# Division/CUDA-RayTracing

Hardware: AMD Instinct MI355X
Metric: Mrays/s + achieved HBM GB/s, Stanford bunny 1920x1080x8spp @1/2/4/8 GPU (higher is better)
Workload: dtype f32

## Files before the change

### cuda-raytracing_amd/__init__.py

```python
import contextlib
import ctypes
import os

import numpy as np
import torch

PKG_DIR = os.path.dirname(os.path.abspath(__file__))
ROOT_DIR = os.path.dirname(PKG_DIR)
LIB_PATH = os.path.join(PKG_DIR, "librt_hip.so")
EXP_LIB_PATH = os.path.join(PKG_DIR, "librt_hip_exp.so")
ASSETS_DIR = os.path.join(ROOT_DIR, "assets")

RT_RENDER_STATS = 1
RT_RENDER_VALIDATE = 16
TRACERS = {"fast": 0, "ref": 2, "flat": 4, "wavefront": 8}
STAT_NAMES = ("segments", "nodes", "tri_tests", "tri_accepts", "sphere_accepts", "hits", "misses", "cycles_tree_cut",
              "wave_small_iters", "lane_small", "wave_big_tris", "lane_big_tris", "wave_segment_iters",
              "lane_segments", "tree_nodes", "tree_tri_tests", "cycles_small", "cycles_big", "cycles_total",
              "rounds_coop", "rounds_shared", "coop_rays", "cycles_tree_clusters", "cycles_tree_tris",
              "big_tests", "twin_decided", "twin_tests", "wave_big_iters", "defer_end2", "defer_redo", None, None)
STAT_COUNT = len(STAT_NAMES)
SCENES = {"bunny": 0, "bunny4": 1, "plane1m": 2}

REFERENCE_SPP = 5
REFERENCE_BOUNCES = 6
RNG_STATE_BYTES = 48


class GPUCamera(ctypes.Structure):
    _fields_ = [("origin", ctypes.c_float * 3), ("viewport_worldspace_size", ctypes.c_float * 2),
                ("aspect", ctypes.c_float), ("horizontal", ctypes.c_float * 3),
                ("vertical", ctypes.c_float * 3), ("lower_left_corner", ctypes.c_float * 3)]


class GPUScene(ctypes.Structure):
    _fields_ = [("gpu_spheres", ctypes.c_void_p), ("gpu_materials", ctypes.c_void_p),
                ("gpu_bvh_nodes", ctypes.c_void_p), ("gpu_bvh_face_indices", ctypes.c_void_p),
                ("gpu_vertices", ctypes.c_void_p), ("gpu_faces", ctypes.c_void_p),
                ("sphere_count", ctypes.c_int32), ("material_count", ctypes.c_int32),
                ("rng_state", ctypes.c_void_p), ("environment_cubemap_tex", ctypes.c_uint64),
                ("camera", GPUCamera)]


class GPUMaterial(ctypes.Structure):
    _fields_ = [("albedo", ctypes.c_float * 4), ("emissive", ctypes.c_float * 4), ("specular", ctypes.c_float * 4),
                ("roughness", ctypes.c_float), ("specular_percent", ctypes.c_float), ("IOR", ctypes.c_float),
                ("_pad", ctypes.c_float)]


class BuildOptions(ctypes.Structure):
    _fields_ = [("leaf_tree_min", ctypes.c_uint32), ("cut_clusters", ctypes.c_uint32), ("cluster_max", ctypes.c_uint32),
                ("split_angle", ctypes.c_float), ("bvh_small", ctypes.c_uint32), ("host_bvh", ctypes.c_int32),
                ("leaf_screens", ctypes.c_int32)]


class RenderParams(ctypes.Structure):
    _fields_ = [("surface", ctypes.c_void_p), ("surface_last_frame", ctypes.c_void_p),
                ("width", ctypes.c_int32), ("height", ctypes.c_int32), ("pitch", ctypes.c_uint64),
                ("frame_index", ctypes.c_int32), ("spp", ctypes.c_int32), ("bounces", ctypes.c_int32),
                ("shard_index", ctypes.c_int32), ("shard_count", ctypes.c_int32), ("flags", ctypes.c_int32),
                ("out_shard", ctypes.c_void_p), ("stats", ctypes.c_void_p), ("segment_counter", ctypes.c_void_p),
                ("tile_list", ctypes.c_void_p), ("tile_count", ctypes.c_int64), ("wave_clock", ctypes.c_void_p),
                ("tune", ctypes.c_uint32), ("lane_slots", ctypes.c_void_p), ("lane_slot_count", ctypes.c_int64),
                ("lane_cost", ctypes.c_void_p), ("priority_waves", ctypes.c_int64), ("refill_lanes", ctypes.c_int32),
                ("waves_per_simd", ctypes.c_int32), ("lone_slots", ctypes.c_void_p), ("lone_count", ctypes.c_int64)]


class Ray(ctypes.Structure):
    _fields_ = [("origin", ctypes.c_float * 3), ("tmax", ctypes.c_float), ("direction", ctypes.c_float * 3),
                ("reserved", ctypes.c_uint32)]


class Hit(ctypes.Structure):
    _fields_ = [("t", ctypes.c_float), ("kind", ctypes.c_uint32), ("id", ctypes.c_uint32), ("material", ctypes.c_uint32),
                ("normal", ctypes.c_float * 3), ("bx", ctypes.c_float), ("position", ctypes.c_float * 3),
                ("by", ctypes.c_float)]


class TraceParams(ctypes.Structure):
    _fields_ = [("rays", ctypes.c_void_p), ("count", ctypes.c_int64), ("width", ctypes.c_int32), ("height", ctypes.c_int32),
                ("hits", ctypes.c_void_p), ("flags", ctypes.c_uint32), ("waves_per_simd", ctypes.c_int32)]


class DenoiseParams(ctypes.Structure):
    _fields_ = [("surface", ctypes.c_void_p), ("pitch", ctypes.c_uint64), ("width", ctypes.c_int32), ("height", ctypes.c_int32),
                ("hits", ctypes.c_void_p), ("materials", ctypes.c_void_p), ("material_count", ctypes.c_int32),
                ("flags", ctypes.c_int32), ("out", ctypes.c_void_p), ("out_pitch", ctypes.c_uint64),
                ("scratch", ctypes.c_void_p), ("scratch_bytes", ctypes.c_uint64), ("iterations", ctypes.c_int32),
                ("normal_power_log2", ctypes.c_int32), ("sigma_plane", ctypes.c_float), ("sigma_color", ctypes.c_float)]


HIT_MISS, HIT_SPHERE, HIT_TRIANGLE = 0, 1, 2
RAY_TMAX = 1e30
DENOISE_DEFAULT = -1
DENOISE_DEFAULTS = {"iterations": 5, "normal_power_log2": 5, "sigma_plane": 0.03, "sigma_color": 8.0}

assert ctypes.sizeof(GPUScene) == 136 and ctypes.sizeof(GPUMaterial) == 64
assert ctypes.sizeof(Ray) == 32 and ctypes.sizeof(Hit) == 48 and ctypes.sizeof(TraceParams) == 40
assert ctypes.sizeof(DenoiseParams) == 96

_P, _I, _U32, _U64, _F, _SZ = ctypes.c_void_p, ctypes.c_int, ctypes.c_uint32, ctypes.c_uint64, ctypes.c_float, ctypes.c_size_t
_FP = ctypes.POINTER(ctypes.c_float)
SIGNATURES = {
    "raytracing_process": (None, [_P, _P, _I, _I, _SZ, _I, _P]),
    "init_rng": (None, [_U32, _U32, _P, ctypes.c_uint]),
    "rt_render": (_I, [ctypes.POINTER(RenderParams), _P, _P]),
    "rt_trace_rays": (_I, [ctypes.POINTER(TraceParams), _P, _P]),
    "rt_denoise_scratch_bytes": (_SZ, [_I, _I]),
    "rt_denoise": (_I, [ctypes.POINTER(DenoiseParams), _P]),
    "rt_foreign_mirror_wait": (_I, [_P]),
    "rt_foreign_last_tracer": (_I, [_P]),
    "rt_experimental_loaded": (_I, []),
    "rt_init_rng": (_I, [_P, _I, _I, _I, _I, _U32, _P]),
    "rt_shard_tiles": (ctypes.c_int64, [_I, _I, _I, _I]),
    "rt_unshard": (_I, [_P, _U64, _I, _I, _I, _P, ctypes.c_int64, _P]),
    "rt_shard_plan_capacity": (ctypes.c_int64, [_I, _I, _I]),
    "rt_shard_plan": (_I, [_I, _I, _I, _P, ctypes.c_int64, _P, _P]),
    "rt_get_build_options": (None, [_P]),
    "rt_set_build_options": (_I, [_P]),
    "rt_lane_plan_capacity": (ctypes.c_int64, [ctypes.c_int64]),
    "rt_lane_plan": (ctypes.c_int64, [_P, ctypes.c_int64, ctypes.c_double, ctypes.c_double, _P, ctypes.c_int64, _P]),
    "rt_lone_plan": (ctypes.c_int64, [_P, ctypes.c_int64, ctypes.c_int64, _U32, _P]),
    "rt_lane_refine": (ctypes.c_int64, [_P, ctypes.c_int64, _P, ctypes.c_int64, _P, ctypes.c_double, _P, ctypes.c_int64,
                                        _P]),
    "rt_init_rng_tiles": (_I, [_P, _I, _I, _P, ctypes.c_int64, _U32, _P]),
    "rt_unshard_tiles": (_I, [_P, _U64, _I, _I, _I, _P, ctypes.c_int64, _P, _P]),
    "rt_comm_unique_id": (_I, [_P]),
    "rt_comm_init_rank": (_I, [ctypes.POINTER(_P), _I, _I, _P]),
    "rt_comm_init_all": (_I, [_P, _I, _P]),
    "rt_comm_destroy": (_I, [_P]),
    "rt_comm_rank": (_I, [_P]),
    "rt_comm_size": (_I, [_P]),
    "rt_comm_group_start": (_I, []),
    "rt_comm_group_end": (_I, []),
    "rt_gather_shards": (_I, [_P, _P, _SZ, _P, _SZ, _P, _I, _P]),
    "rt_tonemap_srgb8": (_I, [_P, _U64, _I, _I, _P, _P]),
    "rt_write_pfm": (_I, [ctypes.c_char_p, _P, _U64, _I, _I]),
    "rt_write_ppm": (_I, [ctypes.c_char_p, _P, _I, _I]),
    "rt_set_device": (_I, [_I]),
    "rt_device_count": (_I, []),
    "rt_malloc": (_I, [ctypes.POINTER(_P), _SZ]),
    "rt_malloc_pitch": (_I, [ctypes.POINTER(_P), ctypes.POINTER(_SZ), _SZ, _SZ]),
    "rt_free": (_I, [_P]),
    "rt_memcpy_h2d": (_I, [_P, _P, _SZ]),
    "rt_memcpy_d2h": (_I, [_P, _P, _SZ]),
    "rt_memcpy_d2d": (_I, [_P, _P, _SZ]),
    "rt_memset": (_I, [_P, _I, _SZ]),
    "rt_synchronize": (_I, []),
    "rt_last_error": (ctypes.c_char_p, []),
    "rt_cubemap_create": (_U64, [_FP, _I]),
    "rt_cubemap_destroy": (_I, [_U64]),
    "rt_scene_create": (_P, []),
    "rt_scene_destroy": (None, [_P]),
    "rt_scene_add_material": (_U32, [_P, ctypes.POINTER(GPUMaterial)]),
    "rt_scene_add_triangle": (None, [_P, _FP, _FP, _FP, _I]),
    "rt_scene_add_quad": (None, [_P, _FP, _FP, _FP, _FP, _I]),
    "rt_scene_add_sphere": (None, [_P, _FP, _F, _I]),
    "rt_scene_add_mesh_file": (_I, [_P, ctypes.c_char_p, _FP, _I]),
    "rt_scene_set_environment_file": (_I, [_P, ctypes.c_char_p]),
    "rt_scene_environment": (_I, [_P, ctypes.POINTER(_P), ctypes.POINTER(_I)]),
    "rt_scene_set_camera": (None, [_P, _FP, _F, _F]),
    "rt_scene_set_viewport": (None, [_P, _I, _I]),
    "rt_scene_upload": (_I, [_P, _P]),
    "rt_scene_gpu": (ctypes.POINTER(GPUScene), [_P]),
    "rt_scene_setup": (_I, [_P, _I, ctypes.c_char_p]),
    "rt_scene_setup_plane": (_I, [_P, _I, ctypes.c_char_p]),
    "rt_scene_build": (None, [_P]),
    "rt_scene_camera": (None, [_P, ctypes.POINTER(GPUCamera)]),
    "rt_scene_host_arrays": (_SZ, [_P, ctypes.POINTER(_P), ctypes.POINTER(_SZ), ctypes.POINTER(_P),
                                   ctypes.POINTER(_SZ), ctypes.POINTER(_P), ctypes.POINTER(_SZ), ctypes.POINTER(_P)]),
    "rt_scene_bvh_max_depth": (_I, [_P]),
    "rt_scene_materials": (_I, [_P, _P, ctypes.POINTER(_SZ)]),
    "rt_bvh_build_device": (_I, [_P, _U32, _P, _U32, _P, _P, ctypes.POINTER(_U32), ctypes.POINTER(_I), _P]),
    "rt_scene_mirror_info": (_I, [_P, ctypes.POINTER(_SZ), ctypes.POINTER(_SZ), ctypes.POINTER(_SZ)]),
    "rt_scene_mirror_copy": (_I, [_P, _P, _P, _P]),
    "rt_scene_mirror_nodes": (_I, [_P, _P, ctypes.POINTER(_SZ)]),
    "rt_scene_mirror_face_leaf": (_I, [_P, _P, ctypes.POINTER(_SZ)]),
    "rt_scene_mirror_twins": (_I, [_P, _P, ctypes.POINTER(_SZ), _P, ctypes.POINTER(_SZ)]),
    "rt_mirror_build_check": (_I, [_P, _SZ, _P, _SZ, _P, _SZ, _P, _SZ, _P, ctypes.POINTER(ctypes.c_int)]),
    "rt_cluster_cull_host": (_I, [_P, _P, ctypes.c_float, _P]),
    "rt_twin_check_host": (_I, [_P, _P, _P]),
    "rt_xorwow_jump_matrix": (_I, [_I, ctypes.POINTER(ctypes.c_uint32)]),
    "rt_xorwow_init_host": (None, [_U32, _U64, _P]),
}

_lib = None


class RTError(RuntimeError):
    pass


def lib():
    global _lib
    if _lib is None:
        if not os.path.exists(LIB_PATH):
            raise RTError(f"{LIB_PATH} not built; run `python -c 'import __graft_entry__ as g; g.build()'`")
        L = ctypes.CDLL(LIB_PATH)
        for name, (res, args) in SIGNATURES.items():
            fn = getattr(L, name)
            fn.restype = res
            fn.argtypes = args
        _lib = L
    return _lib


_exp_lib = None


def load_experimental():
    global _exp_lib
    lib()
    if _exp_lib is None:
        if not os.path.exists(EXP_LIB_PATH):
            raise RTError(f"{EXP_LIB_PATH} not built; run `python -c 'import __graft_entry__ as g; g.build()'`")
        _exp_lib = ctypes.CDLL(EXP_LIB_PATH)
    if lib().rt_experimental_loaded() != 1:
        raise RTError("librt_hip_exp.so loaded but its kernels are not registered with librt_hip.so: "
                      + lib().rt_last_error().decode(errors="replace"))
    return _exp_lib


def _check(code, what):
    if code:
        raise RTError(f"{what} failed ({code}): {lib().rt_last_error().decode(errors='replace')}")


def _f3(v):
    return (ctypes.c_float * 3)(*[float(x) for x in v])


def _stream_ptr(stream=None):
    s = stream if stream is not None else torch.cuda.current_stream()
    return ctypes.c_void_p(s.cuda_stream)


class Scene:

    def __init__(self):
        self.handle = lib().rt_scene_create()
        if not self.handle:
            raise RTError("rt_scene_create failed")

    def __del__(self):
        if getattr(self, "handle", None) and _lib is not None:
            _lib.rt_scene_destroy(self.handle)
            self.handle = None

    def add_material(self, albedo=(0, 0, 0), emissive=(0, 0, 0), specular=(0, 0, 0, 0), roughness=0.9,
                     specular_percent=0.0, ior=1.0):
        m = GPUMaterial()
        m.albedo[:] = [*map(float, albedo[:3]), 1.0]
        m.emissive[:] = [*map(float, emissive[:3]), 1.0]
        m.specular[:] = [*map(float, (list(specular) + [0.0])[:4])]
        m.roughness, m.specular_percent, m.IOR = roughness, specular_percent, ior
        return lib().rt_scene_add_material(self.handle, ctypes.byref(m))

    def add_triangle(self, a, b, c, material=0):
        lib().rt_scene_add_triangle(self.handle, _f3(a), _f3(b), _f3(c), material)

    def add_quad(self, a, b, c, d, material=0):
        lib().rt_scene_add_quad(self.handle, _f3(a), _f3(b), _f3(c), _f3(d), material)

    def add_sphere(self, position, radius, material=0):
        lib().rt_scene_add_sphere(self.handle, _f3(position), float(radius), material)

    def add_loaded_scene(self, mesh_path, transform, material=0):
        t = (ctypes.c_float * 16)(*[float(x) for x in transform])
        _check(lib().rt_scene_add_mesh_file(self.handle, mesh_path.encode(), t, material), "add_loaded_scene")

    def set_environment(self, path):
        _check(lib().rt_scene_set_environment_file(self.handle, path.encode()), "set_environment")

    def environment(self):
        p, n = ctypes.c_void_p(), ctypes.c_int()
        _check(lib().rt_scene_environment(self.handle, ctypes.byref(p), ctypes.byref(n)), "rt_scene_environment")
        if not p.value:
            return None
        k = n.value
        buf = ctypes.string_at(p.value, 6 * k * k * 16)
        return np.frombuffer(buf, dtype=np.float32).reshape(6, k, k, 4).copy()

    def setup(self, which="bunny", assets_dir=ASSETS_DIR):
        _check(lib().rt_scene_setup(self.handle, SCENES[which], assets_dir.encode()), f"setup({which})")

    def setup_plane(self, n=708, assets_dir=ASSETS_DIR):
        _check(lib().rt_scene_setup_plane(self.handle, int(n), assets_dir.encode()), f"setup_plane({n})")

    def set_camera(self, position=(0, 0, 0), angle_x=0.0, angle_y=180.0):
        lib().rt_scene_set_camera(self.handle, _f3(position), float(angle_x), float(angle_y))

    def set_viewport(self, width, height):
        lib().rt_scene_set_viewport(self.handle, int(width), int(height))

    def upload(self, rng_state_ptr):
        _check(lib().rt_scene_upload(self.handle, ctypes.c_void_p(rng_state_ptr)), "upload")

    @property
    def gpu(self):
        return lib().rt_scene_gpu(self.handle)

    def build(self):
        lib().rt_scene_build(self.handle)

    def camera(self):
        c = GPUCamera()
        lib().rt_scene_camera(self.handle, ctypes.byref(c))
        return c

    def max_depth(self):
        return lib().rt_scene_bvh_max_depth(self.handle)

    def mirror(self, trees=False):
        import numpy as np
        n = [ctypes.c_size_t() for _ in range(3)]
        _check(lib().rt_scene_mirror_info(self.handle, *[ctypes.byref(x) for x in n]), "rt_scene_mirror_info")
        tris = np.zeros((n[0].value, 12), dtype=np.float32)
        tree = np.zeros((n[1].value, 16), dtype=np.float32)
        ltris = np.zeros((n[2].value, 12), dtype=np.float32)
        _check(lib().rt_scene_mirror_copy(self.handle, tris.ctypes.data, tree.ctypes.data, ltris.ctypes.data),
               "rt_scene_mirror_copy")
        return (tris, tree, ltris) if trees else tris

    def mirror_nodes(self):
        import numpy as np
        n = ctypes.c_size_t()
        _check(lib().rt_scene_mirror_nodes(self.handle, None, ctypes.byref(n)), "rt_scene_mirror_nodes")
        out = np.zeros((n.value, 8), dtype=np.float32)
        _check(lib().rt_scene_mirror_nodes(self.handle, out.ctypes.data, ctypes.byref(n)), "rt_scene_mirror_nodes")
        return out

    def mirror_face_leaf(self):
        import numpy as np
        n = ctypes.c_size_t()
        _check(lib().rt_scene_mirror_face_leaf(self.handle, None, ctypes.byref(n)), "rt_scene_mirror_face_leaf")
        out = np.zeros(n.value, dtype=np.uint32)
        if n.value:
            _check(lib().rt_scene_mirror_face_leaf(self.handle, out.ctypes.data, ctypes.byref(n)), "rt_scene_mirror_face_leaf")
        return out

    def mirror_twins(self):
        import numpy as np
        nq, nu = ctypes.c_size_t(), ctypes.c_size_t()
        _check(lib().rt_scene_mirror_twins(self.handle, None, ctypes.byref(nq), None, ctypes.byref(nu)), "rt_scene_mirror_twins")
        q = np.zeros((nq.value, 28), dtype=np.float32)
        u = np.zeros((nu.value, 16), dtype=np.float32)
        _check(lib().rt_scene_mirror_twins(self.handle, q.ctypes.data, ctypes.byref(nq), u.ctypes.data, ctypes.byref(nu)),
               "rt_scene_mirror_twins")
        return q, u

    def materials(self):
        n = ctypes.c_size_t()
        _check(lib().rt_scene_materials(self.handle, None, ctypes.byref(n)), "rt_scene_materials")
        out = np.zeros((n.value, 16), dtype=np.float32)
        if n.value:
            _check(lib().rt_scene_materials(self.handle, out.ctypes.data, ctypes.byref(n)), "rt_scene_materials")
        return out

    def host_arrays(self):
        import numpy as np
        ptrs = [ctypes.c_void_p() for _ in range(4)]
        counts = [ctypes.c_size_t() for _ in range(3)]
        lib().rt_scene_host_arrays(self.handle, ctypes.byref(ptrs[0]), ctypes.byref(counts[0]), ctypes.byref(ptrs[1]),
                                   ctypes.byref(counts[1]), ctypes.byref(ptrs[2]), ctypes.byref(counts[2]),
                                   ctypes.byref(ptrs[3]))

        def grab(p, nbytes):
            if not p.value or nbytes == 0:
                return np.zeros(0, dtype=np.uint8)
            return np.frombuffer(ctypes.string_at(p.value, nbytes), dtype=np.uint8).copy()

        nn, nf, nv = counts[0].value, counts[1].value, counts[2].value
        return {"nodes": grab(ptrs[0], nn * 32), "face_indices": grab(ptrs[1], nf * 4),
                "vertices": grab(ptrs[2], nv * 32), "faces": grab(ptrs[3], nf * 16)}


def mirror_build_check(nodes, face_indices, faces, vertices):
    import numpy as np
    nodes, fi = np.ascontiguousarray(nodes), np.ascontiguousarray(face_indices, dtype=np.uint32)
    faces, vertices = np.ascontiguousarray(faces), np.ascontiguousarray(vertices)
    meta = np.zeros((fi.size, 2), dtype=np.uint32)
    tw = ctypes.c_int(0)
    _check(lib().rt_mirror_build_check(nodes.ctypes.data, nodes.shape[0], fi.ctypes.data, fi.size, faces.ctypes.data,
                                       faces.shape[0], vertices.ctypes.data, vertices.shape[0], meta.ctypes.data,
                                       ctypes.byref(tw)), "rt_mirror_build_check")
    return meta, bool(tw.value)


def bvh_build_device(vertices, faces, stream=None):
    import torch
    nf = faces.shape[0]
    nodes = torch.empty((max(1, 2 * nf - 1), 8), dtype=torch.float32, device=faces.device)
    fi = torch.empty((nf,), dtype=torch.int32, device=faces.device)
    count, depth = _U32(0), _I(0)
    _check(lib().rt_bvh_build_device(vertices.data_ptr(), vertices.shape[0], faces.data_ptr(), nf, nodes.data_ptr(),
                                     fi.data_ptr(), ctypes.byref(count), ctypes.byref(depth), _stream_ptr(stream)),
           "rt_bvh_build_device")
    return nodes, fi, count.value, depth.value


def alloc_surface(width, height, device=None):
    row_floats = ((width * 16 + 255) // 256) * 256 // 4
    t = torch.zeros((height, row_floats), dtype=torch.float32, device=device or "cuda")
    return t


def surface_view(t, width):
    return t[:, : width * 4].reshape(t.shape[0], width, 4)


def alloc_rng(count, device=None):
    return torch.zeros((count * RNG_STATE_BYTES // 4,), dtype=torch.int32, device=device or "cuda")


def init_rng_states(rng, width, height, seed, shard_index=0, shard_count=1, stream=None):
    _check(lib().rt_init_rng(ctypes.c_void_p(rng.data_ptr()), width, height, shard_index, shard_count, seed,
                             _stream_ptr(stream)), "rt_init_rng")


def render(scene, surface, last, width, height, spp, bounces, frame_index=0, shard_index=0, shard_count=1,
           out_shard=None, stats=None, segment_counter=None, stream=None, tracer="fast", tile_list=None,
           wave_clock=None, tune=0, lane_slots=None, lane_cost=None, priority_waves=0, refill_lanes=0,
           waves_per_simd=0, lone_slots=None, validate=False):
    p = RenderParams()
    if lone_slots is not None and lone_slots.numel() > 0:
        assert lone_slots.dtype == torch.int32 and lone_slots.is_cuda and lone_slots.dim() == 1
        p.lone_slots, p.lone_count = lone_slots.data_ptr(), lone_slots.numel()
    if lane_slots is not None:
        assert lane_slots.dtype == torch.int32 and lane_slots.is_cuda and lane_slots.numel() % 64 == 0
        p.lane_slots, p.lane_slot_count = lane_slots.data_ptr(), lane_slots.numel()
        p.priority_waves = int(priority_waves)
    if lane_cost is not None:
        assert lane_cost.dtype == torch.int32 and lane_cost.is_cuda
        p.lane_cost = lane_cost.data_ptr()
    if tile_list is not None:
        assert tile_list.dtype == torch.int32 and tile_list.is_cuda and tile_list.dim() == 1
        p.tile_list, p.tile_count = tile_list.data_ptr(), tile_list.numel()
    if wave_clock is not None:
        n = tile_list.numel() if tile_list is not None else tiles_of(width, height, shard_index, shard_count)
        waves = lane_slots.numel() // 64 if lane_slots is not None else 4 * n
        assert wave_clock.dtype == torch.int64 and wave_clock.numel() >= waves
        p.wave_clock = wave_clock.data_ptr()
    p.tune = int(tune)
    p.refill_lanes = int(refill_lanes)
    p.waves_per_simd = int(waves_per_simd)
    p.surface = surface.data_ptr() if surface is not None else None
    p.surface_last_frame = last.data_ptr() if last is not None else None
    p.width, p.height = width, height
    p.pitch = surface.shape[1] * 4 if surface is not None else width * 16
    p.frame_index, p.spp, p.bounces = frame_index, spp, bounces
    p.shard_index, p.shard_count = shard_index, shard_count
    p.out_shard = out_shard.data_ptr() if out_shard is not None else None
    p.flags = TRACERS[tracer] | (RT_RENDER_VALIDATE if validate else 0)
    if segment_counter is not None:
        p.segment_counter = segment_counter.data_ptr()
    if stats is not None:
        p.flags |= RT_RENDER_STATS
        p.stats = stats.data_ptr()
    gpu = scene.gpu if hasattr(scene, "gpu") else ctypes.pointer(scene)
    _check(lib().rt_render(ctypes.byref(p), ctypes.cast(gpu, ctypes.c_void_p), _stream_ptr(stream)), "rt_render")


def _trace(scene, rays, count, width, height, hits, stream, waves_per_simd):
    if hits is None:
        hits = torch.empty((count, 12), dtype=torch.float32, device=rays.device if rays is not None else "cuda")
    assert hits.dtype == torch.float32 and hits.is_cuda and hits.is_contiguous() and hits.dim() == 2
    assert hits.shape[1] == 12 and hits.shape[0] >= count
    p = TraceParams()
    p.rays = rays.data_ptr() if rays is not None else None
    p.count, p.width, p.height = count, width, height
    p.hits = hits.data_ptr()
    p.waves_per_simd = int(waves_per_simd)
    gpu = scene.gpu if hasattr(scene, "gpu") else ctypes.pointer(scene)
    _check(lib().rt_trace_rays(ctypes.byref(p), ctypes.cast(gpu, ctypes.c_void_p), _stream_ptr(stream)), "rt_trace_rays")
    return hits


def trace_rays(scene, rays, hits=None, stream=None, waves_per_simd=0):
    assert rays.dtype == torch.float32 and rays.is_cuda and rays.is_contiguous() and rays.dim() == 2 and rays.shape[1] == 8
    return _trace(scene, rays, rays.shape[0], 0, 0, hits, stream, waves_per_simd)


def trace_camera(scene, width, height, hits=None, stream=None, waves_per_simd=0):
    return _trace(scene, None, int(width) * int(height), int(width), int(height), hits, stream, waves_per_simd)


def hit_fields(hits):
    ints = hits.view(torch.int32) if isinstance(hits, torch.Tensor) else hits.view(np.int32)
    return {"t": hits[:, 0], "kind": ints[:, 1], "id": ints[:, 2], "material": ints[:, 3], "normal": hits[:, 4:7],
            "bx": hits[:, 7], "position": hits[:, 8:11], "by": hits[:, 11]}


def gbuffer(scene, width, height, stream=None, waves_per_simd=0):
    w, h = int(width), int(height)
    f = hit_fields(trace_camera(scene, w, h, stream=stream, waves_per_simd=waves_per_simd))
    hit = f["kind"] != HIT_MISS
    mats = torch.from_numpy(scene.materials()).to(hit.device)
    albedo = torch.zeros((w * h, 3), dtype=torch.float32, device=hit.device)
    if mats.shape[0]:
        albedo = torch.where(hit[:, None], mats[f["material"].long().clamp(0, mats.shape[0] - 1), :3], albedo)
    return {"depth": torch.where(hit, f["t"], torch.full_like(f["t"], float("inf"))).reshape(h, w),
            "normal": f["normal"].reshape(h, w, 3).clone(), "position": f["position"].reshape(h, w, 3).clone(),
            "albedo": albedo.reshape(h, w, 3), "material": f["material"].reshape(h, w).clone(),
            "prim": torch.where(hit, f["id"], torch.full_like(f["id"], -1)).reshape(h, w),
            "kind": f["kind"].reshape(h, w).clone()}


def denoise_scratch_bytes(width, height):
    return int(lib().rt_denoise_scratch_bytes(int(width), int(height)))


def _allocating_on(stream):
    return torch.cuda.stream(stream) if stream is not None else contextlib.nullcontext()


def _denoise(surface, hits, materials_ptr, material_count, width, height, out, scratch, iterations, normal_power_log2,
             sigma_plane, sigma_color, stream):
    w, h = int(width), int(height)
    assert surface.dtype == torch.float32 and surface.is_cuda and surface.dim() == 2 and surface.stride(1) == 1
    assert surface.shape[0] >= h and surface.shape[1] >= 4 * w
    assert hits.dtype == torch.float32 and hits.is_cuda and hits.is_contiguous() and hits.dim() == 2
    assert hits.shape[1] == 12 and hits.shape[0] >= w * h
    need = denoise_scratch_bytes(w, h)
    with _allocating_on(stream):
        if out is None:
            out = alloc_surface(w, h, device=surface.device)
        if scratch is None:
            scratch = torch.empty((need // 4,), dtype=torch.float32, device=surface.device)
    assert out.dtype == torch.float32 and out.is_cuda and out.dim() == 2 and out.stride(1) == 1
    assert out.shape[0] >= h and out.shape[1] >= 4 * w
    assert scratch.is_cuda and scratch.is_contiguous()
    p = DenoiseParams()
    p.surface, p.pitch = surface.data_ptr(), surface.stride(0) * 4
    p.width, p.height = w, h
    p.hits, p.materials, p.material_count = hits.data_ptr(), materials_ptr, int(material_count)
    p.out, p.out_pitch = out.data_ptr(), out.stride(0) * 4
    p.scratch, p.scratch_bytes = scratch.data_ptr(), scratch.numel() * scratch.element_size()
    p.iterations, p.normal_power_log2 = int(iterations), int(normal_power_log2)
    p.sigma_plane, p.sigma_color = float(sigma_plane), float(sigma_color)
    _check(lib().rt_denoise(ctypes.byref(p), _stream_ptr(stream)), "rt_denoise")
    return out
# ... 234 lines not shown
```

### cuda-raytracing_amd/build.py

```python
import os
import re
import shutil
import subprocess
import sys

ROOT = os.path.dirname(os.path.dirname(os.path.abspath(__file__)))
PKG = os.path.join(ROOT, "cuda-raytracing_amd")
CSRC = os.path.join(PKG, "csrc")
INC = os.path.join(ROOT, "include")
BUILD = os.path.join(PKG, "build")
LIB = os.path.join(PKG, "librt_hip.so")
ORACLE_DIR = os.path.join(ROOT, "oracle")
ORACLE_LIB = os.path.join(ORACLE_DIR, "liboracle.so")

HIPCC = os.environ.get("HIPCC", "/opt/rocm/bin/hipcc")
ARCH = os.environ.get("RT_OFFLOAD_ARCH", "gfx950")

FP_FLAGS = ["-ffp-contract=off", "-fno-fast-math"]
HIP_CODEGEN_FLAGS = ["-mllvm", "-structurizecfg-skip-uniform-regions=1", "-mllvm", "-amdgpu-remove-redundant-endcf=0"]
HOST_SOURCES = ["scene.cpp", "objload.cpp", "mirror.cpp", "leaftree.cpp", "xorwow.cpp", "image.cpp", "shard.cpp"]
HIP_SOURCES = ["rt_fast_prod.hip", "rt_fast_lean.hip", "rt_fast_timing.hip", "rt_fast_stats.hip", "rt_ref.hip", "rt_kernel.hip", "image.hip",
               "bvh_build.hip", "comm.hip", "rt_query.hip", "denoise.hip"]
EXP_SOURCES = ["rt_fast_ab.hip", "rt_fast_ab2.hip", "rt_fast_refill.hip", "rt_fast_screen.hip", "rt_lone.hip", "rt_wavefront.hip",
               "rt_exp.hip"]
# ... 22 lines not shown
                 "-fhip-fp32-correctly-rounded-divide-sqrt", "-munsafe-fp-atomics", "-fno-slp-vectorize",
                 *HIP_CODEGEN_FLAGS, "-I", INC, "-I", CSRC, "-c", os.path.join(CSRC, src), "-o", obj]


LLVM_BIN = "/opt/rocm/lib/llvm/bin"
_VECTOR_OP = re.compile(r"\s*(v_|global_|scratch_|buffer_|ds_|flat_)")
_LANE_OP = re.compile(r"\s*v_(readlane|readfirstlane|writelane)_")


def disassemble(obj):
    import tempfile
    with tempfile.TemporaryDirectory() as td:
        fat, co = os.path.join(td, "fat.bin"), os.path.join(td, "dev.co")
        secs = subprocess.run([f"{LLVM_BIN}/llvm-readelf", "-S", obj], check=True, capture_output=True, text=True).stdout
        if ".hip_fatbin" not in secs:
            return ""
        subprocess.run([f"{LLVM_BIN}/llvm-objcopy", f"--dump-section=.hip_fatbin={fat}", obj, os.path.join(td, "x.o")],
                       check=True, capture_output=True)
        subprocess.run([f"{LLVM_BIN}/clang-offload-bundler", "--type=o", f"--targets=hipv4-amdgcn-amd-amdhsa--{ARCH}",
                        f"--input={fat}", f"--output={co}", "--unbundle"], check=True, capture_output=True)
        return subprocess.run([f"{LLVM_BIN}/llvm-objdump", "-d", f"--mcpu={ARCH}", co], check=True,
                              capture_output=True, text=True).stdout


def parse_disassembly(dis):
    base, ins = {}, []
    kernel = None
    for ln in dis.split("\n"):
        m = re.match(r"^([0-9a-f]+) <(\S+)>:$", ln)
        if m:
            kernel = m.group(2)
            base[kernel] = int(m.group(1), 16)
            continue
        m = re.match(r"^\t(.*?)\s*// ([0-9A-F]+):[0-9A-F ]*(?:<(\S+)\+0x([0-9a-f]+)>)?", ln)
        if m:
            tgt = (m.group(3), int(m.group(4), 16)) if m.group(3) else None
            ins.append((int(m.group(2), 16), m.group(1), tgt, kernel))
    return base, ins


def exec_narrowing_hazards(dis):
    base, ins = parse_disassembly(dis)
    at = {a: i for i, (a, _, _, _) in enumerate(ins)}
    out = []
    for i, (addr, text, _, k) in enumerate(ins):
        if not text.startswith("s_and_b64 exec, exec,"):
            continue
        j, target = i + 1, None
        while j < len(ins) and not ins[j][1].startswith("s_or_b64 exec, exec,"):
            if target is None and ins[j][1].startswith("s_cbranch_execz") and ins[j][2]:
                sym, off = ins[j][2]
                target = base.get(sym, -1) + off
            j += 1
        if target is None:
            continue
        if target not in at:
            out.append((k, addr, ["(execz target not found)"]))
            continue
        bad = []
        for _, tx, _, _ in ins[at[target]:]:
            if tx.startswith("s_or_b64 exec, exec,") or tx.startswith("s_endpgm"):
                break
            if _VECTOR_OP.match(tx) and not _LANE_OP.match(tx):
                bad.append(tx)
        if bad:
            out.append((k, addr, bad))
    return out


def check_exec_narrowing(objs):
    problems, flagged = [], []
    for obj in objs:
        dis = disassemble(obj)
        if dis and not parse_disassembly(dis)[1]:
            problems.append(f"{os.path.basename(obj)}: device code but no instruction parsed (llvm-objdump format?)")
            flagged.append(obj)
            continue
        for k, addr, bad in exec_narrowing_hazards(dis):
            problems.append(f"{os.path.basename(obj)}: {k} at 0x{addr:x}: " + "; ".join(bad[:4]))
            flagged.append(obj)
    if problems:
        for obj in set(flagged):
            for f in (obj, obj + ".cmd"):
                if os.path.exists(f):
                    os.remove(f)
        raise RuntimeError("exec narrowed without a save with vector code behind it (tools/exec_narrow_scan.py, "
                           "rt_fast_body.h RT_FAST_FAMILY):\n  " + "\n  ".join(problems))


def _compile(jobs, force):
    headers = _deps(CSRC, (".h",)) + _deps(INC, (".h",))

    def stale(j):
        obj, cmd = j
        rec = obj + ".cmd"
        same_cmd = os.path.exists(rec) and open(rec).read() == " ".join(cmd)
        return force or not same_cmd or not _newer(obj, [cmd[cmd.index("-c") + 1]] + headers)

    def run(j):
        _run(j[1])
        with open(j[0] + ".cmd", "w") as fh:
            fh.write(" ".join(j[1]))

    from concurrent.futures import ThreadPoolExecutor
    workers = max(1, min(len(jobs), int(os.environ.get("MAX_JOBS", os.cpu_count() or 1)), 8))
    todo = [j for j in jobs if stale(j)]
    with ThreadPoolExecutor(max_workers=workers) as ex:
        list(ex.map(run, todo))
    return bool(todo)


def build_product(force=False):
    os.makedirs(BUILD, exist_ok=True)
    jobs = [_hip_job(src) for src in HIP_SOURCES]
    for src in HOST_SOURCES:
        obj = os.path.join(BUILD, src + ".o")
        jobs.append((obj, ["g++", "-O2", "-std=c++17", "-fPIC", *FP_FLAGS, "-I", INC, "-I", CSRC,
                           "-c", os.path.join(CSRC, src), "-o", obj]))
    exp_jobs = [_hip_job(src) for src in EXP_SOURCES]
    changed = _compile(jobs + exp_jobs, force)
    objs = [o for o, _ in jobs]
    eobjs = [o for o, _ in exp_jobs]
    relink = changed or not _newer(LIB, objs)
    relink_exp = changed or not _newer(EXP_LIB, eobjs + [LIB])
    if relink or relink_exp:
        check_exec_narrowing([o for o, _ in jobs + exp_jobs if o.endswith(".hip.o")])
    if relink:
        tmp = LIB + ".tmp"
        _run([HIPCC, "-shared", "-fPIC", f"--offload-arch={ARCH}", *objs, "-L/opt/rocm/lib", "-lrccl", "-o", tmp])
        os.replace(tmp, LIB)
    if relink_exp:
        tmp = EXP_LIB + ".tmp"
        _run([HIPCC, "-shared", "-fPIC", f"--offload-arch={ARCH}", *eobjs, "-L", PKG, "-l:librt_hip.so",
              "-Wl,-rpath,$ORIGIN", "-Wl,--no-undefined", "-o", tmp])
        os.replace(tmp, EXP_LIB)
    return LIB


HOST_DRIVER_SRC = os.path.join(ROOT, "tests", "cpp", "host_driver.cpp")
HOST_DRIVER = os.path.join(ROOT, "tests", "cpp", "host_driver")


def build_host_driver(force=False):
    deps = [HOST_DRIVER_SRC, LIB, os.path.join(INC, "rt_abi.h")]
    if not os.path.exists(HOST_DRIVER_SRC) or (not force and _newer(HOST_DRIVER, deps)):
        return HOST_DRIVER
    tmp = HOST_DRIVER + ".tmp"
    _run(["g++", "-O2", "-std=c++17", "-I", INC, HOST_DRIVER_SRC, "-L", PKG, "-lrt_hip",
          "-Wl,-rpath,$ORIGIN/../../cuda-raytracing_amd", "-o", tmp])
    os.replace(tmp, HOST_DRIVER)
    return HOST_DRIVER


def build_oracle(force=False):
    src = os.path.join(ORACLE_DIR, "rt_oracle.c")
    deps = [src, os.path.abspath(__file__)] + _deps(ORACLE_DIR, (".h",))
    if not force and _newer(ORACLE_LIB, deps):
        return ORACLE_LIB
    tmp = ORACLE_LIB + ".tmp"
    _run(["gcc", "-O2", "-std=c11", "-fPIC", "-shared", "-fopenmp", *FP_FLAGS, src, "-o", tmp, "-lm"])
    os.replace(tmp, ORACLE_LIB)
    return ORACLE_LIB


def build_reference_parts(force=False):
    out = os.path.join(ORACLE_DIR, "_ref", "libref_glm.so")
    deps = [os.path.join(ORACLE_DIR, "ref_glm.cpp"), os.path.join(ORACLE_DIR, "build_ref.sh")]
    if not os.path.isdir("/root/reference/include/glm") or (not force and _newer(out, deps)):
        return out if os.path.exists(out) else None
    _run(["bash", os.path.join(ORACLE_DIR, "build_ref.sh")])
    return out


def build_all(force=False):
    build_product(force)
    build_oracle(force)
    build_reference_parts(force)
    build_host_driver(force)


if __name__ == "__main__":
    build_all(force="--force" in sys.argv)
```

### cuda-raytracing_amd/csrc/mirror.cpp

```cpp
#include "mirror.h"

#include <cstdlib>
#include <functional>

#include "leaftree.h"

#include <algorithm>
#include <cmath>
#include <cstring>
#include <map>
#include <mutex>
#include <stdexcept>
#include <string>

namespace {
void put_flat(float* o, const float* p0, const float* p1, const float* p2, uint32_t face) {
    o[0] = p0[0], o[1] = p0[1], o[2] = p0[2];
    o[3] = p1[0] - p0[0], o[4] = p1[1] - p0[1], o[5] = p1[2] - p0[2];
    o[6] = p2[0] - p0[0], o[7] = p2[1] - p0[1], o[8] = p2[2] - p0[2];
    std::memcpy(&o[9], &face, 4);
    o[10] = o[11] = 0.0f;
}
void put_pair(float* q, const float* a, const float* b) {
    static const float zero[12] = {};
    if (!b) b = zero;
    for (int c = 0; c < 9; c++) q[2 * c] = a[c], q[2 * c + 1] = b[c];
    std::memcpy(&q[18], &a[9], 4);
    std::memcpy(&q[19], &b[9], 4);
}
}

void rt_twin_bounds(const float* r, float* kd, float* ke) {
    const double U = std::ldexp(1.0, -24);
    const double n1 = std::fabs((double)r[3]) + std::fabs((double)r[4]) + std::fabs((double)r[5]);
    const double n2 = std::fabs((double)r[6]) + std::fabs((double)r[7]) + std::fabs((double)r[8]);
    const double w = 1.0 + std::ldexp(1.0, -20);
    *kd = (float)(10.0001 * U * n1 * n2 * w * w);
    *ke = (float)(10.0001 * U * std::max(n1, n2) * w * w);
}

namespace {
bool build_twins(const float* tris, uint32_t first, uint32_t count, std::vector<float>& quads,
                 std::vector<float>& units, uint32_t* nq, uint32_t* nu) {
    if (count >= 0xffffu) return false;
    auto key = [&](uint32_t i, bool swapped) {
        const float* r = &tris[(size_t)(first + i) * 12];
        std::string k(reinterpret_cast<const char*>(r), 12);
        k.append(reinterpret_cast<const char*>(r + (swapped ? 6 : 3)), 12);
        k.append(reinterpret_cast<const char*>(r + (swapped ? 3 : 6)), 12);
        return k;
    };
    std::map<std::string, std::vector<uint32_t>> by;
    for (uint32_t i = 0; i < count; i++) by[key(i, false)].push_back(i);
    std::vector<char> used(count, 0);
    std::vector<std::pair<uint32_t, uint32_t>> un;
    for (uint32_t i = 0; i < count; i++) {
        if (used[i]) continue;
        used[i] = 1;
        uint32_t twin = ~0u;
        auto it = by.find(key(i, true));
        if (it != by.end())
            for (uint32_t j : it->second)
                if (!used[j]) {
                    twin = j;
                    used[j] = 1;
                    break;
                }
        un.push_back({i, twin});
    }
    static const float zero[12] = {};
    const uint32_t none = ~0u;
    auto face = [&](uint32_t pos) { return pos == none ? none : *reinterpret_cast<const uint32_t*>(&tris[(size_t)(first + pos) * 12 + 9]); };
    auto packed = [&](uint32_t pos, uint32_t twin) { return (pos & 0xffffu) | ((twin == none ? 0xffffu : twin) << 16); };
    for (const auto& [pos, twin] : un) {
        float q[16] = {};
        std::memcpy(q, &tris[(size_t)(first + pos) * 12], 10 * 4);
        const uint32_t ft = face(twin), w = packed(pos, twin);
        std::memcpy(&q[10], &ft, 4);
        std::memcpy(&q[11], &w, 4);
        rt_twin_bounds(&tris[(size_t)(first + pos) * 12], &q[12], &q[13]);
        if (twin == none) q[12] = -1.0f;
        units.insert(units.end(), q, q + 16);
    }
    for (size_t u = 0; u < un.size(); u += 2) {
        const bool hb = u + 1 < un.size();
        const float* ra = &tris[(size_t)(first + un[u].first) * 12];
        const float* rb = hb ? &tris[(size_t)(first + un[u + 1].first) * 12] : zero;
        float q[28] = {};
        put_pair(q, ra, rb);
        float kd, ke;
        rt_twin_bounds(ra, &kd, &ke);
        q[20] = un[u].second == none ? -1.0f : kd, q[22] = ke;
        rt_twin_bounds(rb, &kd, &ke);
        q[21] = (!hb || un[u + 1].second == none) ? -1.0f : kd, q[23] = ke;
        const uint32_t wa = packed(un[u].first, un[u].second), wb = hb ? packed(un[u + 1].first, un[u + 1].second) : none;
        const uint32_t fa = face(un[u].second), fb = hb ? face(un[u + 1].second) : none;
        std::memcpy(&q[24], &wa, 4);
        std::memcpy(&q[25], &wb, 4);
        std::memcpy(&q[26], &fa, 4);
        std::memcpy(&q[27], &fb, 4);
        quads.insert(quads.end(), q, q + 28);
    }
    *nq = (uint32_t)((un.size() + 1) / 2);
    *nu = (uint32_t)un.size();
    return true;
}
}

void rt_build_mirror(const GPUBVHNode* nodes, size_t node_count, const uint32_t* fi, size_t index_count,
                     const GPUFace* faces, size_t face_count, const GPUVertex* verts, size_t vertex_count,
                     MirrorHost* out) {
    auto bad = [](const char* what) { throw std::runtime_error(std::string("mirror: ") + what); };
    out->tris.assign(index_count * 12, 0.0f);
    for (size_t i = 0; i < index_count; i++) {
        const uint32_t f = fi[i];
        if (f >= face_count) bad("face index out of range");
        const GPUFace& fc = faces[f];
        if (fc.v0 >= vertex_count || fc.v1 >= vertex_count || fc.v2 >= vertex_count) bad("vertex index out of range");
        put_flat(&out->tris[i * 12], verts[fc.v0].position, verts[fc.v1].position, verts[fc.v2].position, f);
    }

    out->pairs.clear();
    out->quads.clear();
    out->units.clear();
    out->tree.clear();
    out->ltris.clear();
    out->flat.clear();
    out->depth = 0;
    out->fast = true;
    out->screens = 0;
    std::vector<uint32_t> big;
    out->spairs.assign(index_count * 20, 0.0f);
    if (node_count == 0) return;
    std::vector<std::pair<uint32_t, int>> st{{0u, 0}};
    size_t visited = 0;
    while (!st.empty()) {
        const auto [n, d] = st.back();
        st.pop_back();
        if (n >= node_count) bad("node index out of range");
        if (++visited > node_count) bad("node graph is not a tree");
        const GPUBVHNode& nd = nodes[n];
        for (int k = 0; k < 3; k++) {
            const float lo = std::fabs(nd.bmin[k]), hi = std::fabs(nd.bmax[k]);
            if ((lo != 0.0f && (lo < 0x1p-60f || lo > 0x1p62f)) || (hi != 0.0f && (hi < 0x1p-60f || hi > 0x1p62f)))
                out->fast = false;
        }
        if (nd.prim_count > 0) {
            if ((size_t)nd.first_index + nd.prim_count > index_count) bad("leaf range out of range");
            out->depth = std::max(out->depth, d);
            if (nd.prim_count > MIRROR_BIG_LEAF)
                big.push_back(n);
            else
                for (uint32_t j = 0; j < nd.prim_count; j += 2)
                    put_pair(&out->spairs[((size_t)nd.first_index + j) * 20], &out->tris[((size_t)nd.first_index + j) * 12],
                             j + 1 < nd.prim_count ? &out->tris[((size_t)nd.first_index + j + 1) * 12] : nullptr);
        } else {
            st.push_back({nd.first_index, d + 1});
            st.push_back({nd.first_index + 1, d + 1});
        }
    }
// ... 52 lines not shown
        }
        po = (uint32_t)(out->pairs.size() / 20);
        std::memcpy(&lead[10], &po, 4);
        std::memcpy(&lead[11], &pf, 4);
        for (uint32_t j = 0; j < nd.prim_count; j += 2) {
            float q[20];
            put_pair(q, &out->tris[((size_t)nd.first_index + j) * 12],
                     j + 1 < nd.prim_count ? &out->tris[((size_t)nd.first_index + j + 1) * 12] : nullptr);
            out->pairs.insert(out->pairs.end(), q, q + 20);
        }
        const uint32_t qb = (uint32_t)(out->quads.size() / 28), ub = (uint32_t)(out->units.size() / 16);
        uint32_t nq = 0, nu = 0;
        if (twins_ok && build_twins(out->tris.data(), nd.first_index, nd.prim_count, out->quads, out->units, &nq, &nu)) {
            float* second = &out->tris[((size_t)nd.first_index + 1) * 12];
            float* third = &out->tris[((size_t)nd.first_index + 2) * 12];
            std::memcpy(&second[10], &qb, 4);
            std::memcpy(&second[11], &nq, 4);
            std::memcpy(&third[10], &ub, 4);
            std::memcpy(&third[11], &nu, 4);
        }
    }
    const uint32_t nl = (uint32_t)(out->ltris.size() / 12);
    for (uint32_t r : roots) std::memcpy(&out->tree[(size_t)r * 16 + 12], &nl, 4);
    rt_build_treelets(nodes, node_count, out->treelets);
    rt_build_private_nodes(nodes, node_count, out->nodes);
    out->face_leaf.clear();
    if (!out->pairs.empty() || !out->tree.empty()) {
        std::vector<uint32_t> fl(face_count, FACE_NO_LEAF);
        const size_t nn = out->nodes.size() / 8;
        for (size_t k = 0; k < nn; k++) {
            uint32_t first, count;
            std::memcpy(&first, &out->nodes[k * 8 + 6], 4);
            std::memcpy(&count, &out->nodes[k * 8 + 7], 4);
            if (count == 0 || (size_t)first + count > index_count) continue;
            for (uint32_t i = first; i < first + count; i++) {
                uint32_t f;
                std::memcpy(&f, &out->tris[(size_t)i * 12 + 9], 4);
                if (f >= face_count) continue;
                fl[f] = fl[f] == FACE_NO_LEAF || fl[f] == (uint32_t)k ? (uint32_t)k : FACE_TWO_LEAVES;
            }
        }
        out->face_leaf.resize(face_count);
        std::memcpy(out->face_leaf.data(), fl.data(), face_count * 4);
    }
}

void rt_build_private_nodes(const GPUBVHNode* nodes, size_t node_count, std::vector<float>& out) {
    out.clear();
    if (node_count == 0) return;
    std::vector<uint32_t> slot(node_count, ~0u);
    slot[0] = 0;
    uint32_t pairs = 0;
    std::vector<uint32_t> st{0u};
    while (!st.empty()) {
        const uint32_t v = st.back();
        st.pop_back();
        const GPUBVHNode& nd = nodes[v];
        if (nd.prim_count > 0) continue;
        const uint32_t l = nd.first_index, r = nd.first_index + 1;
        slot[l] = 2 + 2 * pairs, slot[r] = 3 + 2 * pairs;
        pairs++;
        st.push_back(l);
        st.push_back(r);
    }
    out.assign((size_t)(2 + 2 * pairs) * 8, 0.0f);
    for (size_t v = 0; v < node_count; v++) {
        if (slot[v] == ~0u) continue;
        GPUBVHNode nd = nodes[v];
        if (nd.prim_count == 0) nd.first_index = slot[nd.first_index];
        std::memcpy(&out[(size_t)slot[v] * 8], &nd, sizeof nd);
    }
}

std::vector<float> rt_ltris_device_layout(const std::vector<float>& ltris) {
    const size_t n = ltris.size() / 12;
    std::vector<float> d(ltris.size());
    for (size_t i = 0; i < n; i++)
        for (int f = 0; f < 3; f++) std::memcpy(&d[(f * n + i) * 4], &ltris[i * 12 + 4 * f], 16);
    return d;
}

void rt_build_treelets(const GPUBVHNode* nodes, size_t node_count, std::vector<float>& out) {
    out.clear();
    if (node_count == 0 || nodes[0].prim_count > 0) return;
    constexpr uint32_t EMPTY = 0xffffffffu;
    const float inf = INFINITY;
    std::vector<uint32_t> roots{0u};
    for (size_t k = 0; k < roots.size(); k++) {
        std::vector<uint32_t> taken{roots[k]};
        std::map<uint32_t, bool> expanded;
        for (size_t q = 0; q < taken.size(); q++) {
            const GPUBVHNode& nd = nodes[taken[q]];
            if (nd.prim_count > 0) continue;
            if (taken.size() + 2 > 63) break;
            expanded[taken[q]] = true;
            taken.push_back(nd.first_index + 1);
            taken.push_back(nd.first_index);
        }
        struct Slot { uint32_t node; int parent; uint32_t size; unsigned long long anc; };
        std::vector<Slot> slots;
        std::function<uint32_t(uint32_t, int, unsigned long long)> place = [&](uint32_t n, int parent,
                                                                                unsigned long long anc) -> uint32_t {
            const uint32_t me = (uint32_t)slots.size();
            slots.push_back({n, parent, 1u, anc});
            if (expanded.count(n)) {
                const unsigned long long a2 = anc | (1ull << me);
                const uint32_t s1 = place(nodes[n].first_index + 1, (int)me, a2);
                const uint32_t s2 = place(nodes[n].first_index, (int)me, a2);
                slots[me].size = 1u + s1 + s2;
            }
            return slots[me].size;
        };
        place(roots[k], -1, 0ull);
        const size_t base = out.size();
        out.resize(base + 64 * 12, 0.0f);
        for (uint32_t p = 0; p < 64; p++) {
            float* o = &out[base + p * 12];
            if (p >= slots.size()) {
                o[0] = o[1] = o[2] = inf, o[3] = o[4] = o[5] = -inf;
                std::memcpy(&o[7], &EMPTY, 4);
                continue;
            }
            const GPUBVHNode& nd = nodes[slots[p].node];
            o[0] = nd.bmin[0], o[1] = nd.bmin[1], o[2] = nd.bmin[2], o[3] = nd.bmax[0], o[4] = nd.bmax[1], o[5] = nd.bmax[2];
            uint32_t X = nd.first_index, cnt = nd.prim_count, frontier = 0u;
            if (cnt == 0 && !expanded.count(slots[p].node)) {
                X = (uint32_t)roots.size();
                roots.push_back(slots[p].node);
                frontier = 1u;
            }
            std::memcpy(&o[6], &X, 4);
            std::memcpy(&o[7], &cnt, 4);
            const uint32_t lo = (uint32_t)slots[p].anc, hi = (uint32_t)(slots[p].anc >> 32);
            std::memcpy(&o[8], &lo, 4);
            std::memcpy(&o[9], &hi, 4);
            std::memcpy(&o[10], &slots[p].size, 4);
            std::memcpy(&o[11], &frontier, 4);
        }
    }
}

namespace {
struct Entry {
    const void* face_indices;
    const void* vertices;
    const void* faces;
    void* block;
    MirrorDevice dev;
};
std::mutex g_mutex;
std::map<const void*, Entry> g_mirrors;

void release(Entry& e) {
    if (e.block) rt_free(e.block);
    e.block = nullptr;
}
}

int rt_internal_install_mirror(const GPUScene* s, const MirrorHost& m, bool owned, uint64_t fingerprint) {
    const std::vector<float> lt = rt_ltris_device_layout(m.ltris);
    const std::vector<float>* parts[11] = {&m.nodes, &m.tris, &m.pairs, &m.tree, &lt, &m.spairs, &m.flat, &m.treelets, &m.quads,
                                           &m.units, &m.face_leaf};
    size_t off[11], total = 0;
    for (int i = 0; i < 11; i++) {
        off[i] = total;
        total += (parts[i]->size() * 4 + 255) & ~(size_t)255;
    }
    void* block = nullptr;
    if (rt_malloc(&block, total + 256) != 0) return -1;
    char* b = static_cast<char*>(block);
    for (int i = 0; i < 11; i++)
        if (!parts[i]->empty() && rt_memcpy_h2d(b + off[i], parts[i]->data(), parts[i]->size() * 4) != 0) {
            rt_free(block);
            return -1;
        }
    auto at = [&](int i) -> const void* { return parts[i]->empty() ? nullptr : b + off[i]; };
    Entry e{s->gpu_bvh_face_indices, s->gpu_vertices, s->gpu_faces, block, {}};
    e.dev.nodes = at(0);
    e.dev.tris = b + off[1];
    e.dev.pairs = at(2);
    e.dev.tree = at(3);
    e.dev.ltris = at(4);
    e.dev.spairs = at(5);
    e.dev.flat = at(6);
    e.dev.treelets = at(7);
    e.dev.quads = at(8);
    e.dev.units = at(9);
    e.dev.face_leaf = at(10);
    e.dev.depth = m.depth;
    e.dev.fast = m.fast;
    e.dev.screens = m.screens;
    e.dev.owned = owned;
    e.dev.fingerprint = fingerprint;
    std::lock_guard<std::mutex> lock(g_mutex);
    auto it = g_mirrors.find(s->gpu_bvh_nodes);
    if (it != g_mirrors.end()) {
        release(it->second);
        g_mirrors.erase(it);
    }
    g_mirrors.emplace(s->gpu_bvh_nodes, e);
    return 0;
}

void rt_internal_forget_mirror(const void* gpu_nodes) {
    std::lock_guard<std::mutex> lock(g_mutex);
    auto it = g_mirrors.find(gpu_nodes);
    if (it == g_mirrors.end()) return;
    release(it->second);
    g_mirrors.erase(it);
}

bool rt_internal_lookup_mirror(const GPUScene* s, MirrorDevice* out) {
    std::lock_guard<std::mutex> lock(g_mutex);
    *out = MirrorDevice{};
    auto it = g_mirrors.find(s->gpu_bvh_nodes);
    if (it == g_mirrors.end()) return false;
    const Entry& e = it->second;
    if (e.face_indices != s->gpu_bvh_face_indices || e.vertices != s->gpu_vertices || e.faces != s->gpu_faces) {
        out->depth = e.dev.depth;
        return false;
    }
    *out = e.dev;
    return true;
}

namespace {
std::mutex g_opt_mutex;
rt_build_options default_options() {
    rt_build_options o;
    const LeafTreeParams p;
    o.leaf_tree_min = MIRROR_TREE_LEAF;
    o.cut_clusters = p.cut_clusters;
    o.cluster_max = p.cluster_max;
    o.split_angle = (float)p.split_angle;
    o.bvh_small = 16;
    o.host_bvh = 0;
    o.leaf_screens = 0;
    return o;
}
rt_build_options g_options = default_options();
}

extern "C" int rt_mirror_build_check(const GPUBVHNode* nodes, size_t node_count, const uint32_t* face_indices,
                                     size_t index_count, const GPUFace* faces, size_t face_count,
                                     const GPUVertex* vertices, size_t vertex_count, uint32_t* meta, int* twins) {
    try {
        MirrorHost m;
        rt_build_mirror(nodes, node_count, face_indices, index_count, faces, face_count, vertices, vertex_count, &m);
        for (size_t i = 0; i < index_count; i++) std::memcpy(&meta[2 * i], &m.tris[i * 12 + 10], 8);
        *twins = m.twins && !m.quads.empty() ? 1 : 0;
        return 0;
    } catch (const std::exception& e) {
        rt_internal_set_error(e.what());
        return -1;
    }
}

extern "C" void rt_get_build_options(rt_build_options* out) {
    if (!out) return;
    std::lock_guard<std::mutex> lock(g_opt_mutex);
    *out = g_options;
}

extern "C" int rt_set_build_options(const rt_build_options* o) {
    const rt_build_options v = o ? *o : default_options();
    if (v.leaf_tree_min < 2 || v.cut_clusters < 1 || v.cut_clusters > 32 || v.cluster_max < 1 || v.cluster_max > kClusterMax ||
        !(v.split_angle >= 0.0f && v.split_angle < 3.2f) || v.bvh_small < 2 || v.bvh_small > 64 || (v.host_bvh != 0 && v.host_bvh != 1) ||
        (v.leaf_screens != 0 && v.leaf_screens != 1)) {
        rt_internal_set_error("rt_set_build_options: value out of range");
        return 1;
    }
    std::lock_guard<std::mutex> lock(g_opt_mutex);
    g_options = v;
    return 0;
}
```

### cuda-raytracing_amd/csrc/mirror.h

```cpp
#pragma once

#include <cstddef>
#include <cstdint>
#include <vector>

#include "rt_abi.h"

constexpr uint32_t MIRROR_BIG_LEAF = 8;
constexpr uint32_t MIRROR_TREE_LEAF = 1024;
constexpr uint32_t FACE_NO_LEAF = 0xffffffffu, FACE_TWO_LEAVES = 0xfffffffeu;

struct MirrorHost {
    std::vector<float> nodes;
    std::vector<float> tris;
    std::vector<float> pairs;
    std::vector<float> quads;
    std::vector<float> units;
    std::vector<float> spairs;
    std::vector<float> tree;
    std::vector<float> ltris;
    std::vector<float> flat;
    std::vector<float> treelets;
    std::vector<float> face_leaf;
    int depth = 0;
    bool fast = true;
    int screens = 0;
    bool twins = true;
};

void rt_build_mirror(const GPUBVHNode* nodes, size_t node_count, const uint32_t* face_indices, size_t index_count,
                     const GPUFace* faces, size_t face_count, const GPUVertex* vertices, size_t vertex_count,
                     MirrorHost* out);

void rt_twin_bounds(const float* rec, float* kd, float* ke);

std::vector<float> rt_ltris_device_layout(const std::vector<float>& ltris);

void rt_build_private_nodes(const GPUBVHNode* nodes, size_t node_count, std::vector<float>& out);

void rt_build_treelets(const GPUBVHNode* nodes, size_t node_count, std::vector<float>& out);

struct MirrorDevice {
    const void* nodes = nullptr;
    const void* tris = nullptr;
    const void* pairs = nullptr;
    const void* quads = nullptr;
    const void* units = nullptr;
    const void* spairs = nullptr;
    const void* tree = nullptr;
    const void* ltris = nullptr;
    const void* flat = nullptr;
    const void* treelets = nullptr;
    const void* face_leaf = nullptr;
    int depth = -1;
    bool fast = false;
    int screens = 0;
    bool owned = true;
    uint64_t fingerprint = 0;
};
int rt_internal_install_mirror(const GPUScene* scene, const MirrorHost& m, bool owned = true,
                               uint64_t fingerprint = 0);
void rt_internal_forget_mirror(const void* gpu_nodes);
bool rt_internal_lookup_mirror(const GPUScene* scene, MirrorDevice* out);

void rt_internal_set_error(const char* msg);
```

### cuda-raytracing_amd/csrc/rt_common.h

```cpp
#pragma once

#include <hip/hip_runtime.h>

#include "rt_abi.h"
#include "rt_math.h"

namespace rtk {

constexpr int TILE = 16;
constexpr int BLOCK = 256;
constexpr int WAVE = 64;

struct FlatTri {
    float4 a, b, c;
};

struct RenderArgs {
    const GeometrySphere* spheres;
    const GPUMaterial* materials;
    const GPUBVHNode* nodes;
    const uint32_t* face_indices;
    const GPUVertex* vertices;
    const GPUFace* faces;
    const FlatTri* tris;
    rt_rng_state* rng;
    const float* sky;
    int sky_n;
    int sphere_count;
    GPUCamera cam;
    float qw, qx, qy, qz;
    char* surface;
    const char* last;
    float4* out_shard;
    uint64_t pitch;
    int width, height, frame_index, spp, bounces;
    int shard_index, shard_count, tiles_x;
    const int32_t* tile_list;
    unsigned long long* wave_clock;
    const int32_t* lane_slots;
    long long slot_count;
    long long entry_count;
    unsigned long long* queue_head;
    int refill_lanes;
    int waves_per_simd;
    uint32_t* lane_cost;
    int priority_waves;
    const int* gate;
    int gate_value;
    unsigned long long* stats;
    unsigned long long* seg_counter;
    int scene_fast;
    int screens;
    const float4* pairs;
    const float4* quads;
    const float4* units;
    const float4* tree;
    const float4* ltris;
    const float4* spairs;
    const float4* flat;
    const uint32_t* face_leaf;
    uint32_t tune;
};

struct Counters {
    unsigned long long seg = 0, node = 0, tri = 0, tacc = 0, sacc = 0, hit = 0, miss = 0;
    unsigned long long w_small = 0, l_small = 0, w_big = 0, l_big = 0, w_seg = 0, l_seg = 0;
    unsigned long long ktest = 0, ktri = 0;
    unsigned long long cy_small = 0, cy_big = 0, r_coop = 0, r_shared = 0, coop_rays = 0, w_iter = 0;
    unsigned long long cy_tcl = 0, cy_ttri = 0, cy_tree = 0;
    uint32_t lane_work = 0;
    unsigned long long big_tests = 0, tw_test = 0, tw_dec = 0, big_iters = 0;
    uint32_t end2 = 0, redo = 0;
};

__device__ __forceinline__ rtm::f3 ld3(const float* p) { return rtm::f3{p[0], p[1], p[2]}; }

__device__ __forceinline__ int shard_tile(const RenderArgs& a, int k) {
    const int t = a.tile_list ? a.tile_list[k] : a.shard_index + k * a.shard_count;
    return (t >= 0 && t < a.tiles_x * ((a.height + TILE - 1) / TILE)) ? t : -1;
}

__device__ __forceinline__ void tile_pixel(int tid, int* lx, int* ly) {
    const int w = tid >> 6, l = tid & 63;
    *lx = (w & 1) * 8 + (l & 7);
    *ly = (w >> 1) * 8 + (l >> 3);
}

}
```

### cuda-raytracing_amd/csrc/rt_fast.h

```cpp
#pragma once

namespace rtfast {

constexpr int BIG = 8;
constexpr int LEAN_BIT = 128;
constexpr int WAVE = 64;

using rtm::f3;

struct Ray {
    f3 o, d, nd, r;
    bool fast;
};

__device__ __forceinline__ bool in_range_or_zero(float v, float lo, float hi) {
    const float a = fabsf(v);
    return v == 0.0f || (a >= lo && a <= hi);
}

__device__ __forceinline__ Ray make_ray(f3 o, f3 d, f3 nd, bool scene_fast) {
    Ray R;
    R.o = o, R.d = d, R.nd = nd;
    R.r = rtm::mk(1.0f / d.x, 1.0f / d.y, 1.0f / d.z);
    const float dlo = 0x1p-40f, dhi = 0x1p20f;
// ... 687 lines not shown
}

template <bool TIMING, class C>
__device__ __forceinline__ void coop_tree(const float4* tris, const float4* tree, const float4* ltris, const float4* flat,
                                          unsigned long long m, uint32_t root_l, const Ray& R, Hit& h, const Trav& T,
                                          uint32_t* scratch, uint32_t tune, C& c) {
    const uint32_t lane = threadIdx.x & 63u;
    const bool order = (tune & 0x80000000u) != 0;
    const f3 rnd_l = rtm::mk(1.0f / R.nd.x, 1.0f / R.nd.y, 1.0f / R.nd.z);
    while (m) {
        const int r = __ffsll((long long)m) - 1;
        m &= m - 1;
        if (TIMING && lane == 0) c.r_coop++;
        const uint32_t root = (uint32_t)__builtin_amdgcn_readlane((int)root_l, r);
        const uint32_t f0 = (uint32_t)__builtin_amdgcn_readlane((int)T.first, r);
        const uint32_t c0 = (uint32_t)__builtin_amdgcn_readlane((int)T.count, r);
        Ray B;
        B.o = bcast3(R.o, r);
        B.nd = bcast3(R.nd, r);
        B.d = B.nd, B.r = B.nd;
        B.fast = __builtin_amdgcn_readlane(R.fast ? 1 : 0, r) != 0;
        const f3 rnd = bcast3(rnd_l, r);
        const float best = bcast(h.best, r);
        const f4v K2 = ((ConstF4)(tree + 4 * (size_t)root))[2];
        const f4v KR = ((ConstF4)(tree + 4 * (size_t)root))[3];
        const uint32_t cb = __float_as_uint(K2.x), nc = __float_as_uint(K2.y), kb = __float_as_uint(K2.z),
                       nk = __float_as_uint(K2.w);
        const size_t ln = __float_as_uint(KR.x);
        const float4* cl = flat + cb;
        const float4* ct = flat + kb;
        LeafBest L;
        L.t = best, L.j = 0, L.id = 0, L.bx = 0.0f, L.by = 0.0f, L.found = false;
        L.nan = !(best == best);
        const bool cull_ok = B.fast && !L.nan;
        float cbest = best;
        for (uint32_t kbase = 0; kbase < nk; kbase += 64u) {
            const uint32_t k = kbase + lane;
            bool need = false;
            uint32_t s0 = 0, s1 = 0;
            float te = 0.0f;
            if (k < nk) {
                const float4 K0 = ct[k], K1 = ct[nk + k], K3 = ct[3 * nk + k];
                s0 = __float_as_uint(K3.y), s1 = __float_as_uint(K3.z);
                need = !(cull_ok && (__float_as_uint(K3.w) & 1u) && cluster_cull(B, rnd, cbest, K0, K1, ct[2 * nk + k], K3));
                if (order) {
                    const float tx1 = (K0.x - B.o.x) * rnd.x, tx2 = (K1.x - B.o.x) * rnd.x;
                    const float ty1 = (K0.y - B.o.y) * rnd.y, ty2 = (K1.y - B.o.y) * rnd.y;
                    const float tz1 = (K0.z - B.o.z) * rnd.z, tz2 = (K1.z - B.o.z) * rnd.z;
                    te = fmaxf(fmaxf(fminf(tx1, tx2), fminf(ty1, ty2)), fminf(tz1, tz2));
                    te = te == te ? te : 0.0f;
                }
            }
            const unsigned long long mk = __ballot(need);
            const uint32_t ns = (uint32_t)__popcll(mk);
            if (TIMING && lane == 0) c.ktest += min(64u, nk - kbase), c.r_shared += ns;
            uint32_t rank = 0;
            if (order) {
                for (unsigned long long w = mk; w; w &= w - 1) {
                    const int b = __ffsll((long long)w) - 1;
                    const float tb = bcast(te, b);
                    rank += (tb < te || (tb == te && b < (int)lane)) ? 1u : 0u;
                }
            } else {
                rank = __builtin_amdgcn_mbcnt_hi((uint32_t)(mk >> 32), __builtin_amdgcn_mbcnt_lo((uint32_t)mk, 0u));
            }
            for (uint32_t q = 0; q < ns; q += 2) {
                const int a = __ffsll((long long)__ballot(need && rank == q)) - 1;
                const int b = q + 1 < ns ? __ffsll((long long)__ballot(need && rank == q + 1)) - 1 : -1;
                const uint32_t a0 = (uint32_t)__builtin_amdgcn_readlane((int)s0, a);
                const uint32_t a1 = (uint32_t)__builtin_amdgcn_readlane((int)s1, a);
                uint32_t b0 = 0, b1 = 0;
                if (b >= 0) {
                    b0 = (uint32_t)__builtin_amdgcn_readlane((int)s0, b);
                    b1 = (uint32_t)__builtin_amdgcn_readlane((int)s1, b);
                }
                const unsigned long long tc0 = TIMING ? __builtin_amdgcn_s_memtime() : 0;
                const uint32_t ci = lane < 32u ? a0 + lane : b0 + (lane - 32u);
                const bool has = lane < 32u ? ci < a1 : ci < b1;
                bool need2 = false;
                uint32_t tb = 0, n = 0;
                if (has) {
                    const float4 Q3 = cl[3 * nc + ci];
                    const uint32_t info = __float_as_uint(Q3.w);
                    tb = __float_as_uint(Q3.z), n = info >> 8;
                    need2 = !(cull_ok && (info & 1u) && cluster_cull(B, rnd, cbest, cl[ci], cl[nc + ci], cl[2 * nc + ci], Q3));
                }
                const unsigned long long mc = __ballot(need2);
                const uint32_t nsc = (uint32_t)__popcll(mc);
                if (TIMING && lane == 0) c.l_big++, c.ktest += __popcll(__ballot(has)), c.coop_rays += nsc;
                const unsigned long long tc1 = TIMING ? __builtin_amdgcn_s_memtime() : 0;
                if (TIMING) c.cy_tcl += tc1 - tc0;
                if (need2) {
                    const uint32_t rk = __builtin_amdgcn_mbcnt_hi((uint32_t)(mc >> 32), __builtin_amdgcn_mbcnt_lo((uint32_t)mc, 0u));
                    scratch[rk] = tb | ((n - 1u) << 26);
                }
                __builtin_amdgcn_wave_barrier();
                constexpr uint32_t CL = kClusterMax, PER = 64u / kClusterMax;
                for (uint32_t base = 0; base < nsc; base += PER) {
                    if (TIMING && lane == 0) c.w_big++;
                    const uint32_t slot = base + lane / CL, i = lane % CL;
                    if (slot < nsc) {
                        const uint32_t w = scratch[slot], my_tb = w & 0x03ffffffu, my_n = (w >> 26) + 1u;
                        if (i < my_n) {
                            const size_t t = (size_t)(my_tb + i);
                            leaf_candidate(B, ltris[t], ltris[ln + t], ltris[2 * ln + t], L);
                        }
                    }
                }
                __builtin_amdgcn_wave_barrier();
                if (TIMING) c.cy_ttri += __builtin_amdgcn_s_memtime() - tc1;
                if (__ballot(L.found)) {
                    const uint32_t mk2 = __ockl_wfred_min_u32(L.found ? tkey(L.t) : 0xffffffffu);
                    const float up = __uint_as_float(mk2 + 1u);
                    cbest = fminf(cbest, up);
                }
            }
        }
        if (__ballot(L.nan)) {
            if ((int)lane == r) {
                for (uint32_t q = f0; q < f0 + c0; q++) {
                    float t, x, y;
                    bool dummy = false;
                    const float4 A = tris[3 * q], Bq = tris[3 * q + 1], Cc = tris[3 * q + 2];
                    if (tri_accept(R.o, R.nd, A, Bq, Cc, h.best, &t, &x, &y, &dummy)) {
                        h.best = t, h.kind = 2, h.bx = x, h.by = y;
                        h.id = __float_as_uint(Cc.y);
                    }
                }
            }
            continue;
        }
        const uint32_t mt = __ockl_wfred_min_u32(L.found ? tkey(L.t) : 0xffffffffu);
        const uint32_t mj = __ockl_wfred_min_u32(L.found && tkey(L.t) == mt ? L.j : 0xffffffffu);
        if (mt != 0xffffffffu) {
            const int wl = __ffsll((long long)__ballot(L.found && L.j == mj)) - 1;
            const float wt = bcast(L.t, wl), wbx = bcast(L.bx, wl), wby = bcast(L.by, wl);
            const uint32_t wid = (uint32_t)__builtin_amdgcn_readlane((int)L.id, wl);
            if ((int)lane == r) h.best = wt, h.kind = 2, h.id = wid, h.bx = wbx, h.by = wby;
        }
    }
}


template <bool STATS, class C>
__device__ __forceinline__ bool trav_begin(const float4* nodes4, const Ray& R, const Hit& h, Trav& T, C& c) {
    const float4 lo = nodes4[0], hi = nodes4[1];
    if (STATS) c.node++;
    float tmin, tmax;
    slab_exact(R, lo, hi, &tmin, &tmax);
    T.first = __float_as_uint(hi.z), T.count = __float_as_uint(hi.w), T.sp = (int)threadIdx.x * 4;
    return tmax >= tmin && tmin < h.best && tmax > 0.0f;
}

template <bool STATS, class C>
__device__ __forceinline__ bool screen_leaf(const float4* tris, const float4* pairs, const Ray& R, Hit& h, const Trav& T,
                                            C& c) {
    if (!R.fast || !pairs) return false;
    const float4 lead = tris[3 * (size_t)T.first + 2];
    if (__float_as_uint(lead.w) != 3u) return false;
    const float4* S = pairs + 5 * ((size_t)__float_as_uint(lead.z) - 1);
    const float4 K0 = S[0], K1 = S[1], K2 = S[2], K3 = S[3];
    const f3 rnd = rtm::mk(1.0f / R.nd.x, 1.0f / R.nd.y, 1.0f / R.nd.z);
    if (!cluster_cull(R, rnd, h.best, K0, K1, K2, K3)) return false;
    const float4 P = S[4];
    const uint32_t n = __float_as_uint(K3.y);
    const uint32_t pos[4] = {__float_as_uint(P.x), __float_as_uint(P.y), __float_as_uint(P.z), __float_as_uint(P.w)};
    for (uint32_t k = 0; k < n && k < 4u; k++) {
        const size_t i = (size_t)T.first + pos[k];
        test_triangle<STATS>(R, tris[3 * i], tris[3 * i + 1], tris[3 * i + 2], h, c);
    }
    return true;
}

constexpr uint32_t DEFER_NONE = 0xffffffffu, DEFER_OFF = 0xfffffffeu, DEFER_END1 = 0xfffffffdu, DEFER_END2 = 0xfffffffcu;
constexpr int DEFER_WORDS = 5 * 64;
template <int MODE>
__device__ __forceinline__ uint32_t* defer_words(uint32_t* scratch) {
    return scratch + ((MODE & 4) ? 64 : 0) + (threadIdx.x & 63u);
}

__device__ __forceinline__ float next_up(float t) {
    return __uint_as_float((__float_as_uint(t) & 0x7fffffffu) + 1u);
}

__device__ __forceinline__ bool defer_leaf(uint32_t* D, const float4* nodes4, const Trav& T, const Ray& R, const Hit& h) {
    if (!D || D[0] != DEFER_NONE || !(h.best <= 1e30f) || !R.fast) return false;
    const f4v lo = ((ConstF4)nodes4)[0], hi = ((ConstF4)nodes4)[1];
    const float sc = fmaxf(fmaxf(fmaxf(fabsf(lo.x), fabsf(lo.y)), fmaxf(fabsf(lo.z), fabsf(lo.w))),
                           fmaxf(fabsf(hi.x), fabsf(hi.y)));
    const float ro = fmaxf(fmaxf(fabsf(R.o.x), fabsf(R.o.y)), fabsf(R.o.z));
    if (!(sc < 0x1p16f && ro < 0x1p16f)) return false;
    D[0] = T.first, D[64] = T.count, D[128] = __float_as_uint(h.best);
    return true;
}

template <bool DEFER, class S>
__device__ __forceinline__ bool pop_d(const float4* nodes4, uint32_t* D, const S& stk, const Ray& R, const Hit& h, Trav& T) {
    for (;;) {
        if (!pop(nodes4, stk, T.sp, R, h.best, T.first, T.count)) return false;
        if (!DEFER || T.count <= (uint32_t)BIG || !defer_leaf(D, nodes4, T, R, h)) return true;
    }
}

template <bool STATS, bool SCR = false, bool DEF = false, bool LEAN = false, class S, class C>
__device__ __forceinline__ bool small_step(const float4* nodes4, const float4* tris, const float4* spairs, const S& stk,
                                           const Ray& R, Hit& h, Trav& T, C& c, const float4* pairs = nullptr,
                                           uint32_t* D = nullptr) {
    if constexpr (SCR) {
        if (T.count > (uint32_t)BIG) {
            if (!screen_leaf<STATS>(tris, pairs, R, h, T, c)) {
                T.sp |= SCREENED;
                return true;
            }
            return pop(nodes4, stk, T.sp, R, h.best, T.first, T.count);
        }
    }
    if (T.count > 0) {
        if (!STATS && (LEAN || spairs)) {
            for (uint32_t i = T.first; i < T.first + T.count; i += 2) pair_test(R, ld_pair(spairs, i), h);
        } else {
            for (uint32_t i = T.first; i < T.first + T.count; i++)
                test_triangle<STATS>(R, tris[3 * i], tris[3 * i + 1], tris[3 * i + 2], h, c);
        }
        return pop_d<DEF>(nodes4, D, stk, R, h, T);
    }
    if (inner_step<STATS>(nodes4, stk, T.sp, R, h.best, T.first, T.count, c)) {
        if (!DEF || T.count <= (uint32_t)BIG || !defer_leaf(D, nodes4, T, R, h)) return true;
    }
    return pop_d<DEF>(nodes4, D, stk, R, h, T);
}

template <bool STATS, int MODE, class C>
__device__ __forceinline__ bool big_round(const float4* tris, const float4* pairs, const float4* quads, const float4* units,
                                          const float4* tree,
                                          const float4* ltris, const float4* flat, uint32_t* scratch, uint32_t tune,
                                          unsigned long long big, bool waiting,
                                          const Ray& R, Hit& h, const Trav& T, C& c) {
    constexpr bool LEAN = (MODE & LEAN_BIT) != 0;
    if ((MODE & 4) && (LEAN || tree)) {
        bool at_tree = false;
        uint32_t root = 0;
        if (waiting) {
            const float4 lead = tris[3 * (size_t)T.first + 2];
            at_tree = __float_as_uint(lead.w) == 2u;
            root = __float_as_uint(lead.z);
        }
        const unsigned long long mt = __ballot(at_tree);
        if (mt) {
            if (!STATS && (LEAN || flat) && (tune & 0x40000000u) == 0)
            {
                const unsigned long long tt0 = (MODE & 8) ? __builtin_amdgcn_s_memtime() : 0;
                coop_tree<(MODE & 8) != 0>(tris, tree, ltris, flat, mt, root, R, h, T, scratch, tune, c);
                if (MODE & 8) c.cy_tree += __builtin_amdgcn_s_memtime() - tt0;
            }
            else if (at_tree)
                tree_leaf<STATS>(tris, tree, ltris, root, T.first, T.count, R, h, c);
            return at_tree;
        }
    }
    const int l0 = __ffsll((long long)big) - 1;
    const uint32_t f0 = __builtin_amdgcn_readlane(T.first, l0);
    const uint32_t c0 = __builtin_amdgcn_readlane(T.count, l0);
    if (STATS) {
        uint32_t mx = waiting ? T.count : 0u;
        for (int off = 32; off > 0; off >>= 1) mx = max(mx, (uint32_t)__shfl_xor((int)mx, off));
        c.w_big += (threadIdx.x & 63) == 0 ? mx : 0;
        c.l_big += waiting ? T.count : 0;
    }
    if (__ballot(waiting && T.first == f0) == big) {
        const f4v lead = ((ConstF4)(tris + 3 * (size_t)f0))[2];
        const uint32_t k = (uint32_t)__popcll(big);
        if (!STATS && (MODE & 3) < 2 && (LEAN || quads) && (__float_as_uint(lead.w) & 1u)) {
            const f4v l2 = ((ConstF4)(tris + 3 * (size_t)f0 + 3))[2];
            const f4v l3 = ((ConstF4)(tris + 3 * (size_t)f0 + 6))[2];
            const uint32_t nq = __float_as_uint(l2.w), nu = __float_as_uint(l3.w);
            const uint32_t cw = (tune >> 21) & 7u;
            if (nu && (tune & 1u) == 0 && k * (70u * ((nu + 63u) / 64u) + 70u) * (cw ? cw : 4u) < 4u * 95u * nq) {
                coop_units<(MODE & 8) != 0>(tris, units + 4 * (size_t)__float_as_uint(l3.z), nu, big, f0, c0, R, h, c);
                if (MODE & 8) c.r_coop++, c.coop_rays += k;
                return waiting;
            }
            if (nq) {
                if (MODE & 8) c.r_shared++;
                const Hit h0 = h;
                uint32_t bpos = NO_POS;
                bool nan = !(h.best == h.best);
                ConstF4 qs = (ConstF4)(quads + 7 * (size_t)__float_as_uint(l2.z));
                for (uint32_t q = 0; q < nq; q++, qs += 7) {
                    const Pair P = make_pair(qs[0], qs[1], qs[2], qs[3], qs[4]);
                    const f4v bnd = qs[5];
                    if (waiting) quad_test<(MODE & 8) != 0>(R.o, R.nd, P, bnd, qs + 6, h, bpos, nan, c);
                }
                if (MODE & 8) c.big_iters += nq;
                if (waiting && nan) {
                    h = h0;
                    leaf_sequential(tris, f0, c0, R.o, R.nd, h);
                }
                return waiting;
            }
        }
        if (!STATS && (MODE & 3) < 2 && (LEAN || pairs) && (__float_as_uint(lead.w) & 1u)) {
            const float4* lp = pairs + 5 * (size_t)__float_as_uint(lead.z);
            const uint32_t np = (c0 + 1u) / 2u, chunks = (np + 63u) / 64u;
            const uint32_t cchunks = (c0 + 63u) / 64u;
            if ((MODE & 3) == 0 && (tune & 1u) == 0 && k * (40u * chunks + 60u) < 40u * np) {
                coop_leaf(tris, lp, big, f0, c0, R, h);
// ... 45 lines not shown
    return big_round<STATS, MODE>(tris, pairs, quads, units, tree, ltris, flat, scratch, tune, big, waiting, R, h, T, c) || dfr;
}

__device__ __forceinline__ uint32_t bcastu(uint32_t v, int lane) { return (uint32_t)__builtin_amdgcn_readlane((int)v, lane); }

template <class S>
__device__ __forceinline__ void lone_traverse(const float4* nodes4, const float4* tris, const S& stk, int r,
                                              const Ray& R, Hit& h, Trav& T, bool& active) {
    constexpr int SL = S::LDS_ENTRIES;
    const int lane = (int)(threadIdx.x & 63u);
    const int sp0 = (int)bcastu((uint32_t)T.sp, r);
    const int rc = S::column(sp0);
    uint32_t* const col = stk.lds0 + rc;
    int sp = S::depth(sp0);
    uint32_t cf = bcastu(T.first, r), cc = bcastu(T.count, r);
    Ray U;
    U.o = bcast3(R.o, r), U.d = bcast3(R.d, r), U.nd = bcast3(R.nd, r), U.r = bcast3(R.r, r);
    U.fast = __builtin_amdgcn_readlane(R.fast ? 1 : 0, r) != 0;
    float best = bcast(h.best, r);
    int kind = __builtin_amdgcn_readlane(h.kind, r);
    uint32_t id = bcastu(h.id, r);
    float bx = bcast(h.bx, r), by = bcast(h.by, r);
    uint32_t e_idx = 0, e_first = 0, e_count = 0;
    float e_tmin = 0.0f;
    bool e_exact = false;
    if (lane < sp) {
        e_idx = col[lane * S::LANES];
        const float4 lo = nodes4[2 * e_idx], hi = nodes4[2 * e_idx + 1];
        float tx;
        if (U.fast) {
            slab_approx(U, lo, hi, &e_tmin, &tx);
        } else {
            slab_exact(U, lo, hi, &e_tmin, &tx);
            e_exact = true;
        }
        e_first = __float_as_uint(hi.z), e_count = __float_as_uint(hi.w);
    }
    bool done = false;
    for (;;) {
        bool do_pop = false;
        if (cc == 0) {
            const f4v a0 = ((ConstF4)nodes4)[2 * cf], a1 = ((ConstF4)nodes4)[2 * cf + 1];
            const f4v b0 = ((ConstF4)nodes4)[2 * cf + 2], b1 = ((ConstF4)nodes4)[2 * cf + 3];
            const float4 l0 = make_float4(a0.x, a0.y, a0.z, a0.w), l1 = make_float4(a1.x, a1.y, a1.z, a1.w);
            const float4 r0 = make_float4(b0.x, b0.y, b0.z, b0.w), r1 = make_float4(b1.x, b1.y, b1.z, b1.w);
            float tl = 0.0f, tlx = 0.0f, tr = 0.0f, trx = 0.0f;
            int okl = UNSURE, okr = UNSURE, rlt = UNSURE;
            if (U.fast) {
                slab_approx(U, l0, l1, &tl, &tlx);
                slab_approx(U, r0, r1, &tr, &trx);
                okl = classify_ok(tl, tlx);
                okr = classify_ok(tr, trx);
                rlt = okr == YES ? classify_lt(tr, best) : NO;
            }
            bool exact_l = false;
            if (__builtin_amdgcn_readfirstlane((okl == UNSURE || okr == UNSURE || rlt == UNSURE) ? 1 : 0)) {
                slab_exact(U, l0, l1, &tl, &tlx);
                slab_exact(U, r0, r1, &tr, &trx);
                okl = (tlx >= tl && tlx > 0.0f) ? YES : NO;
                okr = (trx >= tr && trx > 0.0f) ? YES : NO;
                rlt = (okr == YES && tr < best) ? YES : NO;
                exact_l = true;
            }
            if (__builtin_amdgcn_readfirstlane(rlt == YES ? 1 : 0)) {
                if (__builtin_amdgcn_readfirstlane(okl == YES ? 1 : 0)) {
                    if (lane == sp) {
                        e_idx = cf, e_tmin = tl, e_exact = exact_l;
                        e_first = __float_as_uint(l1.z), e_count = __float_as_uint(l1.w);
                    }
                    sp++;
                }
                cf = __float_as_uint(r1.z), cc = __float_as_uint(r1.w);
            } else {
                bool llt = false;
                if (__builtin_amdgcn_readfirstlane(okl == YES ? 1 : 0)) {
                    int cl = exact_l ? (tl < best ? YES : NO) : classify_lt(tl, best);
                    if (__builtin_amdgcn_readfirstlane(cl == UNSURE ? 1 : 0)) {
                        float te, tx;
                        slab_exact(U, l0, l1, &te, &tx);
                        cl = te < best ? YES : NO;
                    }
                    llt = __builtin_amdgcn_readfirstlane(cl == YES ? 1 : 0) != 0;
                }
                if (llt) cf = __float_as_uint(l1.z), cc = __float_as_uint(l1.w);
                else do_pop = true;
            }
        } else if (cc <= (uint32_t)BIG) {
            float t = 0.0f, x = 0.0f, y = 0.0f;
            bool nan = false, acc = false;
            if ((uint32_t)lane < cc) {
                const uint32_t i = cf + (uint32_t)lane;
                acc = tri_accept(U.o, U.nd, tris[3 * i], tris[3 * i + 1], tris[3 * i + 2], best, &t, &x, &y, &nan);
            }
            if (__ballot(nan)) {
                if (lane == 0) {
                    for (uint32_t i = cf; i < cf + cc; i++) {
                        float tt, xx, yy;
                        bool dummy = false;
                        if (tri_accept(U.o, U.nd, tris[3 * i], tris[3 * i + 1], tris[3 * i + 2], best, &tt, &xx, &yy, &dummy)) {
                            best = tt, kind = 2, bx = xx, by = yy, id = __float_as_uint(tris[3 * i + 2].y);
                        }
                    }
                }
                best = bcast(best, 0), kind = __builtin_amdgcn_readlane(kind, 0), id = bcastu(id, 0);
                bx = bcast(bx, 0), by = bcast(by, 0);
            } else if (__ballot(acc)) {
                const uint32_t mk = __ockl_wfred_min_u32(acc ? tkey(t) : 0xffffffffu);
                const uint32_t mi = __ockl_wfred_min_u32(acc && tkey(t) == mk ? (uint32_t)lane : 0xffffffffu);
                const int wl = (int)mi;
                best = bcast(t, wl), bx = bcast(x, wl), by = bcast(y, wl), kind = 2;
                id = __float_as_uint(tris[3 * (cf + mi) + 2].y);
            }
            do_pop = true;
        } else {
            break;
        }
        if (do_pop) {
            int cl = NO;
            if (lane < sp) cl = e_exact ? (e_tmin < best ? YES : NO) : classify_lt(e_tmin, best);
            if (__ballot(cl == UNSURE)) {
                if (cl == UNSURE) {
                    const float4 lo = nodes4[2 * e_idx], hi = nodes4[2 * e_idx + 1];
                    float tx;
                    slab_exact(U, lo, hi, &e_tmin, &tx);
                    e_exact = true;
                    cl = e_tmin < best ? YES : NO;
                }
            }
            const unsigned long long m = __ballot(cl == YES);
            if (!m) {
                done = true;
                sp = 0;
                break;
            }
            const int j = 63 - __clzll((long long)m);
            cf = bcastu(e_first, j), cc = bcastu(e_count, j);
            sp = j;
        }
    }
    if (lane == r) {
        T.first = cf, T.count = cc, T.sp = S::empty(rc) + sp * S::STEP;
        h.best = best, h.kind = kind, h.id = id, h.bx = bx, h.by = by;
        active = !done;
    }
    if (!done) {
        if (lane < sp && lane < SL) col[lane * S::LANES] = e_idx;
        for (int j = SL; j < sp; j++) {
            const uint32_t v = bcastu(e_idx, j);
            if (lane == r) stk.put(S::empty(rc) + j * S::STEP, v);
        }
    }
}

template <bool STATS, int MODE, class S, class C>
__device__ __forceinline__ void trace(const float4* nodes4, const float4* tris, const float4* pairs,
                                      const float4* tree, const float4* ltris, const float4* flat,
                                      const float4* spairs, uint32_t tune_arg, const S& stk, uint32_t* scratch,
                                      Ray& R, Hit& h, bool live, C& c, const float4* quads = nullptr,
                                      const float4* units = nullptr, const uint32_t* face_leaf = nullptr) {
    constexpr bool LEAN = (MODE & LEAN_BIT) != 0;
    const uint32_t tune = LEAN ? 0u : tune_arg;
    Trav T{0, 0, 0};
    bool active = live && trav_begin<STATS>(nodes4, R, h, T, c);
    constexpr bool scr_on = !STATS && (MODE & 16) != 0 && (MODE & 32) != 0;
    constexpr bool TIMING = (MODE & 8) != 0;
    constexpr bool DEFER = !STATS && (MODE & 32) == 0 && (MODE & 4) != 0;
    uint32_t* const D = (DEFER && (tune & (1u << 24)) == 0) ? defer_words<MODE>(scratch) : nullptr;
    if (D) D[0] = DEFER_NONE;
    unsigned long long t0 = TIMING ? __builtin_amdgcn_s_memtime() : 0;
    for (;;) {
        if constexpr ((MODE & 16) != 0) {
            const bool inner = active && T.count == 0;
            const bool leafs = active && T.count > 0 && (T.count <= (uint32_t)BIG || (scr_on && !(T.sp & SCREENED)));
            const unsigned long long mI = __ballot(inner), mL = __ballot(leafs);
            if (mI | mL) {
                const uint32_t nI = (uint32_t)__popcll(mI), nL = (uint32_t)__popcll(mL);
                if constexpr (!STATS) {
#ifndef RT_LONE_MAX
#define RT_LONE_MAX 1
#endif
                    if (nI + nL <= (uint32_t)RT_LONE_MAX && (tune & (1u << 26)) == 0) {
                        const int r = __ffsll((long long)(mI | mL)) - 1;
                        if (S::depth(__builtin_amdgcn_readlane(T.sp, r)) <= S::LDS_ENTRIES &&
                            (!scr_on || (uint32_t)__builtin_amdgcn_readlane((int)T.count, r) <= (uint32_t)BIG)) {
#ifdef RT_LANE_HIST
                            const unsigned long long tl0 = TIMING ? __builtin_amdgcn_s_memtime() : 0;
#endif
                            lone_traverse(nodes4, tris, stk, r, R, h, T, active);
#ifdef RT_LANE_HIST
                            if (TIMING) c.cy_ttri += __builtin_amdgcn_s_memtime() - tl0;
#endif
                            continue;
                        }
                    }
                }
                const uint32_t qv = (tune >> 13) & 7u, q = qv ? qv - 1u : 1u;
                if (TIMING) c.w_small++, c.l_small += inner || leafs;
#ifdef RT_LANE_HIST
                const unsigned long long th0 = TIMING ? __builtin_amdgcn_s_memtime() : 0;
#endif
                if (!mI || nL * 4u >= nI * (q + 1u)) {
                    if (leafs) {
                        active = small_step<STATS, scr_on, false, LEAN>(nodes4, tris, spairs, stk, R, h, T, c, pairs);
                        if (TIMING) c.lane_work++;
                    }
                } else if (inner) {
                    active = small_step<STATS, false, DEFER, LEAN>(nodes4, tris, spairs, stk, R, h, T, c, nullptr, D);
                    if (TIMING) c.lane_work++;
                }
#ifdef RT_LANE_HIST
                if (TIMING) {
                    const unsigned long long dt = __builtin_amdgcn_s_memtime() - th0;
                    const uint32_t n = nI + nL;
                    c.ktest += n <= 4u ? dt : 0ull;
                    c.ktri += (n > 4u && n <= 16u) ? dt : 0ull;
                    c.cy_tcl += dt;
                    c.r_shared += n <= 4u;
                }
#endif
                continue;
            }
        }
        const bool small = active && T.count <= (uint32_t)BIG;
        if (__ballot(small)) {
            if (STATS) {
                c.w_small += (threadIdx.x & 63) == 0;
                c.l_small += small;
            } else if (TIMING) {
                c.w_small++;
                c.l_small += small;
            }
            if (small) {
                active = small_step<STATS>(nodes4, tris, spairs, stk, R, h, T, c);
                if (TIMING) c.lane_work++;
            }
            continue;
        }
        if (TIMING) {
            const unsigned long long t1 = __builtin_amdgcn_s_memtime();
            c.cy_small += t1 - t0;
            t0 = t1;
        }
        const unsigned long long big = __ballot(active);
        if (!big) {
            if (DEFER && D) {
                const uint32_t st = D[0];
                bool go = false;
                if (st < DEFER_END2) {
                    const uint32_t entry = D[128], h1 = __float_as_uint(h.best);
                    D[192] = h1, D[256] = st, D[0] = DEFER_END1;
                    h.best = h1 != entry ? next_up(h.best) : h.best;
                    T.first = st, T.count = D[64];
                    go = true;
                } else if (st == DEFER_END1) {
                    const uint32_t entry = D[128], h1 = D[192];
                    const float bnd = h1 != entry ? next_up(__uint_as_float(h1)) : __uint_as_float(h1);
                    D[0] = DEFER_NONE;
                    if (__float_as_uint(h.best) == __float_as_uint(bnd)) {
                        h.best = __uint_as_float(h1);
                        if (h1 != entry) {
                            const uint32_t P = (LEAN || face_leaf) ? face_leaf[h.id] : 0xffffffffu;
                            float tp = INFINITY, tx;
                            if (P < 0xfffffffeu) slab_exact(R, ldo(nodes4, 2 * P), ldo(nodes4, 2 * P + 1), &tp, &tx);
                            if (tp > h.best) {
                                const float b2 = P < 0xfffffffeu ? next_up(tp) : __uint_as_float(entry);
                                T.first = D[256], T.count = D[64];
                                D[256] = __float_as_uint(b2), D[0] = DEFER_END2;
                                h.best = b2;
                                if (TIMING) c.end2++;
                                go = true;
                            }
                        }
                    }
                } else if (st == DEFER_END2) {
                    if (__float_as_uint(h.best) != D[256]) {
                        h.best = __uint_as_float(D[128]);
                        D[0] = DEFER_OFF;
                        if (TIMING) c.redo++;
                        active = trav_begin<STATS>(nodes4, R, h, T, c);
                    } else {
                        h.best = __uint_as_float(D[192]);
                        D[0] = DEFER_NONE;
                    }
                }
                if (go) active = true;
                if (__ballot(active)) continue;
            }
            break;
        }
        if (big_round_d<STATS, MODE>(nodes4, D, tris, pairs, quads, units, tree, ltris, flat, scratch, tune, big, active, R, h,
                                     T, c)) {
            if (TIMING) c.lane_work += 3;
            if constexpr (scr_on) T.sp &= ~SCREENED;
            active = pop_d<DEFER>(nodes4, D, stk, R, h, T);
        }
        if (TIMING) {
            const unsigned long long t1 = __builtin_amdgcn_s_memtime();
            c.cy_big += t1 - t0;
            t0 = t1;
        }
    }
}

}
```

### cuda-raytracing_amd/csrc/rt_fast_body.h

```cpp
#pragma once

#include <hip/hip_runtime.h>

#include <algorithm>
#include <map>
#include <mutex>
#include <utility>

#include "rt_abi.h"
#include "rt_device.h"
#include "rt_math.h"
#include "rt_common.h"
#include "leaftree.h"
#include "rt_fast.h"
#include "rt_render.h"

namespace rtk {

typedef const volatile __attribute__((address_space(4))) RenderArgs* KernelArgs;
template <bool COLD, class T>
__device__ __forceinline__ T arg(const RenderArgs& a, T RenderArgs::*m) {
    if constexpr (COLD) return ((KernelArgs)__builtin_amdgcn_kernarg_segment_ptr())->*m;
    else return a.*m;
}
// ... 116 lines not shown
        }
    };
    auto bind_entry = [&](long long i) {
        const long long s = a.lane_slots ? (long long)a.lane_slots[i] : i;
        const bool ok = s >= 0 && s < a.slot_count;
        bind(ok ? (int)(s >> 8) : -1, (int)(s & 255));
    };
    const int lane = (int)(threadIdx.x & 63u);
    const int lb = xcd_block(LEAN ? 0u : a.tune);
    bind_entry((long long)lb * WAVE + lane);
    if (a.lane_slots && lb < a.priority_waves) __builtin_amdgcn_s_setprio(3);
    constexpr bool REFILL = (MODE & 64) != 0;
    bool drained = !REFILL || a.queue_head == nullptr || __popcll(__ballot(pixel)) < 32;
    const long long qbase = (long long)gridDim.x * WAVE;
    Counters c;
    const rtm::f3 cam_o = ld3(a.cam.origin), cam_h = ld3(a.cam.horizontal), cam_v = ld3(a.cam.vertical),
                  cam_ll = ld3(a.cam.lower_left_corner);
    float acc_r = 0.0f, acc_g = 0.0f, acc_b = 0.0f;
    int sample = 0, bounce = 0;
    bool path = false;
    rtm::f3 ro = cam_o, rd = cam_o, color = rtm::mk(0, 0, 0), thr = rtm::mk(1, 1, 1);
    auto cam = [&](const rtm::f3& loaded, size_t off) {
        if constexpr (COLD) return arg3<true>(a, offsetof(RenderArgs, cam) + off);
        else return loaded;
    };
    const unsigned long long t_start = (MODE & 8) ? __builtin_amdgcn_s_memtime() : 0;
    const bool wave_times = (MODE & 8) && !LEAN && (a.tune & 2048u);
    const unsigned long long rt_start = (a.wave_clock || wave_times) ? __builtin_amdgcn_s_memrealtime() : 0;

#ifdef RT_LIVE_HIST
    unsigned long long lh_t = 0;
    uint32_t lh_n = 0;
#endif
    for (;;) {
        if (!drained) {
            const unsigned long long idle = __ballot(!pixel && !path);
            const uint32_t ni = (uint32_t)__popcll(idle);
            if (ni && (ni >= (uint32_t)a.refill_lanes || !__ballot(path))) {
                const int lead = __ffsll((long long)idle) - 1;
                unsigned long long base = 0;
                if (lane == lead) base = atomicAdd(a.queue_head, (unsigned long long)ni);
                base = ((unsigned long long)(uint32_t)__builtin_amdgcn_readlane((int)(uint32_t)(base >> 32), lead) << 32) |
                       (uint32_t)__builtin_amdgcn_readlane((int)(uint32_t)base, lead);
                const long long qn = a.entry_count - qbase;
                if (!pixel && !path) {
                    const unsigned long long i =
                        base + __builtin_amdgcn_mbcnt_hi((uint32_t)(idle >> 32), __builtin_amdgcn_mbcnt_lo((uint32_t)idle, 0u));
                    if ((long long)i < qn) {
                        bind_entry(qbase + (long long)i);
                        acc_r = acc_g = acc_b = 0.0f;
                        sample = 0;
                    }
                }
                if ((long long)(base + ni) >= qn) drained = true;
            }
        }
        if (pixel && !path) {
            if (sample < A(&RenderArgs::spp)) {
                const float ru = rng.uniform();
                const float rv = rng.uniform();
                const float uvx = ((float)x + ru) / (float)A(&RenderArgs::width);
                const float uvy = ((float)y + rv) / (float)A(&RenderArgs::height);
                const rtm::f3 co = cam(cam_o, offsetof(GPUCamera, origin)), ch = cam(cam_h, offsetof(GPUCamera, horizontal)),
                              cv = cam(cam_v, offsetof(GPUCamera, vertical)),
                              cl = cam(cam_ll, offsetof(GPUCamera, lower_left_corner));
                ro = co;
                rd = rtm::sub(rtm::add(rtm::add(cl, rtm::muls(ch, uvx)), rtm::muls(cv, uvy)), co);
                color = rtm::mk(0, 0, 0);
                thr = rtm::mk(1, 1, 1);
                bounce = 0;
                path = true;
                if (A(&RenderArgs::bounces) == 0) {
                    sample++;
                    path = false;
                    continue;
                }
            } else {
                pixel = false;
                const float fs = (float)A(&RenderArgs::spp);
                const rtm::f4 res{acc_r / fs, acc_g / fs, acc_b / fs, (float)min(sample, 1 << 24) / fs};
                const int frame_index = A(&RenderArgs::frame_index);
                const float lerp = frame_index > 0 ? 1.0f / (float)(frame_index + 1) : 1.0f;
                float4 prev;
                float4* out;
                float4* const out_shard = A(&RenderArgs::out_shard);
                const char* const last = A(&RenderArgs::last);
                if (out_shard) {
                    prev = last ? reinterpret_cast<const float4*>(last)[slot] : make_float4(0, 0, 0, 0);
                    out = out_shard + slot;
                } else {
                    const size_t at = (size_t)y * A(&RenderArgs::pitch) + (size_t)x * 16;
                    prev = last ? *reinterpret_cast<const float4*>(last + at) : make_float4(0, 0, 0, 0);
                    out = reinterpret_cast<float4*>(A(&RenderArgs::surface) + at);
                }
                const rtm::f4 o = rtm::mix4(rtm::f4{prev.x, prev.y, prev.z, prev.w}, res, lerp);
                *out = make_float4(o.x, o.y, o.z, 1.0f);
                rt_rng_state* rs = rng_slot();
                rs->d = rng.d;
                rs->v[0] = rng.v0;
                rs->v[1] = rng.v1;
                rs->v[2] = rng.v2;
                rs->v[3] = rng.v3;
                rs->v[4] = rng.v4;
                if (MODE & 8) {
                    uint32_t* const lane_cost = A(&RenderArgs::lane_cost);
                    if (lane_cost) lane_cost[slot] = c.lane_work + (uint32_t)c.seg;
                }
            }
        }
#ifdef RT_LIVE_HIST
        if (MODE & 8) {
            const unsigned long long tn = __builtin_amdgcn_s_memtime();
            if (lh_t) {
                const unsigned long long dt = tn - lh_t;
                c.ktest += lh_n <= 8u ? dt : 0ull;
                c.ktri += (lh_n > 8u && lh_n <= 16u) ? dt : 0ull;
                c.cy_tcl += (lh_n > 16u && lh_n <= 32u) ? dt : 0ull;
                c.cy_ttri += dt;
            }
            lh_t = tn;
            lh_n = (uint32_t)__popcll(__ballot(pixel || path));
        }
#endif
        if (!__ballot(path)) {
            if (drained) break;
            continue;
        }
        if (MODE & 8) c.w_iter++;
        if (STATS) {
            c.w_seg += (threadIdx.x & 63) == 0;
            c.l_seg += path;
        }

        rtfast::Hit h;
        h.best = 1e30f, h.kind = 0, h.id = 0, h.bx = h.by = 0.0f;
        const rtm::f3 nd = rtm::normalize(rd);
        if (path) {
            c.seg++;
            const int sphere_count = A(&RenderArgs::sphere_count);
            const GeometrySphere* const spheres = A(&RenderArgs::spheres);
            for (int i = 0; i < sphere_count; i++) {
                const GeometrySphere& sp = spheres[i];
                float dist;
                if (rtd::intersect_sphere(ro, nd, ld3(sp.position), sp.radius * sp.radius, &dist)) {
                    if (dist >= h.best) continue;
                    h.best = dist;
                    h.kind = 1;
                    h.id = (uint32_t)i;
                    if (STATS) c.sacc++;
                }
            }
        }
        rtfast::Ray R = rtfast::make_ray(ro, rd, nd, A(&RenderArgs::scene_fast) != 0);
        rtfast::trace<STATS, MODE>(nodes4, tris, a.pairs, a.tree, a.ltris, a.flat, a.spairs, a.tune, stk, scratch, R, h,
                                   path, c, a.quads, a.units, a.face_leaf);
        if (!path) continue;

        bool end = shade_segment<STATS, COLD>(a, h, ro, rd, nd, rng, color, thr, c);
        if (++bounce >= A(&RenderArgs::bounces)) end = true;
        if (end) {
            acc_r += color.x;
            acc_g += color.y;
            acc_b += color.z;
            sample++;
            path = false;
        }
    }

    if (unsigned long long* const seg_counter = A(&RenderArgs::seg_counter)) {
        unsigned long long v = c.seg;
        for (int off = 32; off > 0; off >>= 1) v += __shfl_xor(v, off);
        if ((threadIdx.x & 63) == 0) atomicAdd(seg_counter, v);
    }
    unsigned long long* const wave_clock = A(&RenderArgs::wave_clock);
    if (wave_clock && lane == 0) wave_clock[lb] = __builtin_amdgcn_s_memrealtime() - rt_start;
    unsigned long long* const stats = A(&RenderArgs::stats);
    unsigned long long lane_max = c.l_small;
    if (MODE & 8)
        for (int off = 32; off > 0; off >>= 1) {
            const unsigned long long o = __shfl_xor(lane_max, off);
            lane_max = o > lane_max ? o : lane_max;
        }
    unsigned long long lane_sum = c.l_small;
    unsigned long long big_sum[5] = {c.big_tests, c.tw_dec, c.tw_test, c.end2, c.redo};
    if ((MODE & 8) && stats)
        for (int off = 32; off > 0; off >>= 1) {
            lane_sum += __shfl_xor(lane_sum, off);
            for (int k = 0; k < 5; k++) big_sum[k] += __shfl_xor(big_sum[k], off);
        }
    if ((MODE & 8) && stats && lane == 0) {
        atomicAdd(stats + RT_STAT_CYCLES_SMALL, c.cy_small);
        atomicAdd(stats + RT_STAT_CYCLES_BIG, c.cy_big);
        atomicAdd(stats + RT_STAT_CYCLES_TOTAL, __builtin_amdgcn_s_memtime() - t_start);
        atomicAdd(stats + RT_STAT_ROUNDS_COOP, c.r_coop);
        atomicAdd(stats + RT_STAT_ROUNDS_SHARED, c.r_shared);
        atomicAdd(stats + RT_STAT_COOP_RAYS, c.coop_rays);
        atomicAdd(stats + RT_STAT_WAVE_SMALL_ITERS, c.w_small);
        atomicAdd(stats + RT_STAT_LANE_SMALL, lane_sum);
        atomicAdd(stats + RT_STAT_BIG_TESTS, big_sum[0]);
        atomicAdd(stats + RT_STAT_TWIN_DECIDED, big_sum[1]);
        atomicAdd(stats + RT_STAT_TWIN_TESTS, big_sum[2]);
        atomicAdd(stats + RT_STAT_WAVE_BIG_ITERS, c.big_iters);
        atomicAdd(stats + RT_STAT_DEFER_END2, big_sum[3]);
        atomicAdd(stats + RT_STAT_DEFER_REDO, big_sum[4]);
        atomicAdd(stats + RT_STAT_TREE_NODES, c.ktest);
        atomicAdd(stats + RT_STAT_TREE_TRI_TESTS, c.ktri);
        atomicAdd(stats + RT_STAT_WAVE_BIG_TRIS, c.w_big);
        atomicAdd(stats + RT_STAT_LANE_BIG_TRIS, c.l_big);
        atomicAdd(stats + RT_STAT_CYCLES_TREE_CLUSTERS, c.cy_tcl);
        atomicAdd(stats + RT_STAT_CYCLES_TREE_CUT, c.cy_tree);
        atomicAdd(stats + RT_STAT_CYCLES_TREE_TRIS, c.cy_ttri);
        if (wave_times) {
            unsigned long long* w = stats + RT_STAT_COUNT + 8 * (size_t)lb;
            w[0] = rt_start;
            w[1] = __builtin_amdgcn_s_memrealtime();
            w[2] = c.cy_small;
            w[3] = c.cy_big;
            w[4] = c.r_coop + c.r_shared;
            w[5] = c.w_iter;
            w[6] = c.w_small;
            w[7] = lane_max;
        }
    }
    if (STATS) {
        atomicAdd(stats + RT_STAT_SEGMENTS, c.seg);
        atomicAdd(stats + RT_STAT_NODES, c.node);
        atomicAdd(stats + RT_STAT_TRI_TESTS, c.tri);
        atomicAdd(stats + RT_STAT_TRI_ACCEPTS, c.tacc);
        atomicAdd(stats + RT_STAT_SPHERE_ACCEPTS, c.sacc);
        atomicAdd(stats + RT_STAT_HITS, c.hit);
        atomicAdd(stats + RT_STAT_MISSES, c.miss);
        atomicAdd(stats + RT_STAT_WAVE_SMALL_ITERS, c.w_small);
        atomicAdd(stats + RT_STAT_LANE_SMALL, c.l_small);
        atomicAdd(stats + RT_STAT_WAVE_BIG_TRIS, c.w_big);
        atomicAdd(stats + RT_STAT_LANE_BIG_TRIS, c.l_big);
        atomicAdd(stats + RT_STAT_CYCLES_TREE_CLUSTERS, c.cy_tcl);
        atomicAdd(stats + RT_STAT_CYCLES_TREE_CUT, c.cy_tree);
        atomicAdd(stats + RT_STAT_CYCLES_TREE_TRIS, c.cy_ttri);
        atomicAdd(stats + RT_STAT_WAVE_SEGMENT_ITERS, c.w_seg);
        atomicAdd(stats + RT_STAT_LANE_SEGMENTS, c.l_seg);
        atomicAdd(stats + RT_STAT_TREE_NODES, c.ktest);
        atomicAdd(stats + RT_STAT_TREE_TRI_TESTS, c.ktri);
    }
}

template <int STACK, bool STATS, int MODE>
__global__ __launch_bounds__(WAVE) void render_fast_kernel(RenderArgs a) {
    constexpr int SL = STACK < RT_LDS_SL ? STACK : RT_LDS_SL;
    __shared__ uint32_t stack_lds[(SL + rtfast::STACK_PAD_ROWS) * WAVE];
    __shared__ uint32_t scratch_lds[((MODE & 4) ? 64 : 0) + rtfast::DEFER_WORDS];
    uint32_t ovf[STACK > SL ? STACK - SL : 1];
    render_fast_body<STACK, STATS, MODE>(a, rtfast::Stack<SL>{stack_lds, ovf}, scratch_lds);
}
template <int STACK, bool STATS, int MODE>
__global__ __launch_bounds__(WAVE) __attribute__((amdgpu_waves_per_eu(5))) void render_fast_kernel_w5(RenderArgs a) {
    constexpr int SL = STACK < RT_LDS_SL ? STACK : RT_LDS_SL;
    __shared__ uint32_t stack_lds[(SL + rtfast::STACK_PAD_ROWS) * WAVE];
    __shared__ uint32_t scratch_lds[((MODE & 4) ? 64 : 0) + rtfast::DEFER_WORDS];
    uint32_t ovf[STACK > SL ? STACK - SL : 1];
    render_fast_body<STACK, STATS, MODE>(a, rtfast::Stack<SL>{stack_lds, ovf}, scratch_lds);
}
template <int STACK, bool STATS, int MODE>
__global__ __launch_bounds__(WAVE) __attribute__((amdgpu_waves_per_eu(6))) void render_fast_kernel_w6(RenderArgs a) {
    constexpr int SL = STACK < RT_LDS_SL ? STACK : RT_LDS_SL;
    __shared__ uint32_t stack_lds[(SL + rtfast::STACK_PAD_ROWS) * WAVE];
    __shared__ uint32_t scratch_lds[((MODE & 4) ? 64 : 0) + rtfast::DEFER_WORDS];
    uint32_t ovf[STACK > SL ? STACK - SL : 1];
    render_fast_body<STACK, STATS, MODE>(a, rtfast::Stack<SL>{stack_lds, ovf}, scratch_lds);
}
template <int STACK, bool STATS, int MODE>
__global__ __launch_bounds__(WAVE) __attribute__((amdgpu_waves_per_eu(7))) void render_fast_kernel_w7(RenderArgs a) {
    constexpr int SL = STACK < RT_LDS_SL ? STACK : RT_LDS_SL;
    __shared__ uint32_t stack_lds[(SL + rtfast::STACK_PAD_ROWS) * WAVE];
    __shared__ uint32_t scratch_lds[((MODE & 4) ? 64 : 0) + rtfast::DEFER_WORDS];
    uint32_t ovf[STACK > SL ? STACK - SL : 1];
    render_fast_body<STACK, STATS, MODE>(a, rtfast::Stack<SL>{stack_lds, ovf}, scratch_lds);
}

template <class K>
int resident_waves(K kernel) {
    static std::mutex mu;
    static std::map<std::pair<int, const void*>, int> cache;
    int dev = 0;
    if (hipGetDevice(&dev) != hipSuccess) return 0;
    std::lock_guard<std::mutex> lock(mu);
    const auto key = std::make_pair(dev, (const void*)kernel);
    auto it = cache.find(key);
    if (it != cache.end()) return it->second;
    hipFuncAttributes fa;
    int cus = 0;
    if (hipFuncGetAttributes(&fa, (const void*)kernel) != hipSuccess ||
        hipDeviceGetAttribute(&cus, hipDeviceAttributeMultiprocessorCount, dev) != hipSuccess)
        return 0;
    const int vgpr_waves = fa.numRegs > 0 ? std::min(8, 512 / ((fa.numRegs + 7) / 8 * 8)) : 8;
    const int lds_waves = fa.sharedSizeBytes > 0 ? (int)(160 * 1024 / fa.sharedSizeBytes) / 4 : 8;
    return cache[key] = std::max(1, std::min(vgpr_waves, lds_waves)) * 4 * std::max(cus, 1);
}

template <class K>
size_t cap_lds_bytes(K kernel, int cap) {
    if (cap < 1 || cap > 4) return 0;
    hipFuncAttributes fa;
    if (hipFuncGetAttributes(&fa, (const void*)kernel) != hipSuccess) return 0;
    const size_t per_wave = (size_t)(160 * 1024 / (4 * cap)) & ~(size_t)1023;
    return per_wave > fa.sharedSizeBytes ? per_wave - fa.sharedSizeBytes : 0;
}

template <class K>
// ... 44 lines not shown
```

### cuda-raytracing_amd/csrc/rt_kernel.hip

```cpp
#include <hip/hip_runtime.h>

#include <cstdio>
#include <cstdlib>
#include <vector>
#include <cstring>
#include <map>
#include <atomic>
#include <memory>
#include <mutex>
#include <stdexcept>
#include <string>
#include <thread>

#include "rt_abi.h"
#include "rt_device.h"
#include "rt_math.h"
#include "xorwow.h"
#include "rt_common.h"
#include "leaftree.h"
#include "rt_fast.h"

#include "mirror.h"

static_assert(MIRROR_BIG_LEAF == (uint32_t)rtfast::BIG, "pair records exist for exactly the big leaves");

static thread_local std::string g_last_error;

static int set_error(const std::string& msg, int code = 1) {
    g_last_error = msg;
    return code;
}
static int check(hipError_t e, const char* what) {
    if (e == hipSuccess) return 0;
    return set_error(std::string(what) + ": " + hipGetErrorString(e), (int)e);
}

extern "C" const char* rt_last_error(void) { return g_last_error.c_str(); }

static size_t bytes_from(const void* p) {
    hipDeviceptr_t base = nullptr;
    size_t size = 0;
    if (!p || hipMemGetAddressRange(&base, &size, (hipDeviceptr_t)p) != hipSuccess) return 0;
    return size - (size_t)((const char*)p - (const char*)base);
}

void rt_internal_set_error(const char* msg) { set_error(msg); }

extern "C" int rt_set_device(int device) { return check(hipSetDevice(device), "hipSetDevice"); }
extern "C" int rt_device_count(void) {
    int n = 0;
    return hipGetDeviceCount(&n) == hipSuccess ? n : 0;
}
extern "C" int rt_malloc(void** ptr, size_t bytes) { return check(hipMalloc(ptr, bytes), "hipMalloc"); }
extern "C" int rt_malloc_pitch(void** ptr, size_t* pitch, size_t width_bytes, size_t height) {
    return check(hipMallocPitch(ptr, pitch, width_bytes, height), "hipMallocPitch");
}
extern "C" int rt_free(void* ptr) { return check(hipFree(ptr), "hipFree"); }
extern "C" int rt_memcpy_h2d(void* dst, const void* src, size_t n) {
    return check(hipMemcpy(dst, src, n, hipMemcpyHostToDevice), "hipMemcpy H2D");
}
extern "C" int rt_memcpy_d2h(void* dst, const void* src, size_t n) {
    return check(hipMemcpy(dst, src, n, hipMemcpyDeviceToHost), "hipMemcpy D2H");
}
extern "C" int rt_memcpy_d2d(void* dst, const void* src, size_t n) {
    return check(hipMemcpy(dst, src, n, hipMemcpyDeviceToDevice), "hipMemcpy D2D");
}
extern "C" int rt_memset(void* dst, int value, size_t n) { return check(hipMemset(dst, value, n), "hipMemset"); }
extern "C" int rt_synchronize(void) { return check(hipDeviceSynchronize(), "hipDeviceSynchronize"); }

static std::mutex g_cube_mutex;
static std::map<uint64_t, int> g_cube_size;

extern "C" uint64_t rt_cubemap_create(const float* rgba, int size) {
    if (!rgba || size <= 0) {
        set_error("rt_cubemap_create: bad arguments");
        return 0;
    }
    void* p = nullptr;
    const size_t bytes = (size_t)6 * size * size * 16;
    if (rt_malloc(&p, bytes) || rt_memcpy_h2d(p, rgba, bytes)) return 0;
    std::lock_guard<std::mutex> lock(g_cube_mutex);
    g_cube_size[(uint64_t)p] = size;
    return (uint64_t)p;
}

extern "C" int rt_cubemap_destroy(uint64_t handle) {
    {
        std::lock_guard<std::mutex> lock(g_cube_mutex);
        if (!g_cube_size.erase(handle)) return set_error("rt_cubemap_destroy: unknown handle");
    }
    return rt_free((void*)handle);
}

static int cube_size(uint64_t handle) {
    std::lock_guard<std::mutex> lock(g_cube_mutex);
    auto it = g_cube_size.find(handle);
    return it == g_cube_size.end() ? -1 : it->second;
}

#include "rt_render.h"

namespace {

using namespace rtk;

__global__ __launch_bounds__(BLOCK) void init_rng_kernel(rt_rng_state* states, const uint32_t* __restrict__ jump,
                                                         uint32_t seed, int64_t count, int width, int height,
                                                         int shard_index, int shard_count, int tiles_x,
                                                         const int32_t* __restrict__ tile_list) {
    const int64_t s = (int64_t)blockIdx.x * blockDim.x + threadIdx.x;
    if (s >= count) return;
    uint64_t sub;
    if (shard_count <= 0) {
        sub = (uint64_t)s;
    } else {
        const int64_t k = s / BLOCK;
        const int tile = tile_list ? tile_list[k] : shard_index + (int)k * shard_count;
        if (tile < 0 || tile >= tiles_x * ((height + TILE - 1) / TILE)) return;
        int lx, ly;
        tile_pixel((int)(s % BLOCK), &lx, &ly);
        const int x = (tile % tiles_x) * TILE + lx, y = (tile / tiles_x) * TILE + ly;
        if (x >= width || y >= height) return;
        sub = (uint64_t)y * (uint64_t)width + (uint64_t)x;
    }
    uint32_t st[6];
    rt_xorwow_seed(seed, st);
    uint32_t v[5] = {st[1], st[2], st[3], st[4], st[5]};
    for (int k = 0; sub && k < RT_XORWOW_JUMPS; k++, sub >>= 2) {
        const uint32_t reps = (uint32_t)(sub & 3u);
        const uint32_t* m = jump + (size_t)k * 800;
        for (uint32_t r = 0; r < reps; r++) {
            uint32_t o[5] = {0, 0, 0, 0, 0};
            for (int i = 0; i < 5; i++) {
                const uint32_t word = v[i];
                for (int j = 0; j < 32; j++) {
                    const uint32_t mask = 0u - ((word >> j) & 1u);
                    const uint32_t* row = m + i * 160 + j * 5;
                    o[0] ^= row[0] & mask;
                    o[1] ^= row[1] & mask;
                    o[2] ^= row[2] & mask;
                    o[3] ^= row[3] & mask;
                    o[4] ^= row[4] & mask;
                }
            }
            for (int w = 0; w < 5; w++) v[w] = o[w];
        }
    }
    rt_rng_state* out = states + s;
    out->d = st[0];
    for (int i = 0; i < 5; i++) out->v[i] = v[i];
    for (int i = 0; i < 6; i++) out->unused[i] = 0;
}

__global__ __launch_bounds__(BLOCK) void unshard_kernel(char* surface, uint64_t pitch, int width, int height,
                                                        int shard_count, const float4* shards, int64_t per_shard,
                                                        int tiles_x, const int32_t* __restrict__ tile_lists) {
    const int rank = blockIdx.y;
    const int64_t k = blockIdx.x;
    const int tile = tile_lists ? tile_lists[(size_t)rank * per_shard + k] : rank + (int)k * shard_count;
    int lx, ly;
    tile_pixel(threadIdx.x, &lx, &ly);
    const int x = (tile % tiles_x) * TILE + lx, y = (tile / tiles_x) * TILE + ly;
    if (tile < 0 || tile >= tiles_x * ((height + TILE - 1) / TILE) || x >= width || y >= height) return;
    const float4 v = shards[((size_t)rank * per_shard + k) * BLOCK + threadIdx.x];
    *reinterpret_cast<float4*>(surface + (size_t)y * pitch + (size_t)x * 16) = v;
}

const uint32_t* device_jump_table() {
    static std::mutex mu;
    static std::map<int, uint32_t*> per_device;
    int dev = 0;
    if (hipGetDevice(&dev) != hipSuccess) return nullptr;
    std::lock_guard<std::mutex> lock(mu);
    auto it = per_device.find(dev);
    if (it != per_device.end()) return it->second;
    uint32_t* d = nullptr;
    const size_t bytes = (size_t)RT_XORWOW_JUMPS * 800 * 4;
    if (hipMalloc(&d, bytes) != hipSuccess) return nullptr;
    if (hipMemcpy(d, rt_xorwow_jump_table(), bytes, hipMemcpyHostToDevice) != hipSuccess) return nullptr;
    per_device[dev] = d;
    return d;
}

std::atomic<const ExperimentalKernels*> g_experimental{nullptr};

bool needs_experimental(const rt_render_params* p, bool has_tree, bool screens) {
    const bool stats = (p->flags & RT_RENDER_STATS) != 0;
    if ((p->flags & RT_RENDER_TRACER_WAVEFRONT) || p->refill_lanes || p->lone_count > 0) return true;
    if (screens && (p->tune & 4096u) == 0 && (!stats || (p->tune & 256u))) return true;
    if (stats || p->lane_cost) return false;
    const uint32_t mode = (p->tune >> 4) & 3u;
    return (p->tune & 4096u) != 0 || (!has_tree && (mode == 2u || mode == 3u));
}

constexpr uint32_t kKernelTuneBits = 1u | (1u << 11) | (7u << 13) | (15u << 16) | (7u << 21) | (1u << 24) | (1u << 26) |
                                     (1u << 30) | (1u << 31);

int lean_mode(const RenderArgs& a, int mode) {
    if ((mode & 4) || (a.tune & kKernelTuneBits)) return mode;
    const bool have = a.nodes && a.tris && a.spairs && a.pairs && a.quads && a.units;
    return have ? mode | rtfast::LEAN_BIT : mode;
}

hipError_t launch_prod(int stack, int mode, const RenderArgs& a, int waves, hipStream_t s) {
    const int m = lean_mode(a, mode);
    return (m & rtfast::LEAN_BIT) ? launch_fast_lean(stack, m, a, waves, s) : launch_fast_prod(stack, m, a, waves, s);
}

hipError_t launch_fast(const RenderArgs& args, int waves, int depth, bool stats, hipStream_t s) {
    const int stack = (depth >= 0 && depth + 2 <= 30) ? 30 : (depth >= 0 && depth + 2 <= 40) ? 40 : 64;
    const ExperimentalKernels* x = g_experimental.load();
    const bool scr = args.screens != 0 && (args.tune & 4096u) == 0;
    if (stats && (args.tune & 256u)) {
        if (scr) return x ? x->fast_screen(stack, args.tree ? 61 : 57, args, waves, s) : hipErrorNotSupported;
        if (!args.tree && (args.tune & 4096u)) return launch_fast_timing(stack, 9, args, waves, s);
        return launch_fast_timing(stack, lean_mode(args, args.tree ? 29 : 25), args, waves, s);
    }
    if (!stats && args.lane_cost) {
        if (scr) return x ? x->fast_screen(stack, args.tree ? 61 : 57, args, waves, s) : hipErrorNotSupported;
        return launch_fast_timing(stack, lean_mode(args, args.tree ? 29 : 25), args, waves, s);
    }
    if (stats) return launch_fast_stats(stack, (args.tree && (args.tune & 128u)) ? 6 : 2, args, waves, s);
    const bool split = (args.tune & 4096u) == 0;
    if (args.queue_head) return x ? x->fast_refill(stack, args.tree ? 85 : 81, args, waves, s) : hipErrorNotSupported;
    if (scr && split && (args.tree || ((args.tune >> 4) & 3u) < 2u))
        return x ? x->fast_screen(stack, args.tree ? 53 : 49, args, waves, s) : hipErrorNotSupported;
    if (args.tree) {
        if (split) return launch_prod(stack, 21, args, waves, s);
        return x ? x->fast_ab(stack, 5, args, waves, s) : hipErrorNotSupported;
    }
    const uint32_t mode = (args.tune >> 4) & 3u;
    if (split && mode < 2) return launch_prod(stack, 17, args, waves, s);
    if (!x) return hipErrorNotSupported;
    if (mode == 2) return x->fast_ab(stack, 2, args, waves, s);
    if (mode == 3) return x->fast_ab(stack, 0, args, waves, s);
    return x->fast_ab(stack, 1, args, waves, s);
}

}

void rtk::register_experimental_kernels(const rtk::ExperimentalKernels* k, uint32_t abi) {
    if (k && abi != rtk::kExperimentalAbi) {
        char msg[160];
        std::snprintf(msg, sizeof msg, "librt_hip_exp.so refused: its ABI stamp 0x%08x is not librt_hip.so's 0x%08x "
                      "(rebuild both)", abi, rtk::kExperimentalAbi);
        set_error(msg);
        return;
    }
    g_experimental.store(k);
}
const rtk::ExperimentalKernels* rtk::experimental_kernels() { return g_experimental.load(); }

namespace {
struct LoneStreams {
    hipStream_t side = nullptr;
    hipEvent_t fork = nullptr, join = nullptr;
};
LoneStreams* lone_streams(hipStream_t s) {
    static std::mutex mu;
    static std::map<std::pair<int, hipStream_t>, LoneStreams> all;
    int dev = 0;
    if (hipGetDevice(&dev) != hipSuccess) return nullptr;
    std::lock_guard<std::mutex> lock(mu);
    LoneStreams& l = all[std::make_pair(dev, s)];
    if (!l.side && (hipStreamCreateWithFlags(&l.side, hipStreamNonBlocking) != hipSuccess ||
                    hipEventCreateWithFlags(&l.fork, hipEventDisableTiming) != hipSuccess ||
                    hipEventCreateWithFlags(&l.join, hipEventDisableTiming) != hipSuccess)) {
        l = LoneStreams{};
        return nullptr;
    }
    return &l;
}

unsigned long long* queue_counter(hipStream_t s) {
    static std::mutex mu;
    static std::map<std::pair<int, hipStream_t>, unsigned long long*> counters;
    int dev = 0;
    if (hipGetDevice(&dev) != hipSuccess) return nullptr;
    std::lock_guard<std::mutex> lock(mu);
    auto& c = counters[std::make_pair(dev, s)];
    if (!c && hipMalloc(&c, sizeof(unsigned long long)) != hipSuccess) c = nullptr;
    return c;
}

int tiles_of_shard(int width, int height, int shard_index, int shard_count) {
    const int tiles = ((width + TILE - 1) / TILE) * ((height + TILE - 1) / TILE);
    if (shard_index >= tiles) return 0;
    return (tiles - shard_index + shard_count - 1) / shard_count;
}

void sky_quat(float* w, float* x, float* y, float* z) {
    const float ex = 0.0f, ey = 3.1415926536f, ez = 0.0f;
    const float cx = rtm::rt_cosf(ex * 0.5f), cy = rtm::rt_cosf(ey * 0.5f), cz = rtm::rt_cosf(ez * 0.5f);
    const float sx = rtm::rt_sinf(ex * 0.5f), sy = rtm::rt_sinf(ey * 0.5f), sz = rtm::rt_sinf(ez * 0.5f);
    *w = cx * cy * cz + sx * sy * sz;
    *x = sx * cy * cz - cx * sy * sz;
    *y = cx * sy * cz + sx * cy * sz;
    *z = cx * cy * sz - sx * sy * cz;
}

}

extern "C" int64_t rt_shard_tiles(int width, int height, int shard_index, int shard_count) {
    if (width <= 0 || height <= 0 || shard_count <= 0 || shard_index < 0 || shard_index >= shard_count) return 0;
    return tiles_of_shard(width, height, shard_index, shard_count);
}

__device__ __forceinline__ unsigned long long mix64(unsigned long long x) {
    x ^= x >> 30;
    x *= 0xbf58476d1ce4e5b9ull;
    x ^= x >> 27;
    x *= 0x94d049bb133111ebull;
    x ^= x >> 31;
    return x;
}

struct HashArrays {
    const uint32_t* w[4];
    unsigned long long n[4];
};

__global__ __launch_bounds__(BLOCK) void fingerprint_kernel(HashArrays h, unsigned long long* out) {
    unsigned long long acc = 0;
    const unsigned long long stride = (unsigned long long)gridDim.x * BLOCK;
    for (int k = 0; k < 4; k++) {
        for (unsigned long long i = (unsigned long long)blockIdx.x * BLOCK + threadIdx.x; i < h.n[k]; i += stride)
            acc += mix64(((unsigned long long)k << 60) ^ (i << 32) ^ h.w[k][i]);
    }
    __shared__ unsigned long long part[BLOCK / 64];
    for (int off = 32; off > 0; off >>= 1) acc += __shfl_xor(acc, off);
    if ((threadIdx.x & 63) == 0) part[threadIdx.x >> 6] = acc;
    __syncthreads();
    if (threadIdx.x == 0) {
        unsigned long long t = 0;
        for (int w = 0; w < BLOCK / 64; w++) t += part[w];
        atomicAdd(out, t);
    }
}

__global__ void fingerprint_gate_kernel(unsigned long long* acc, unsigned long long salt, unsigned long long expected,
                                        int have, int* flag, unsigned long long* out) {
    const unsigned long long fp = *acc ^ salt;
    *flag = (have && fp == expected) ? 1 : 0;
    *out = fp;
    *acc = 0;
}

static uint64_t host_fingerprint(const std::vector<const uint32_t*>& w, const std::vector<size_t>& n, uint64_t salt) {
    auto mix = [](unsigned long long x) {
        x ^= x >> 30;
        x *= 0xbf58476d1ce4e5b9ull;
        x ^= x >> 27;
        x *= 0x94d049bb133111ebull;
        x ^= x >> 31;
        return x;
    };
    unsigned long long acc = 0;
    for (int k = 0; k < 4; k++)
        for (size_t i = 0; i < n[k]; i++) acc += mix(((unsigned long long)k << 60) ^ ((unsigned long long)i << 32) ^ w[k][i]);
    return acc ^ salt;
}

namespace {
// ... 255 lines not shown
}

extern "C" int rt_render(const rt_render_params* p, const GPUScene* scene, void* stream) {
    if (!p || !scene) return set_error("rt_render: null argument");
    if (p->width <= 0 || p->height <= 0 || p->spp <= 0 || p->bounces < 0)
        return set_error("rt_render: bad frame size / spp / bounces");
    if (p->shard_count <= 0 || p->shard_index < 0 || p->shard_index >= p->shard_count)
        return set_error("rt_render: bad shard");
    if (!p->out_shard && (!p->surface || p->pitch < (uint64_t)p->width * 16))
        return set_error("rt_render: need a surface with pitch >= 16*width, or out_shard");
    if (p->shard_count > 1 && !p->out_shard) return set_error("rt_render: sharded render needs out_shard");
    if (!scene->rng_state || !scene->gpu_bvh_nodes || !scene->gpu_materials)
        return set_error("rt_render: scene not uploaded (rng_state / bvh / materials missing)");
    if ((p->flags & RT_RENDER_STATS) && !p->stats) return set_error("rt_render: stats flag without buffer");

    RenderArgs a;
    std::memset(&a, 0, sizeof(a));
    a.spheres = scene->gpu_spheres;
    a.materials = scene->gpu_materials;
    a.nodes = scene->gpu_bvh_nodes;
    a.face_indices = scene->gpu_bvh_face_indices;
    a.vertices = scene->gpu_vertices;
    a.faces = scene->gpu_faces;
    a.rng = (rt_rng_state*)scene->rng_state;
    a.sphere_count = scene->sphere_count;
    a.cam = scene->camera;
    if (scene->environment_cubemap_tex) {
        const int n = cube_size(scene->environment_cubemap_tex);
        if (n <= 0) return set_error("rt_render: unknown environment cube map handle");
        a.sky = (const float*)scene->environment_cubemap_tex;
        a.sky_n = n;
    }
    sky_quat(&a.qw, &a.qx, &a.qy, &a.qz);
    a.surface = (char*)p->surface;
    a.last = (const char*)p->surface_last_frame;
    a.out_shard = (float4*)p->out_shard;
    a.pitch = p->pitch;
    a.width = p->width, a.height = p->height;
    a.frame_index = p->frame_index, a.spp = p->spp, a.bounces = p->bounces;
    a.shard_index = p->shard_index, a.shard_count = p->shard_count;
    a.tiles_x = (p->width + TILE - 1) / TILE;
    a.stats = (unsigned long long*)p->stats;
    a.seg_counter = (unsigned long long*)p->segment_counter;

    if (p->tile_list && (p->tile_count <= 0 || p->tile_count > (int64_t)1 << 28))
        return set_error("rt_render: tile_list needs 0 < tile_count < 2^28");
    if (p->tile_list && !p->out_shard && p->shard_count > 1) return set_error("rt_render: sharded render needs out_shard");
    a.tile_list = p->tile_list;
    a.wave_clock = (unsigned long long*)p->wave_clock;
    const int tiles = p->tile_list ? (int)p->tile_count : tiles_of_shard(p->width, p->height, p->shard_index, p->shard_count);
    if (tiles == 0) return 0;
    if (p->lane_slots && (p->lane_slot_count <= 0 || p->lane_slot_count % WAVE != 0 || p->lane_slot_count > (int64_t)1 << 30))
        return set_error("rt_render: lane_slots needs a positive multiple of 64 entries (< 2^30)");
    a.lane_slots = p->lane_slots;
    a.slot_count = (long long)tiles * TILE * TILE;
    if (a.slot_count > (1LL << 32)) return set_error("rt_render: more than 2^32 pixel slots in one launch");
    a.lane_cost = p->lane_cost;
    a.priority_waves = p->lane_slots ? (int)std::min<int64_t>(std::max<int64_t>(p->priority_waves, 0), 1 << 30) : 0;
    const int waves = p->lane_slots ? (int)(p->lane_slot_count / WAVE) : tiles * 4;
    a.entry_count = (long long)waves * WAVE;
    if (p->refill_lanes < 0 || p->refill_lanes > 64) return set_error("rt_render: refill_lanes must be in [0, 64]");
    if (p->waves_per_simd < 0 || p->waves_per_simd > 7)
        return set_error("rt_render: waves_per_simd must be 0 (default), 1-4 (LDS-capped residency), 5, 6 or 7");
    if (((p->tune >> 9) & 3u) == 1u)
        return set_error("rt_render: RT_TUNE occupancy override 1 (compiler's choice) is not built");
    a.waves_per_simd = p->waves_per_simd;
    a.refill_lanes = p->refill_lanes;
    {
        const bool compact = p->out_shard != nullptr;
        const size_t slots = (size_t)tiles * TILE * TILE;
        const size_t frame = (size_t)p->pitch * (size_t)(p->height - 1) + (size_t)p->width * 16;
        const size_t rng_need = (compact ? slots : (size_t)p->width * p->height) * sizeof(rt_rng_state);
        if (bytes_from(scene->rng_state) < rng_need) return set_error("rt_render: rng_state is smaller than the frame / shard");
        if (compact && bytes_from(p->out_shard) < slots * 16) return set_error("rt_render: out_shard too small");
        if (compact && p->surface_last_frame && bytes_from(p->surface_last_frame) < slots * 16)
            return set_error("rt_render: surface_last_frame (shard) too small");
        if (!compact && bytes_from(p->surface) < frame) return set_error("rt_render: surface too small");
        if (!compact && p->surface_last_frame && bytes_from(p->surface_last_frame) < frame)
            return set_error("rt_render: surface_last_frame too small");
        if (p->tile_list && bytes_from(p->tile_list) < (size_t)tiles * 4) return set_error("rt_render: tile_list too small");
        if (p->wave_clock && bytes_from(p->wave_clock) < (size_t)waves * 8)
            return set_error("rt_render: wave_clock too small");
        if (p->lane_slots && bytes_from(p->lane_slots) < (size_t)p->lane_slot_count * 4)
            return set_error("rt_render: lane_slots too small");
        if (p->lane_cost && bytes_from(p->lane_cost) < slots * 4) return set_error("rt_render: lane_cost too small");
        const size_t stats_need = (RT_STAT_COUNT + ((p->tune & 2048u) ? (size_t)waves * 8 : 0)) * 8;
        if (p->stats && bytes_from(p->stats) < stats_need) return set_error("rt_render: stats too small");
    }
    const bool want_ref = (p->flags & RT_RENDER_TRACER_REF) != 0;
    MirrorDevice mir;
    int* gate = nullptr;
    bool foreign_fast = false;
    if ((!rt_internal_lookup_mirror(scene, &mir) || !mir.owned) && !want_ref) {
        if (foreign_frame(scene, (hipStream_t)stream, &mir, &foreign_fast, &gate) != 0) return 1;
        if (!foreign_fast) gate = nullptr, mir = MirrorDevice{};
    }
    const void* tris = mir.tris;
    const int depth = mir.depth;
    const bool scene_fast = mir.fast;
    a.tune = p->tune;
    a.pairs = (a.tune & 2u) ? nullptr : (const float4*)mir.pairs;
    a.quads = (a.tune & ((1u << 20) | 2u)) ? nullptr : (const float4*)mir.quads;
    a.units = (const float4*)mir.units;
    a.tree = (a.tune & 4u) ? nullptr : (const float4*)mir.tree;
    a.ltris = (const float4*)mir.ltris;
    a.spairs = (a.tune & 8u) ? nullptr : (const float4*)mir.spairs;
    a.flat = (const float4*)mir.flat;
    a.face_leaf = (const uint32_t*)mir.face_leaf;
    a.tris = want_ref ? nullptr : (const FlatTri*)tris;
    const bool stats = (p->flags & RT_RENDER_STATS) != 0;
    hipStream_t s = (hipStream_t)stream;
    const bool want_flat = (p->flags & RT_RENDER_TRACER_FLAT) != 0;
    if ((p->lane_slots || p->lane_cost || p->refill_lanes) && (gate || !a.tris || want_flat))
        return set_error("rt_render: lane_slots / lane_cost / refill_lanes need the production tracer on an rt_scene_upload scene");
    if (p->lane_cost && p->refill_lanes) return set_error("rt_render: lane_cost probes run without refill");
    const bool want_wf = (p->flags & RT_RENDER_TRACER_WAVEFRONT) != 0;
    if (want_wf && (gate || !a.tris || want_flat || stats || p->lane_cost || p->refill_lanes || p->wave_clock ||
                    p->lone_count))
        return set_error("rt_render: the wavefront tracer needs an rt_scene_upload scene and no statistics / lane_cost / "
                         "wave_clock / refill / lone frames");
    if (want_wf && (p->spp > 65535 || p->bounces > 255 || (int64_t)p->spp * p->bounces > 65536))
        return set_error("rt_render: the wavefront tracer needs spp <= 65535, bounces <= 255, spp x bounces <= 65536");
    a.screens = (mir.screens > 0 && (a.tune & (1u << 28)) == 0 && a.tris && !(p->flags & RT_RENDER_TRACER_FLAT)) ? 1 : 0;
    if (!g_experimental.load() && needs_experimental(p, a.tree != nullptr, a.screens != 0))
        return set_error("rt_render: this frame asks for an experimental render path (wavefront tracer, refill, lone-pixel "
                         "kernel or an RT_TUNE A/B variant), which lives in librt_hip_exp.so -- load it first "
                         "(rt.load_experimental())");
    const bool lone = p->lone_count > 0;
    if (p->lone_count < 0 || p->lone_count > (int64_t)1 << 28 || (lone && !p->lone_slots))
        return set_error("rt_render: lone_count must be in [0, 2^28] with lone_slots");
    if (lone && (!p->lane_slots || gate || !a.tris || want_flat || stats || p->lane_cost || p->refill_lanes))
        return set_error("rt_render: lone_slots need lane_slots and the production tracer on an rt_scene_upload scene "
                         "(no statistics / lane_cost / refill frames)");
    if (lone && (!mir.treelets || depth < 0 || depth > 75))
        return set_error("rt_render: lone_slots need the scene's treelets (a BVH of depth <= 75 with an inner root)");
    if (lone && bytes_from(p->lone_slots) < (size_t)p->lone_count * 4) return set_error("rt_render: lone_slots too small");
    if ((p->flags & RT_RENDER_VALIDATE) && lone && validate_lone(p->lone_slots, p->lone_count, p->lane_slots,
                                                                  p->lane_slot_count, a.slot_count, s) != 0)
        return 1;
    if (p->refill_lanes) {
        a.queue_head = queue_counter(s);
        if (!a.queue_head) return set_error("rt_render: cannot allocate the refill queue counter");
        if (check(hipMemsetAsync(a.queue_head, 0, sizeof(unsigned long long), s), "hipMemsetAsync") != 0) return 1;
    }
    a.scene_fast = scene_fast ? 1 : 0;
    const GPUBVHNode* const trav_nodes =
        (mir.nodes && (a.tune & (1u << 27)) == 0) ? (const GPUBVHNode*)mir.nodes : scene->gpu_bvh_nodes;
    auto trav = [&](const RenderArgs& x) {
        RenderArgs f = x;
        f.nodes = trav_nodes;
        if (trav_nodes != (const GPUBVHNode*)mir.nodes) f.face_leaf = nullptr;
        return f;
    };
    hipError_t e;
    if (gate) {
        a.gate = gate, a.gate_value = 1;
        e = want_flat ? launch_ref_tracer(true, a, tiles * 4, depth, stats, s) : launch_fast(trav(a), waves, depth, stats, s);
        if (e == hipSuccess) {
            RenderArgs r = a;
            r.tris = nullptr, r.gate_value = 0;
            e = launch_ref_tracer(false, r, tiles * 4, -1, stats, s);
        }
    } else if (!a.tris)
        e = launch_ref_tracer(false, a, tiles * 4, depth, stats, s);
    else if (want_flat)
        e = launch_ref_tracer(true, a, tiles * 4, depth, stats, s);
    else if (want_wf)
        e = g_experimental.load()->wavefront(trav(a), depth, s);
    else if (lone) {
        LoneStreams* ls = lone_streams(s);
        if (!ls) return set_error("rt_render: cannot create the lone-pixel stream");
        if (check(hipEventRecord(ls->fork, s), "hipEventRecord") || check(hipStreamWaitEvent(ls->side, ls->fork, 0), "hipStreamWaitEvent"))
            return 1;
        e = g_experimental.load()->lone(a, p->lone_slots, (int)p->lone_count, mir.treelets, ls->side);
        if (e == hipSuccess) e = launch_fast(trav(a), waves, depth, stats, s);
        if (check(hipEventRecord(ls->join, ls->side), "hipEventRecord") || check(hipStreamWaitEvent(s, ls->join, 0), "hipStreamWaitEvent"))
            return 1;
    } else
        e = launch_fast(trav(a), waves, depth, stats, s);
    return check(e, "render_kernel launch");
}

extern "C" int rt_trace_rays(const rt_trace_params* p, const GPUScene* scene, void* stream) {
    if (!p) return set_error("rt_trace_rays: null params");
    if (!scene) return set_error("rt_trace_rays: null scene");
    if (!p->hits) return set_error("rt_trace_rays: null hits");
    if (p->flags != 0) return set_error("rt_trace_rays: flags must be 0");
    if (p->waves_per_simd != 0 && (p->waves_per_simd < 5 || p->waves_per_simd > 7))
        return set_error("rt_trace_rays: waves_per_simd must be 0 (default), 5, 6 or 7");
    const bool camera = p->rays == nullptr;
    if (camera && (p->width <= 0 || p->height <= 0)) return set_error("rt_trace_rays: camera mode needs width, height > 0");
    const int64_t count = camera ? (int64_t)p->width * p->height : p->count;
    if (count < 0) return set_error("rt_trace_rays: negative count");
    if (count > (int64_t)1 << 31) return set_error("rt_trace_rays: more than 2^31 rays in one call");
    if ((((uintptr_t)p->rays) | ((uintptr_t)p->hits)) & 15u) return set_error("rt_trace_rays: rays and hits must be 16-byte aligned");
    if (count == 0) return 0;

    MirrorDevice mir;
    if (!rt_internal_lookup_mirror(scene, &mir) || !mir.owned)
        return set_error("rt_trace_rays: this GPUScene was not uploaded by rt_scene_upload (a foreign scene has no private "
                         "mirror to query; foreign scenes are not supported here)");
    if (!mir.nodes || !mir.tris) return set_error("rt_trace_rays: the scene's mirror has no triangles to traverse");
    if (scene->sphere_count > 0 && !scene->gpu_spheres) return set_error("rt_trace_rays: sphere_count without spheres");
    if (!camera && bytes_from(p->rays) < (size_t)count * sizeof(rt_ray)) return set_error("rt_trace_rays: rays too small");
    if (bytes_from(p->hits) < (size_t)count * sizeof(rt_hit)) return set_error("rt_trace_rays: hits too small");

    QueryArgs q;
    std::memset(&q, 0, sizeof(q));
    q.rays = p->rays;
    q.hits = p->hits;
    q.count = count;
    q.width = camera ? p->width : 1, q.height = camera ? p->height : 1;
    q.cam = scene->camera;
    q.spheres = scene->gpu_spheres;
    q.sphere_count = scene->sphere_count;
    q.scene_fast = mir.fast ? 1 : 0;
    q.faces = scene->gpu_faces;
    q.vertices = scene->gpu_vertices;
    q.nodes = (const GPUBVHNode*)mir.nodes;
    q.tris = (const FlatTri*)mir.tris;
    q.pairs = (const float4*)mir.pairs, q.quads = (const float4*)mir.quads, q.units = (const float4*)mir.units;
    q.tree = (const float4*)mir.tree, q.ltris = (const float4*)mir.ltris, q.spairs = (const float4*)mir.spairs;
    q.flat = (const float4*)mir.flat;
    q.face_leaf = (const uint32_t*)mir.face_leaf;
    const int depth = mir.depth;
    const int stack = (depth >= 0 && depth + 2 <= 30) ? 30 : (depth >= 0 && depth + 2 <= 40) ? 40 : 64;
    int mode = q.tree ? 21 : 17;
    if (mode == 17 && q.spairs && q.pairs && q.quads && q.units) mode |= rtfast::LEAN_BIT;
    const int w = p->waves_per_simd ? p->waves_per_simd : (mode == 21 ? 5 : 7);
    return check(launch_query(stack, mode, w, q, (hipStream_t)stream), "query_kernel launch");
}

extern "C" int rt_experimental_loaded() { return rtk::experimental_kernels() ? 1 : 0; }

extern "C" int rt_init_rng(void* states, int width, int height, int shard_index, int shard_count, uint32_t seed,
                           void* stream) {
    if (!states || width <= 0 || height <= 0 || shard_count <= 0 || shard_index < 0 || shard_index >= shard_count)
        return set_error("rt_init_rng: bad arguments");
    const uint32_t* jump = device_jump_table();
    if (!jump) return set_error("rt_init_rng: jump table upload failed");
    const int tiles_x = (width + TILE - 1) / TILE;
    int64_t count;
    int sc;
    if (shard_count == 1) {
        count = (int64_t)width * height;
        sc = 0;
    } else {
        count = (int64_t)tiles_of_shard(width, height, shard_index, shard_count) * BLOCK;
        sc = shard_count;
    }
    if (count == 0) return 0;
    if (bytes_from(states) < (size_t)count * sizeof(rt_rng_state)) return set_error("rt_init_rng: rng_states too small");
    const int blocks = (int)((count + BLOCK - 1) / BLOCK);
    hipLaunchKernelGGL(init_rng_kernel, dim3(blocks), dim3(BLOCK), 0, (hipStream_t)stream, (rt_rng_state*)states, jump,
                       seed, count, width, height, shard_index, sc, tiles_x, (const int32_t*)nullptr);
    return check(hipGetLastError(), "init_rng_kernel launch");
}

extern "C" int rt_init_rng_tiles(void* states, int width, int height, const int32_t* tile_list, int64_t tile_count,
                                 uint32_t seed, void* stream) {
    if (!states || !tile_list || width <= 0 || height <= 0 || tile_count <= 0 || tile_count > ((int64_t)1 << 28))
        return set_error("rt_init_rng_tiles: bad arguments");
    const uint32_t* jump = device_jump_table();
    if (!jump) return set_error("rt_init_rng_tiles: jump table upload failed");
    const int64_t count = tile_count * BLOCK;
    if (bytes_from(states) < (size_t)count * sizeof(rt_rng_state) || bytes_from(tile_list) < (size_t)tile_count * 4)
        return set_error("rt_init_rng_tiles: rng_states or tile_list too small");
    hipLaunchKernelGGL(init_rng_kernel, dim3((unsigned)tile_count), dim3(BLOCK), 0, (hipStream_t)stream,
                       (rt_rng_state*)states, jump, seed, count, width, height, 0, 1, (width + TILE - 1) / TILE,
                       tile_list);
    return check(hipGetLastError(), "init_rng_kernel launch");
}

extern "C" int rt_unshard(void* surface, uint64_t pitch, int width, int height, int shard_count, const void* shards,
                          int64_t per_shard, void* stream) {
    if (!surface || !shards || shard_count <= 0 || per_shard <= 0 || width <= 0 || height <= 0)
        return set_error("rt_unshard: bad arguments");
    if (bytes_from(shards) < (size_t)shard_count * per_shard * BLOCK * 16 ||
        bytes_from(surface) < pitch * (size_t)(height - 1) + (size_t)width * 16)
        return set_error("rt_unshard: shards or surface too small");
    const int tiles_x = (width + TILE - 1) / TILE;
    hipLaunchKernelGGL(unshard_kernel, dim3((unsigned)per_shard, shard_count), dim3(BLOCK), 0, (hipStream_t)stream,
                       (char*)surface, pitch, width, height, shard_count, (const float4*)shards, per_shard, tiles_x,
                       (const int32_t*)nullptr);
    return check(hipGetLastError(), "unshard_kernel launch");
}

extern "C" int rt_unshard_tiles(void* surface, uint64_t pitch, int width, int height, int shard_count,
                                const void* shards, int64_t per_shard, const int32_t* tile_lists, void* stream) {
    if (!surface || !shards || !tile_lists || shard_count <= 0 || per_shard <= 0 || width <= 0 || height <= 0)
        return set_error("rt_unshard_tiles: bad arguments");
    if (bytes_from(shards) < (size_t)shard_count * per_shard * BLOCK * 16 ||
        bytes_from(tile_lists) < (size_t)shard_count * per_shard * 4 ||
        bytes_from(surface) < pitch * (size_t)(height - 1) + (size_t)width * 16)
        return set_error("rt_unshard_tiles: shards, tile_lists or surface too small");
    hipLaunchKernelGGL(unshard_kernel, dim3((unsigned)per_shard, shard_count), dim3(BLOCK), 0, (hipStream_t)stream,
                       (char*)surface, pitch, width, height, shard_count, (const float4*)shards, per_shard,
                       (width + TILE - 1) / TILE, tile_lists);
    return check(hipGetLastError(), "unshard_kernel launch");
}

extern "C" void raytracing_process(void* surface, void* surface_last_frame, int width, int height, size_t pitch,
                                   int frame_index, GPUScene* scene) {
    rt_render_params p;
    std::memset(&p, 0, sizeof(p));
    p.surface = surface;
    p.surface_last_frame = surface_last_frame;
    p.width = width, p.height = height, p.pitch = pitch;
    p.frame_index = frame_index;
    p.spp = 5;
    p.bounces = 6;
    p.shard_index = 0, p.shard_count = 1;
    if (rt_render(&p, scene, nullptr) != 0)
        std::printf("(raytracing_kernel_main) failed to launch error = %s\n", rt_last_error());
}

extern "C" void init_rng(uint32_t thread_block_count, uint32_t thread_block_size, void* states, unsigned int seed) {
    const uint32_t* jump = device_jump_table();
    const int64_t count = (int64_t)thread_block_count * thread_block_size;
    if (bytes_from(states) < (size_t)count * sizeof(rt_rng_state)) {
        set_error("init_rng: rngStates is smaller than thread_block_count * thread_block_size states");
        std::printf("(init_rng) failed: %s\n", rt_last_error());
        return;
    }
    if (!jump || count == 0) {
        set_error("init_rng: jump table upload failed");
        std::printf("(init_rng) failed: %s\n", rt_last_error());
        return;
    }
    hipLaunchKernelGGL(init_rng_kernel, dim3(thread_block_count), dim3(thread_block_size), 0, nullptr,
                       (rt_rng_state*)states, jump, seed, count, 0, 0, 0, 0, 0, (const int32_t*)nullptr);
    if (check(hipGetLastError(), "init_rng_kernel launch")) std::printf("(init_rng) failed: %s\n", rt_last_error());
}


// ... 41 lines not shown
```

### include/rt_abi.h

```cpp
#ifndef RT_ABI_H
#define RT_ABI_H

#include <stddef.h>
#include <stdint.h>

#ifdef __cplusplus
extern "C" {
#endif

#if defined(__cplusplus)
#define RT_ALIGNAS(n) alignas(n)
#else
#define RT_ALIGNAS(n) _Alignas(n)
#endif


typedef struct GPUCamera {
    float origin[3];
    float viewport_worldspace_size[2];
    float aspect;
    float horizontal[3];
    float vertical[3];
    float lower_left_corner[3];
} GPUCamera;
// ... 162 lines not shown
    uint32_t material;
    float normal[3];
    float bx;
    float position[3];
    float by;
} rt_hit;

typedef struct rt_trace_params {
    const rt_ray* rays;
    int64_t count;
    int32_t width, height;
    rt_hit* hits;
    uint32_t flags;
    int32_t waves_per_simd;
} rt_trace_params;

#if defined(__cplusplus)
static_assert(sizeof(rt_ray) == 32 && offsetof(rt_ray, tmax) == 12 && offsetof(rt_ray, direction) == 16 &&
              offsetof(rt_ray, reserved) == 28, "rt_ray");
static_assert(sizeof(rt_hit) == 48 && offsetof(rt_hit, kind) == 4 && offsetof(rt_hit, id) == 8 &&
              offsetof(rt_hit, material) == 12 && offsetof(rt_hit, normal) == 16 && offsetof(rt_hit, bx) == 28 &&
              offsetof(rt_hit, position) == 32 && offsetof(rt_hit, by) == 44, "rt_hit");
static_assert(sizeof(rt_trace_params) == 40 && offsetof(rt_trace_params, hits) == 24 &&
              offsetof(rt_trace_params, flags) == 32, "rt_trace_params");
#endif

int rt_trace_rays(const rt_trace_params* params, const GPUScene* scene, void* stream);

#define RT_DENOISE_DEFAULT (-1)
#define RT_DENOISE_MAX_HEIGHT 131072
#define RT_DENOISE_MAX_PIXELS 1073741824

typedef struct rt_denoise_params {
    const void* surface;
    uint64_t pitch;
    int32_t width, height;
    const rt_hit* hits;
    const GPUMaterial* materials;
    int32_t material_count;
    int32_t flags;
    void* out;
    uint64_t out_pitch;
    void* scratch;
    uint64_t scratch_bytes;
    int32_t iterations;
    int32_t normal_power_log2;
    float sigma_plane;
    float sigma_color;
} rt_denoise_params;

#if defined(__cplusplus)
static_assert(sizeof(rt_denoise_params) == 96 &&offsetof(rt_denoise_params, pitch) == 8 &&
              offsetof(rt_denoise_params, width) == 16 && offsetof(rt_denoise_params, hits) == 24 &&
              offsetof(rt_denoise_params, materials) == 32 && offsetof(rt_denoise_params, material_count) == 40 &&
              offsetof(rt_denoise_params, flags) == 44 && offsetof(rt_denoise_params, out) == 48 &&
              offsetof(rt_denoise_params, out_pitch) == 56 && offsetof(rt_denoise_params, scratch) == 64 &&
              offsetof(rt_denoise_params, scratch_bytes) == 72 && offsetof(rt_denoise_params, iterations) == 80 &&
              offsetof(rt_denoise_params, normal_power_log2) == 84 && offsetof(rt_denoise_params, sigma_plane) == 88 &&
              offsetof(rt_denoise_params, sigma_color) == 92,
              "rt_denoise_params");
#endif

size_t rt_denoise_scratch_bytes(int width, int height);
int rt_denoise(const rt_denoise_params* params, void* stream);

int rt_init_rng(void* rng_states, int width, int height, int shard_index, int shard_count, uint32_t seed,
                void* stream);

int64_t rt_shard_tiles(int width, int height, int shard_index, int shard_count);

int rt_unshard(void* surface, uint64_t pitch, int width, int height, int shard_count, const void* shards,
               int64_t tiles_per_shard_max, void* stream);

int64_t rt_shard_plan_capacity(int width, int height, int shard_count);
int rt_shard_plan(int width, int height, int shard_count, const double* tile_cost, int64_t capacity,
                  int32_t* tile_lists, int64_t* counts);
int64_t rt_lane_plan_capacity(int64_t slots);
int64_t rt_lane_plan(const uint32_t* cost, int64_t slots, double parallel_units, double slack,
                     int32_t* lane_slots, int64_t capacity, int64_t* long_waves);
int64_t rt_lane_refine(const int32_t* lane_slots, int64_t entries, const uint32_t* cost, int64_t slots,
                       const int64_t* wave_ticks, double theta, int32_t* out, int64_t capacity, int64_t* split_waves);
int64_t rt_lone_plan(uint32_t* cost, int64_t slots, int64_t max_lone, uint32_t min_cost, int32_t* lone_slots);
int rt_init_rng_tiles(void* rng_states, int width, int height, const int32_t* tile_list, int64_t tile_count,
                      uint32_t seed, void* stream);
int rt_unshard_tiles(void* surface, uint64_t pitch, int width, int height, int shard_count, const void* shards,
                     int64_t tiles_per_shard_max, const int32_t* tile_lists, void* stream);

#define RT_COMM_ID_BYTES 128
typedef struct rt_comm rt_comm;
int rt_comm_unique_id(uint8_t id[RT_COMM_ID_BYTES]);
int rt_comm_init_rank(rt_comm** comm, int nranks, int rank, const uint8_t id[RT_COMM_ID_BYTES]);
int rt_comm_init_all(rt_comm** comms, int ndev, const int* devices);
int rt_comm_destroy(rt_comm* comm);
int rt_comm_rank(const rt_comm* comm);
int rt_comm_size(const rt_comm* comm);
int rt_comm_group_start(void);
int rt_comm_group_end(void);
int rt_gather_shards(rt_comm* comm, const void* shard, size_t shard_bytes, void* gathered, size_t stride,
                     const size_t* recv_bytes, int root, void* stream);

int rt_tonemap_srgb8(const void* surface, uint64_t pitch, int width, int height, uint8_t* out_rgb, void* stream);
int rt_write_pfm(const char* path, const float* rgba, uint64_t pitch, int width, int height);
int rt_write_ppm(const char* path, const uint8_t* rgb, int width, int height);

int rt_set_device(int device);
int rt_device_count(void);
int rt_malloc(void** ptr, size_t bytes);
int rt_malloc_pitch(void** ptr, size_t* pitch, size_t width_bytes, size_t height);
int rt_free(void* ptr);
int rt_memcpy_h2d(void* dst, const void* src, size_t bytes);
int rt_memcpy_d2h(void* dst, const void* src, size_t bytes);
int rt_memcpy_d2d(void* dst, const void* src, size_t bytes);
int rt_memset(void* dst, int value, size_t bytes);
int rt_synchronize(void);
const char* rt_last_error(void);

uint64_t rt_cubemap_create(const float* rgba_level0, int size);
int rt_cubemap_destroy(uint64_t handle);

typedef struct rt_scene rt_scene;

rt_scene* rt_scene_create(void);
void rt_scene_destroy(rt_scene* scene);
uint32_t rt_scene_add_material(rt_scene* scene, const GPUMaterial* material);
void rt_scene_add_triangle(rt_scene* scene, const float a[3], const float b[3], const float c[3], int material);
void rt_scene_add_quad(rt_scene* scene, const float a[3], const float b[3], const float c[3], const float d[3],
                       int material);
void rt_scene_add_sphere(rt_scene* scene, const float position[3], float radius, int material);
int rt_scene_add_mesh_file(rt_scene* scene, const char* path, const float transform[16], int material);
int rt_scene_set_environment_file(rt_scene* scene, const char* path);
int rt_scene_environment(const rt_scene* scene, const float** texels, int* size);
void rt_scene_set_camera(rt_scene* scene, const float position[3], float angle_x_deg, float angle_y_deg);
void rt_scene_set_viewport(rt_scene* scene, int width, int height);
int rt_scene_upload(rt_scene* scene, void* rng_state);
const GPUScene* rt_scene_gpu(const rt_scene* scene);
void rt_scene_build(rt_scene* scene);
void rt_scene_camera(const rt_scene* scene, GPUCamera* out);
int rt_scene_setup(rt_scene* scene, int which, const char* assets_dir);
int rt_scene_setup_plane(rt_scene* scene, int n, const char* assets_dir);
size_t rt_scene_host_arrays(const rt_scene* scene, const GPUBVHNode** nodes, size_t* node_count,
                            const uint32_t** face_indices, size_t* face_count, const GPUVertex** vertices,
                            size_t* vertex_count, const GPUFace** faces);
int rt_scene_bvh_max_depth(const rt_scene* scene);
int rt_scene_materials(rt_scene* scene, void* out, size_t* count);

typedef struct rt_build_options {
    uint32_t leaf_tree_min;
    uint32_t cut_clusters;
    uint32_t cluster_max;
    float split_angle;
    uint32_t bvh_small;
    int32_t host_bvh;
    int32_t leaf_screens;
} rt_build_options;
void rt_get_build_options(rt_build_options* out);
int rt_set_build_options(const rt_build_options* options);

int rt_bvh_build_device(const GPUVertex* vertices, uint32_t vertex_count, const GPUFace* faces, uint32_t face_count,
                        GPUBVHNode* nodes_out, uint32_t* face_indices_out, uint32_t* node_count_out,
                        int* max_depth_out, void* stream);

int rt_scene_mirror_info(rt_scene* scene, size_t* tri_records, size_t* tree_nodes, size_t* tree_tri_records);
int rt_scene_mirror_copy(rt_scene* scene, float* tris, float* tree, float* tree_tris);
int rt_cluster_cull_host(const float origin[3], const float nd[3], float best, const float node[16]);
int rt_twin_check_host(const float rec[12], const float origin[3], const float nd[3]);
int rt_scene_mirror_nodes(rt_scene* scene, GPUBVHNode* nodes, size_t* count);
int rt_scene_mirror_twins(rt_scene* scene, float* quads, size_t* quad_count, float* units, size_t* unit_count);
int rt_scene_mirror_face_leaf(rt_scene* scene, uint32_t* leaf, size_t* count);

int rt_mirror_build_check(const GPUBVHNode* nodes, size_t node_count, const uint32_t* face_indices, size_t index_count,
                          const GPUFace* faces, size_t face_count, const GPUVertex* vertices, size_t vertex_count,
                          uint32_t* meta, int* twins);

int rt_xorwow_jump_matrix(int k, uint32_t out[800]);
void rt_xorwow_init_host(uint32_t seed, uint64_t subsequence, rt_rng_state* out);

#ifdef __cplusplus
}
#endif

#endif
```

Baseline: 2345.

## Seed primary-ray traversal from per-8x8-tile BVH entry frontiers

Adds a per-tile entry table, built on the GPU and cached per camera and BVH generation. For each 8x8 pixel tile it conservatively culls BVH nodes against the tile's view frustum, keeping up to 15 surviving subtrees. Lean fast kernels start primary-ray traversal from this frontier instead of the root, skipping upper-level node tests. This costs a small table-build kernel, a deeper stack reservation and extra gating logic. It is enabled only when the build option entry_frontier is set.

```diff
diff --git a/cuda-raytracing_amd/__init__.py b/cuda-raytracing_amd/__init__.py
--- a/cuda-raytracing_amd/__init__.py
+++ b/cuda-raytracing_amd/__init__.py
@@ -51,7 +51,7 @@
 class BuildOptions(ctypes.Structure):
     _fields_ = [("leaf_tree_min", ctypes.c_uint32), ("cut_clusters", ctypes.c_uint32), ("cluster_max", ctypes.c_uint32),
                 ("split_angle", ctypes.c_float), ("bvh_small", ctypes.c_uint32), ("host_bvh", ctypes.c_int32),
-                ("leaf_screens", ctypes.c_int32)]
+                ("leaf_screens", ctypes.c_int32), ("entry_frontier", ctypes.c_int32)]
 
 
 class RenderParams(ctypes.Structure):
@@ -116,6 +116,7 @@
     "rt_unshard": (_I, [_P, _U64, _I, _I, _I, _P, ctypes.c_int64, _P]),
     "rt_shard_plan_capacity": (ctypes.c_int64, [_I, _I, _I]),
     "rt_shard_plan": (_I, [_I, _I, _I, _P, ctypes.c_int64, _P, _P]),
+    "rt_entry_table_builds": (_U64, []),
     "rt_get_build_options": (None, [_P]),
     "rt_set_build_options": (_I, [_P]),
     "rt_lane_plan_capacity": (ctypes.c_int64, [ctypes.c_int64]),
@@ -387,6 +388,10 @@
     return meta, bool(tw.value)
 
 
+def entry_table_builds():
+    return int(lib().rt_entry_table_builds())
+
+
 def bvh_build_device(vertices, faces, stream=None):
     import torch
     nf = faces.shape[0]
diff --git a/cuda-raytracing_amd/build.py b/cuda-raytracing_amd/build.py
--- a/cuda-raytracing_amd/build.py
+++ b/cuda-raytracing_amd/build.py
@@ -198,6 +198,21 @@
     return HOST_DRIVER
 
 
+ENTRY_HOST_SRC = os.path.join(CSRC, "entry_host.cpp")
+ENTRY_HOST_LIB = os.path.join(PKG, "librt_entry_host.so")
+
+
+def build_entry_host(force=False):
+    deps = [ENTRY_HOST_SRC, LIB] + _deps(CSRC, (".h",)) + _deps(INC, (".h",))
+    if not force and _newer(ENTRY_HOST_LIB, deps):
+        return ENTRY_HOST_LIB
+    tmp = ENTRY_HOST_LIB + ".tmp"
+    _run(["g++", "-O2", "-std=c++17", "-fPIC", "-shared", *FP_FLAGS, "-I", INC, "-I", CSRC, ENTRY_HOST_SRC, "-L", PKG,
+          "-l:librt_hip.so", "-Wl,-rpath,$ORIGIN", "-o", tmp])
+    os.replace(tmp, ENTRY_HOST_LIB)
+    return ENTRY_HOST_LIB
+
+
 def build_oracle(force=False):
     src = os.path.join(ORACLE_DIR, "rt_oracle.c")
     deps = [src, os.path.abspath(__file__)] + _deps(ORACLE_DIR, (".h",))
@@ -220,6 +235,7 @@
 
 def build_all(force=False):
     build_product(force)
+    build_entry_host(force)
     build_oracle(force)
     build_reference_parts(force)
     build_host_driver(force)
diff --git a/cuda-raytracing_amd/csrc/entry_frontier.h b/cuda-raytracing_amd/csrc/entry_frontier.h
--- /dev/null
+++ b/cuda-raytracing_amd/csrc/entry_frontier.h
@@ -0,0 +1,226 @@
+#pragma once
+
+#include <cmath>
+#include <cstdint>
+#include <cstring>
+
+#if defined(__HIPCC__)
+#define EF_HD __host__ __device__ inline
+#else
+#define EF_HD inline
+#endif
+
+#ifndef RT_EF_K
+#define RT_EF_K 15
+#endif
+#ifndef RT_EF_TILE
+#define RT_EF_TILE 8
+#endif
+constexpr int EF_K = RT_EF_K;
+constexpr int EF_TILE = RT_EF_TILE;
+constexpr int EF_WORDS = (EF_K + 16) / 16 * 16;
+constexpr int EF_MAX_PASSES = 64;
+
+struct EfCamera {
+    float origin[3], lower_left[3], horizontal[3], vertical[3];
+};
+
+struct EfTile {
+    double n[5][3];
+    bool use[5];
+    double o[3];
+    bool ok;
+};
+
+EF_HD bool ef_in_range_or_zero(float v) {
+    const float a = fabsf(v);
+    return v == 0.0f || (a >= 0x1p-60f && a <= 0x1p62f);
+}
+
+EF_HD bool ef_camera_ok(const EfCamera& c, int width, int height) {
+    if (width <= 0 || height <= 0 || width > (1 << 20) || height > (1 << 20)) return false;
+    for (int i = 0; i < 3; i++) {
+        if (!ef_in_range_or_zero(c.origin[i])) return false;
+        if (!(fabsf(c.lower_left[i]) < 0x1p60f && fabsf(c.horizontal[i]) < 0x1p60f && fabsf(c.vertical[i]) < 0x1p60f)) return false;
+    }
+    return true;
+}
+
+EF_HD int ef_tiles_x(int width) { return (width + EF_TILE - 1) / EF_TILE; }
+EF_HD int ef_tiles_y(int height) { return (height + EF_TILE - 1) / EF_TILE; }
+
+EF_HD void ef_tile_setup(const EfCamera& c, int width, int height, int tx, int ty, EfTile* T) {
+    T->ok = ef_camera_ok(c, width, height);
+    for (int i = 0; i < 3; i++) T->o[i] = c.origin[i];
+    for (int k = 0; k < 5; k++) T->use[k] = false;
+    if (!T->ok) return;
+    const int x0 = tx * EF_TILE, y0 = ty * EF_TILE;
+    const int x1 = x0 + EF_TILE < width ? x0 + EF_TILE : width, y1 = y0 + EF_TILE < height ? y0 + EF_TILE : height;
+    const double ulo = (double)x0 / width * (1.0 - 0x1p-22), uhi = (double)x1 / width * (1.0 + 0x1p-22);
+    const double vlo = (double)y0 / height * (1.0 - 0x1p-22), vhi = (double)y1 / height * (1.0 + 0x1p-22);
+    const double du = (uhi - ulo) * (1.0 / 64), dv = (vhi - vlo) * (1.0 / 64);
+    double E[3], cr[4][3], g[4][3];
+    const double us[4] = {ulo, uhi, uhi, ulo}, vs[4] = {vlo, vlo, vhi, vhi};
+    const double gu[4] = {ulo - du, uhi + du, uhi + du, ulo - du}, gv[4] = {vlo - dv, vlo - dv, vhi + dv, vhi + dv};
+    for (int i = 0; i < 3; i++) {
+        const double ll = c.lower_left[i], h = c.horizontal[i], v = c.vertical[i], o = c.origin[i];
+        E[i] = 0x1p-21 * (fabs(ll) + fabs(h) * uhi + fabs(v) * vhi + fabs(o)) + 0x1p-100;
+        for (int k = 0; k < 4; k++) {
+            cr[k][i] = ((ll + h * us[k]) + v * vs[k]) - o;
+            g[k][i] = ((ll + h * gu[k]) + v * gv[k]) - o;
+        }
+    }
+    for (int k = 0; k < 5; k++) {
+        double* n = T->n[k];
+        if (k < 4) {
+            const double* a = g[k];
+            const double* b = g[(k + 1) & 3];
+            n[0] = a[1] * b[2] - a[2] * b[1], n[1] = a[2] * b[0] - a[0] * b[2], n[2] = a[0] * b[1] - a[1] * b[0];
+            const double* op = g[(k + 2) & 3];
+            if (n[0] * op[0] + n[1] * op[1] + n[2] * op[2] < 0.0) n[0] = -n[0], n[1] = -n[1], n[2] = -n[2];
+        } else {
+            for (int i = 0; i < 3; i++) n[i] = (g[0][i] + g[1][i]) + (g[2][i] + g[3][i]);
+        }
+        bool good = true;
+        for (int j = 0; j < 4 && good; j++) {
+            double dot = 0.0, mag = 0.0, err = 0.0;
+            for (int i = 0; i < 3; i++) {
+                dot += n[i] * cr[j][i];
+                mag += fabs(n[i]) * fabs(cr[j][i]);
+                err += fabs(n[i]) * E[i];
+            }
+            good = (dot - err * (1.0 + 0x1p-30) - 0x1p-40 * mag >= 0.0) && mag < 0x1p900;
+        }
+        T->use[k] = good;
+    }
+}
+
+EF_HD bool ef_box_missed(const EfTile& T, const float* lo, const float* hi) {
+    if (!T.ok) return false;
+    double a[3], b[3];
+    for (int i = 0; i < 3; i++) {
+        const double l = (double)lo[i] - T.o[i], h = (double)hi[i] - T.o[i];
+        a[i] = l - 0x1p-21 * fabs(l);
+        b[i] = h + 0x1p-21 * fabs(h);
+    }
+    for (int k = 0; k < 5; k++) {
+        if (!T.use[k]) continue;
+        double top = 0.0, mag = 0.0;
+        for (int i = 0; i < 3; i++) {
+            const double pa = T.n[k][i] * a[i], pb = T.n[k][i] * b[i];
+            top += pa > pb ? pa : pb;
+            mag += fabs(pa) > fabs(pb) ? fabs(pa) : fabs(pb);
+        }
+        if (top + 0x1p-40 * mag < 0.0) return true;
+    }
+    return false;
+}
+
+EF_HD uint32_t ef_bits(float f) {
+    union { float f; uint32_t u; } v;
+    v.f = f;
+    return v.u;
+}
+EF_HD bool ef_finite3(const float* p) { return fabsf(p[0]) < INFINITY && fabsf(p[1]) < INFINITY && fabsf(p[2]) < INFINITY; }
+
+EF_HD bool ef_contains_children(const float* nodes, uint32_t p, uint32_t left) {
+    const float* P = nodes + 8 * (size_t)p;
+    if (!ef_finite3(P) || !ef_finite3(P + 3)) return false;
+    for (uint32_t c = left; c < left + 2; c++) {
+        const float* C = nodes + 8 * (size_t)c;
+        if (!ef_finite3(C) || !ef_finite3(C + 3)) return false;
+        for (int i = 0; i < 3; i++)
+            if (!(C[i] >= P[i] && C[3 + i] <= P[3 + i] && C[i] <= C[3 + i])) return false;
+    }
+    return true;
+}
+
+EF_HD bool ef_on_face_plane(const float* N, const float* origin) {
+    for (int i = 0; i < 3; i++)
+        if (N[i] == origin[i] || N[3 + i] == origin[i]) return true;
+    return false;
+}
+
+EF_HD void ef_build_record(const float* nodes, uint32_t node_count, const EfCamera& cam, int width, int height, int tx,
+                           int ty, uint32_t* rec, uint32_t* dropped = nullptr, int dropped_cap = 0,
+                           int* dropped_n = nullptr) {
+    EfTile T;
+    ef_tile_setup(cam, width, height, tx, ty, &T);
+    uint32_t list[EF_K];
+    int n = 1, nd = 0;
+    list[0] = 0;
+    bool fallback = !T.ok || node_count == 0;
+    for (int pass = 0; pass < EF_MAX_PASSES && !fallback; pass++) {
+        bool changed = false;
+        for (int i = 0; i < n && !fallback; i++) {
+            const uint32_t p = list[i];
+            const float* P = nodes + 8 * (size_t)p;
+            if (ef_bits(P[7]) != 0) continue;
+            const uint32_t left = ef_bits(P[6]);
+            if (left >= node_count || left + 1 >= node_count || left == 0) {
+                fallback = true;
+                break;
+            }
+            if (!ef_contains_children(nodes, p, left)) continue;
+            const float* L = nodes + 8 * (size_t)left;
+            const float* R = L + 8;
+            if (ef_on_face_plane(P, cam.origin) || ef_on_face_plane(L, cam.origin) || ef_on_face_plane(R, cam.origin)) {
+                fallback = true;
+                break;
+            }
+            const bool kr = !ef_box_missed(T, R, R + 3), kl = !ef_box_missed(T, L, L + 3);
+            if (kr && kl) {
+                if (n == EF_K) continue;
+                for (int j = n; j > i + 1; j--) list[j] = list[j - 1];
+                list[i] = left + 1, list[i + 1] = left;
+                n++;
+                i++;
+            } else if (kr || kl) {
+                list[i] = kr ? left + 1 : left;
+                if (dropped && nd < dropped_cap) dropped[nd] = kr ? left : left + 1;
+                nd++;
+            } else {
+                if (dropped && nd < dropped_cap) dropped[nd] = left + 1;
+                if (dropped && nd + 1 < dropped_cap) dropped[nd + 1] = left;
+                nd += 2;
+                for (int j = i; j + 1 < n; j++) list[j] = list[j + 1];
+                n--;
+                i--;
+            }
+            changed = true;
+        }
+        if (!changed) break;
+    }
+    if (fallback) {
+        n = 1, nd = 0;
+        list[0] = 0;
+    }
+    rec[0] = (uint32_t)n;
+    for (int i = 0; i < EF_K; i++) rec[1 + i] = i < n ? list[i] : 0u;
+    if (dropped_n) *dropped_n = nd;
+}
+
+EF_HD bool ef_ray_ok(const float* o, const float* d) {
+    for (int i = 0; i < 3; i++) {
+        if (!(fabsf(d[i]) >= 0x1p-40f && fabsf(d[i]) <= 0x1p20f)) return false;
+        if (!ef_in_range_or_zero(o[i])) return false;
+    }
+    return true;
+}
+
+struct EfKey {
+    EfCamera cam;
+    int width, height;
+    const void* nodes;
+    uint64_t generation;
+    int k;
+};
+inline EfKey ef_make_key(const EfCamera& cam, int width, int height, const void* nodes, uint64_t generation) {
+    EfKey key{};
+    key.cam = cam, key.width = width, key.height = height, key.nodes = nodes, key.generation = generation, key.k = EF_K;
+    return key;
+}
+inline bool ef_key_same(const EfKey& a, const EfKey& b) {
+    return memcmp(&a.cam, &b.cam, sizeof(EfCamera)) == 0 && a.width == b.width && a.height == b.height && a.nodes == b.nodes &&
+           a.generation == b.generation && a.k == b.k;
+}
diff --git a/cuda-raytracing_amd/csrc/entry_host.cpp b/cuda-raytracing_amd/csrc/entry_host.cpp
--- /dev/null
+++ b/cuda-raytracing_amd/csrc/entry_host.cpp
@@ -0,0 +1,219 @@
+#include "entry_frontier.h"
+
+#include <cstring>
+#include <exception>
+#include <stdexcept>
+#include <vector>
+
+#include "entry_host.h"
+#include "mirror.h"
+
+struct rt_entry_host {
+    EfKey key{};
+    bool valid = false;
+    uint64_t builds = 0;
+    MirrorHost mirror;
+    const void* mirror_of = nullptr;
+    size_t mirror_nodes = 0;
+    uint64_t generation = 0;
+    std::vector<uint32_t> records;
+    std::vector<std::vector<uint32_t>> dropped;
+};
+namespace {
+constexpr int kDroppedCap = 4096;
+
+EfCamera ef_camera(const GPUCamera& c) {
+    EfCamera e;
+    for (int i = 0; i < 3; i++) {
+        e.origin[i] = c.origin[i], e.lower_left[i] = c.lower_left_corner[i];
+        e.horizontal[i] = c.horizontal[i], e.vertical[i] = c.vertical[i];
+    }
+    return e;
+}
+
+bool aabb_hit(const float* o, const float* d, const float* n, float len) {
+    const float tx1 = (n[0] - o[0]) / d[0], tx2 = (n[3] - o[0]) / d[0];
+    float tmin = fminf(tx1, tx2), tmax = fmaxf(tx1, tx2);
+    const float ty1 = (n[1] - o[1]) / d[1], ty2 = (n[4] - o[1]) / d[1];
+    tmin = fmaxf(tmin, fminf(ty1, ty2)), tmax = fminf(tmax, fmaxf(ty1, ty2));
+    const float tz1 = (n[2] - o[2]) / d[2], tz2 = (n[5] - o[2]) / d[2];
+    tmin = fmaxf(tmin, fminf(tz1, tz2)), tmax = fminf(tmax, fmaxf(tz1, tz2));
+    return tmax >= tmin && tmin < len && tmax > 0;
+}
+
+struct V3 {
+    float x, y, z;
+};
+V3 cross(V3 a, V3 b) { return V3{a.y * b.z - b.y * a.z, a.z * b.x - b.z * a.x, a.x * b.y - b.x * a.y}; }
+float dot(V3 a, V3 b) { return (a.x * b.x + a.y * b.y) + a.z * b.z; }
+
+bool tri_hit(V3 o, V3 d, const float* r, float* dist) {
+    const float eps = 1.1920928955078125e-07f;
+    const V3 a{r[0], r[1], r[2]}, e1{r[3], r[4], r[5]}, e2{r[6], r[7], r[8]};
+    const V3 p = cross(d, e2);
+    const float det = dot(e1, p);
+    const V3 t{o.x - a.x, o.y - a.y, o.z - a.z};
+    V3 q;
+    if (det > eps) {
+        const float u = dot(t, p);
+        if (u < 0.0f || u > det) return false;
+        q = cross(t, e1);
+        const float v = dot(d, q);
+        if (v < 0.0f || u + v > det) return false;
+    } else if (det < -eps) {
+        const float u = dot(t, p);
+        if (u > 0.0f || u < det) return false;
+        q = cross(t, e1);
+        const float v = dot(d, q);
+        if (v > 0.0f || u + v < det) return false;
+    } else {
+        return false;
+    }
+    *dist = dot(e2, q) * (1.0f / det);
+    return true;
+}
+
+void walk(const MirrorHost& m, const float* o, const float* d, std::vector<uint32_t> stack, uint32_t* face, float* best,
+          uint32_t* visits, uint32_t* depth) {
+    std::vector<char> held;
+    uint32_t nheld = 0;
+    for (uint32_t i : stack) {
+        held.push_back(aabb_hit(o, d, &m.nodes[8 * (size_t)i], INFINITY));
+        nheld += held.back();
+    }
+    *depth = nheld;
+    const float len = sqrtf((d[0] * d[0] + d[1] * d[1]) + d[2] * d[2]);
+    const V3 nd{d[0] / len, d[1] / len, d[2] / len}, ro{o[0], o[1], o[2]};
+    *face = 0xffffffffu, *best = 1e30f, *visits = 0;
+    while (!stack.empty()) {
+        const uint32_t i = stack.back();
+        stack.pop_back();
+        nheld -= held.back();
+        held.pop_back();
+        const float* n = &m.nodes[8 * (size_t)i];
+        ++*visits;
+        if (!aabb_hit(o, d, n, *best)) continue;
+        uint32_t first, count;
+        std::memcpy(&first, n + 6, 4), std::memcpy(&count, n + 7, 4);
+        if (count > 0) {
+            for (uint32_t k = first; k < first + count; k++) {
+                float dist;
+                if (tri_hit(ro, nd, &m.tris[12 * (size_t)k], &dist)) {
+                    if (dist >= *best || dist < 0.0f) continue;
+                    *best = dist;
+                    std::memcpy(face, &m.tris[12 * (size_t)k + 9], 4);
+                }
+            }
+        } else {
+            stack.push_back(first);
+            stack.push_back(first + 1);
+            held.push_back(aabb_hit(o, d, &m.nodes[8 * (size_t)first], INFINITY));
+            nheld += held.back();
+            if (nheld > *depth) *depth = nheld;
+            held.push_back(0);
+        }
+    }
+}
+}
+
+extern "C" rt_entry_host* rt_entry_host_create(void) { return new rt_entry_host(); }
+extern "C" void rt_entry_host_destroy(rt_entry_host* t) { delete t; }
+
+extern "C" int rt_entry_host_update(rt_entry_host* t, const GPUBVHNode* nodes, size_t node_count, const uint32_t* face_indices,
+                                    size_t index_count, const GPUFace* faces, size_t face_count, const GPUVertex* vertices,
+                                    size_t vertex_count, const GPUCamera* cam, int width, int height) {
+    if (!t || !nodes || !cam || width <= 0 || height <= 0) {
+        rt_internal_set_error("rt_entry_host_update: bad argument");
+        return -1;
+    }
+    try {
+        if (t->mirror_of != nodes || t->mirror_nodes != node_count) {
+            t->mirror = MirrorHost{};
+            rt_build_mirror(nodes, node_count, face_indices, index_count, faces, face_count, vertices, vertex_count, &t->mirror);
+            t->mirror_of = nodes, t->mirror_nodes = node_count;
+            t->generation++;
+        }
+        const EfKey now = ef_make_key(ef_camera(*cam), width, height, nodes, t->generation);
+        if (t->valid && ef_key_same(t->key, now)) return 0;
+        const int tx = ef_tiles_x(width), ty = ef_tiles_y(height);
+        t->records.assign((size_t)tx * ty * EF_WORDS, 0u);
+        t->dropped.assign((size_t)tx * ty, std::vector<uint32_t>());
+        std::vector<uint32_t> out(kDroppedCap);
+        const uint32_t nn = (uint32_t)(t->mirror.nodes.size() / 8);
+        for (int y = 0; y < ty; y++)
+            for (int x = 0; x < tx; x++) {
+                const size_t i = (size_t)y * tx + x;
+                if (t->mirror.fast) {
+                    int nd = 0;
+                    ef_build_record(t->mirror.nodes.data(), nn, now.cam, width, height, x, y, &t->records[i * EF_WORDS],
+                                    out.data(), kDroppedCap, &nd);
+                    if (nd > kDroppedCap) throw std::runtime_error("rt_entry_host_update: more nodes left out than the list holds");
+                    t->dropped[i].assign(out.begin(), out.begin() + nd);
+                } else {
+                    t->records[i * EF_WORDS] = 1;
+                }
+            }
+        t->key = now, t->valid = true;
+        t->builds++;
+        return 1;
+    } catch (const std::exception& e) {
+        rt_internal_set_error(e.what());
+        return -1;
+    }
+}
+
+extern "C" uint64_t rt_entry_host_builds(const rt_entry_host* t) { return t ? t->builds : 0; }
+
+extern "C" const uint32_t* rt_entry_host_records(const rt_entry_host* t, size_t* count) {
+    if (count) *count = t ? t->records.size() / EF_WORDS : 0;
+    return t && !t->records.empty() ? t->records.data() : nullptr;
+}
+
+extern "C" const float* rt_entry_host_nodes(const rt_entry_host* t, size_t* count) {
+    if (count) *count = t ? t->mirror.nodes.size() / 8 : 0;
+    return t && !t->mirror.nodes.empty() ? t->mirror.nodes.data() : nullptr;
+}
+
+extern "C" int rt_entry_host_dropped(const rt_entry_host* t, int tx, int ty, uint32_t* out, int cap) {
+    if (!t || !t->valid || tx < 0 || ty < 0 || tx >= ef_tiles_x(t->key.width) || ty >= ef_tiles_y(t->key.height)) return -1;
+    const size_t i = (size_t)ty * ef_tiles_x(t->key.width) + tx;
+    const int n = (int)t->dropped[i].size();
+    for (int k = 0; k < n && k < cap; k++) out[k] = t->dropped[i][k];
+    return n;
+}
+
+extern "C" int rt_entry_host_replay(const rt_entry_host* t, size_t n, const int32_t* px, const int32_t* py, const float* ru,
+                                    const float* rv, rt_entry_replay* out) {
+    if (!t || !t->valid || !px || !py || !ru || !rv || !out) {
+        rt_internal_set_error("rt_entry_host_replay: bad argument");
+        return -1;
+    }
+    const EfCamera& c = t->key.cam;
+    const int W = t->key.width, H = t->key.height, tiles_x = ef_tiles_x(W);
+    for (size_t r = 0; r < n; r++) {
+        const int x = px[r], y = py[r];
+        if (x < 0 || y < 0 || x >= W || y >= H) {
+            rt_internal_set_error("rt_entry_host_replay: pixel outside the viewport");
+            return -1;
+        }
+        const float uvx = ((float)x + ru[r]) / (float)W, uvy = ((float)y + rv[r]) / (float)H;
+        float d[3];
+        for (int i = 0; i < 3; i++) d[i] = ((c.lower_left[i] + c.horizontal[i] * uvx) + c.vertical[i] * uvy) - c.origin[i];
+        rt_entry_replay& o = out[r];
+        std::memset(&o, 0, sizeof(o));
+        o.direction[0] = d[0], o.direction[1] = d[1], o.direction[2] = d[2];
+        walk(t->mirror, c.origin, d, std::vector<uint32_t>{0u}, &o.face_root, &o.t_root, &o.visits_root, &o.stack_root);
+        const size_t rec = ((size_t)(y / EF_TILE) * tiles_x + x / EF_TILE);
+        o.qualifies = t->mirror.fast && ef_ray_ok(c.origin, d) ? 1 : 0;
+        std::vector<uint32_t> start{0u};
+        if (o.qualifies) {
+            const uint32_t* R = &t->records[rec * EF_WORDS];
+            start.assign(R + 1, R + 1 + R[0]);
+            for (size_t a = 0, b = start.size(); a + 1 < b; a++, b--) std::swap(start[a], start[b - 1]);
+        }
+        walk(t->mirror, c.origin, d, start, &o.face_entry, &o.t_entry, &o.visits_entry, &o.stack_entry);
+        for (uint32_t k : t->dropped[rec])
+            if (aabb_hit(c.origin, d, &t->mirror.nodes[8 * (size_t)k], INFINITY)) o.dropped_hit++;
+    }
+    return 0;
+}
diff --git a/cuda-raytracing_amd/csrc/entry_host.h b/cuda-raytracing_amd/csrc/entry_host.h
--- /dev/null
+++ b/cuda-raytracing_amd/csrc/entry_host.h
@@ -0,0 +1,36 @@
+#pragma once
+
+#include <stddef.h>
+#include <stdint.h>
+
+#include "rt_abi.h"
+
+#ifdef __cplusplus
+extern "C" {
+#endif
+typedef struct rt_entry_host rt_entry_host;
+typedef struct rt_entry_replay {
+    uint32_t face_root, face_entry;
+    float t_root, t_entry;
+    uint32_t visits_root, visits_entry;
+    int32_t qualifies;
+    int32_t dropped_hit;
+    float direction[3];
+    uint32_t stack_root, stack_entry;
+    uint32_t reserved;
+} rt_entry_replay;
+rt_entry_host* rt_entry_host_create(void);
+void rt_entry_host_destroy(rt_entry_host* table);
+int rt_entry_host_update(rt_entry_host* table, const GPUBVHNode* nodes, size_t node_count, const uint32_t* face_indices,
+                         size_t index_count, const GPUFace* faces, size_t face_count, const GPUVertex* vertices,
+                         size_t vertex_count, const GPUCamera* camera, int width, int height);
+uint64_t rt_entry_host_builds(const rt_entry_host* table);
+const uint32_t* rt_entry_host_records(const rt_entry_host* table, size_t* record_count);
+const float* rt_entry_host_nodes(const rt_entry_host* table, size_t* node_count);
+int rt_entry_host_dropped(const rt_entry_host* table, int tile_x, int tile_y, uint32_t* out, int cap);
+int rt_entry_host_replay(const rt_entry_host* table, size_t count, const int32_t* px, const int32_t* py, const float* ru,
+                         const float* rv, rt_entry_replay* out);
+
+#ifdef __cplusplus
+}
+#endif
diff --git a/cuda-raytracing_amd/csrc/mirror.cpp b/cuda-raytracing_amd/csrc/mirror.cpp
--- a/cuda-raytracing_amd/csrc/mirror.cpp
+++ b/cuda-raytracing_amd/csrc/mirror.cpp
@@ -6,6 +6,7 @@
 #include "leaftree.h"
 
 #include <algorithm>
+#include <atomic>
 #include <cmath>
 #include <cstring>
 #include <map>
@@ -364,6 +365,7 @@
 std::map<const void*, Entry> g_mirrors;
 
 void release(Entry& e) {
+    rt_internal_forget_entry_table(e.dev.nodes);
     if (e.block) rt_free(e.block);
     e.block = nullptr;
 }
@@ -399,6 +401,9 @@
     e.dev.quads = at(8);
     e.dev.units = at(9);
     e.dev.face_leaf = at(10);
+    static std::atomic<uint64_t> generation{0};
+    e.dev.generation = ++generation;
+    e.dev.node_count = (uint32_t)(m.nodes.size() / 8);
     e.dev.depth = m.depth;
     e.dev.fast = m.fast;
     e.dev.screens = m.screens;
@@ -448,6 +453,7 @@
     o.bvh_small = 16;
     o.host_bvh = 0;
     o.leaf_screens = 0;
+    o.entry_frontier = 0;
     return o;
 }
 rt_build_options g_options = default_options();
@@ -478,7 +484,7 @@
     const rt_build_options v = o ? *o : default_options();
     if (v.leaf_tree_min < 2 || v.cut_clusters < 1 || v.cut_clusters > 32 || v.cluster_max < 1 || v.cluster_max > kClusterMax ||
         !(v.split_angle >= 0.0f && v.split_angle < 3.2f) || v.bvh_small < 2 || v.bvh_small > 64 || (v.host_bvh != 0 && v.host_bvh != 1) ||
-        (v.leaf_screens != 0 && v.leaf_screens != 1)) {
+        (v.leaf_screens != 0 && v.leaf_screens != 1) || (v.entry_frontier != 0 && v.entry_frontier != 1)) {
         rt_internal_set_error("rt_set_build_options: value out of range");
         return 1;
     }
diff --git a/cuda-raytracing_amd/csrc/mirror.h b/cuda-raytracing_amd/csrc/mirror.h
--- a/cuda-raytracing_amd/csrc/mirror.h
+++ b/cuda-raytracing_amd/csrc/mirror.h
@@ -55,6 +55,8 @@
     int depth = -1;
     bool fast = false;
     int screens = 0;
+    uint32_t node_count = 0;
+    uint64_t generation = 0;
     bool owned = true;
     uint64_t fingerprint = 0;
 };
@@ -63,4 +65,6 @@
 void rt_internal_forget_mirror(const void* gpu_nodes);
 bool rt_internal_lookup_mirror(const GPUScene* scene, MirrorDevice* out);
 
+void rt_internal_forget_entry_table(const void* mirror_nodes);
+
 void rt_internal_set_error(const char* msg);
diff --git a/cuda-raytracing_amd/csrc/rt_common.h b/cuda-raytracing_amd/csrc/rt_common.h
--- a/cuda-raytracing_amd/csrc/rt_common.h
+++ b/cuda-raytracing_amd/csrc/rt_common.h
@@ -59,6 +59,7 @@
     const float4* spairs;
     const float4* flat;
     const uint32_t* face_leaf;
+    const uint32_t* entry;
     uint32_t tune;
 };
 
diff --git a/cuda-raytracing_amd/csrc/rt_fast.h b/cuda-raytracing_amd/csrc/rt_fast.h
--- a/cuda-raytracing_amd/csrc/rt_fast.h
+++ b/cuda-raytracing_amd/csrc/rt_fast.h
@@ -863,6 +863,40 @@
     return tmax >= tmin && tmin < h.best && tmax > 0.0f;
 }
 
+template <class S>
+__device__ __forceinline__ bool trav_begin_entry(const float4* nodes4, const S& stk, const uint32_t* rec, const Ray& R,
+                                                 const Hit& h, Trav& T) {
+    const int base = (int)threadIdx.x * 4;
+    const uint4* rec4 = reinterpret_cast<const uint4*>(rec);
+    const uint4 q0 = rec4[0], q1 = rec4[1], q2 = rec4[2], q3 = rec4[3];
+    const uint32_t n = q0.x < 15u ? q0.x : 15u;
+    const int top = base + ((int)n - 1) * S::STEP;
+    auto park = [&](uint32_t j, uint32_t v) {
+        if (j < n) *stk.at(top - (int)j * S::STEP) = v;
+    };
+    park(0, q0.y), park(1, q0.z), park(2, q0.w), park(3, q1.x), park(4, q1.y), park(5, q1.z), park(6, q1.w), park(7, q2.x);
+    park(8, q2.y), park(9, q2.z), park(10, q2.w), park(11, q3.x), park(12, q3.y), park(13, q3.z), park(14, q3.w);
+    int sp = base;
+    for (int at = base; at <= top; at += S::STEP) {
+        const uint32_t idx = *stk.at(at);
+        const float4 lo = ldo(nodes4, 2 * idx), hi = ldo(nodes4, 2 * idx + 1);
+        float te, tx;
+        slab_approx(R, lo, hi, &te, &tx);
+        int co = R.fast ? classify_ok(te, tx) : UNSURE;
+        if (co == UNSURE) {
+            slab_exact(R, lo, hi, &te, &tx);
+            co = (tx >= te && tx > 0.0f) ? YES : NO;
+        }
+        if (co == YES) {
+            *stk.at(sp) = idx;
+            sp += S::STEP;
+        }
+    }
+    T.sp = sp;
+    return pop(nodes4, stk, T.sp, R, h.best, T.first, T.count);
+}
+constexpr uint32_t ENTRY_NONE = 0xffffffffu;
+
 template <bool STATS, class C>
 __device__ __forceinline__ bool screen_leaf(const float4* tris, const float4* pairs, const Ray& R, Hit& h, const Trav& T,
                                             C& c) {
@@ -1214,16 +1248,23 @@
     }
 }
 
-template <bool STATS, int MODE, class S, class C>
+template <bool STATS, int MODE, bool ENTRY = false, class S, class C>
 __device__ __forceinline__ void trace(const float4* nodes4, const float4* tris, const float4* pairs,
                                       const float4* tree, const float4* ltris, const float4* flat,
                                       const float4* spairs, uint32_t tune_arg, const S& stk, uint32_t* scratch,
                                       Ray& R, Hit& h, bool live, C& c, const float4* quads = nullptr,
-                                      const float4* units = nullptr, const uint32_t* face_leaf = nullptr) {
+                                      const float4* units = nullptr, const uint32_t* face_leaf = nullptr,
+                                      const uint32_t* etab = nullptr, uint32_t erec = ENTRY_NONE) {
     constexpr bool LEAN = (MODE & LEAN_BIT) != 0;
     const uint32_t tune = LEAN ? 0u : tune_arg;
     Trav T{0, 0, 0};
-    bool active = live && trav_begin<STATS>(nodes4, R, h, T, c);
+    bool active = false;
+    if constexpr (ENTRY) {
+        if (live && erec != ENTRY_NONE) active = trav_begin_entry(nodes4, stk, etab + 16 * (size_t)erec, R, h, T);
+        else if (live) active = trav_begin<STATS>(nodes4, R, h, T, c);
+    } else {
+        active = live && trav_begin<STATS>(nodes4, R, h, T, c);
+    }
     constexpr bool scr_on = !STATS && (MODE & 16) != 0 && (MODE & 32) != 0;
     constexpr bool TIMING = (MODE & 8) != 0;
     constexpr bool DEFER = !STATS && (MODE & 32) == 0 && (MODE & 4) != 0;
diff --git a/cuda-raytracing_amd/csrc/rt_fast_body.h b/cuda-raytracing_amd/csrc/rt_fast_body.h
--- a/cuda-raytracing_amd/csrc/rt_fast_body.h
+++ b/cuda-raytracing_amd/csrc/rt_fast_body.h
@@ -292,8 +292,16 @@
             }
         }
         rtfast::Ray R = rtfast::make_ray(ro, rd, nd, A(&RenderArgs::scene_fast) != 0);
-        rtfast::trace<STATS, MODE>(nodes4, tris, a.pairs, a.tree, a.ltris, a.flat, a.spairs, a.tune, stk, scratch, R, h,
-                                   path, c, a.quads, a.units, a.face_leaf);
+        constexpr bool ENTRY = LEAN && !STATS;
+        uint32_t erec = rtfast::ENTRY_NONE;
+        const uint32_t* etab = nullptr;
+        if constexpr (ENTRY) {
+            etab = A(&RenderArgs::entry);
+            if (etab && path && bounce == 0 && R.fast)
+                erec = (uint32_t)(y >> 3) * (uint32_t)((A(&RenderArgs::width) + 7) >> 3) + (uint32_t)(x >> 3);
+        }
+        rtfast::trace<STATS, MODE, ENTRY>(nodes4, tris, a.pairs, a.tree, a.ltris, a.flat, a.spairs, a.tune, stk, scratch, R, h,
+                                          path, c, a.quads, a.units, a.face_leaf, etab, erec);
         if (!path) continue;
 
         bool end = shade_segment<STATS, COLD>(a, h, ro, rd, nd, rng, color, thr, c);
diff --git a/cuda-raytracing_amd/csrc/rt_kernel.hip b/cuda-raytracing_amd/csrc/rt_kernel.hip
--- a/cuda-raytracing_amd/csrc/rt_kernel.hip
+++ b/cuda-raytracing_amd/csrc/rt_kernel.hip
@@ -21,6 +21,7 @@
 #include "rt_fast.h"
 
 #include "mirror.h"
+#include "entry_frontier.h"
 
 static_assert(MIRROR_BIG_LEAF == (uint32_t)rtfast::BIG, "pair records exist for exactly the big leaves");
 
@@ -207,8 +208,69 @@
     return (m & rtfast::LEAN_BIT) ? launch_fast_lean(stack, m, a, waves, s) : launch_fast_prod(stack, m, a, waves, s);
 }
 
+static_assert(EF_K == 15 && EF_TILE == 8 && EF_WORDS == 16, "the lean kernels read 16-word records of 8x8 sub-tiles (rt_fast.h)");
+__global__ __launch_bounds__(64) void entry_table_kernel(const float* nodes, uint32_t node_count, EfCamera cam, int width,
+                                                         int height, int tiles_x, int tiles, uint32_t* out) {
+    const int i = (int)(blockIdx.x * blockDim.x + threadIdx.x);
+    if (i >= tiles) return;
+    uint32_t rec[EF_WORDS];
+    ef_build_record(nodes, node_count, cam, width, height, i % tiles_x, i / tiles_x, rec);
+    uint4* o = reinterpret_cast<uint4*>(out + (size_t)EF_WORDS * i);
+    for (int k = 0; k < EF_WORDS / 4; k++) o[k] = make_uint4(rec[4 * k], rec[4 * k + 1], rec[4 * k + 2], rec[4 * k + 3]);
+}
+
+struct EntryTable {
+    EfKey key{};
+    bool valid = false;
+    uint32_t* dev = nullptr;
+    size_t bytes = 0;
+    hipEvent_t built = nullptr;
+    hipStream_t built_on = nullptr;
+};
+std::mutex g_entry_mutex;
+std::map<const void*, EntryTable> g_entry;
+std::atomic<uint64_t> g_entry_builds{0};
+
+const uint32_t* entry_table(const MirrorDevice& mir, const GPUCamera& c, int width, int height, hipStream_t s) {
+    EfCamera cam;
+    for (int i = 0; i < 3; i++) {
+        cam.origin[i] = c.origin[i], cam.lower_left[i] = c.lower_left_corner[i];
+        cam.horizontal[i] = c.horizontal[i], cam.vertical[i] = c.vertical[i];
+    }
+    const EfKey now = ef_make_key(cam, width, height, mir.nodes, mir.generation);
+    const int tiles_x = ef_tiles_x(width), tiles = tiles_x * ef_tiles_y(height);
+    const size_t bytes = (size_t)tiles * EF_WORDS * 4;
+    std::lock_guard<std::mutex> lock(g_entry_mutex);
+    EntryTable& t = g_entry[mir.nodes];
+    if (t.valid && ef_key_same(t.key, now)) {
+        if (s != t.built_on && hipStreamWaitEvent(s, t.built, 0) != hipSuccess) return nullptr;
+        return t.dev;
+    }
+    t.valid = false;
+    if (t.bytes != bytes) {
+        if (t.dev) (void)hipFree(t.dev);
+        t.dev = nullptr, t.bytes = 0;
+        if (hipMalloc((void**)&t.dev, bytes) != hipSuccess) {
+            (void)hipGetLastError();
+            t.dev = nullptr;
+            return nullptr;
+        }
+        t.bytes = bytes;
+    }
+    hipLaunchKernelGGL(entry_table_kernel, dim3((unsigned)((tiles + 63) / 64)), dim3(64), 0, s, (const float*)mir.nodes,
+                       mir.node_count, cam, width, height, tiles_x, tiles, t.dev);
+    if (hipGetLastError() != hipSuccess) return nullptr;
+    if (!t.built && hipEventCreateWithFlags(&t.built, hipEventDisableTiming) != hipSuccess) return nullptr;
+    if (hipEventRecord(t.built, s) != hipSuccess) return nullptr;
+    t.built_on = s;
+    t.key = now, t.valid = true;
+    g_entry_builds++;
+    return t.dev;
+}
+
 hipError_t launch_fast(const RenderArgs& args, int waves, int depth, bool stats, hipStream_t s) {
-    const int stack = (depth >= 0 && depth + 2 <= 30) ? 30 : (depth >= 0 && depth + 2 <= 40) ? 40 : 64;
+    const int need = depth + 2 + (args.entry ? EF_K - 1 : 0);
+    const int stack = (depth >= 0 && need <= 30) ? 30 : (depth >= 0 && need <= 40) ? 40 : 64;
     const ExperimentalKernels* x = g_experimental.load();
     const bool scr = args.screens != 0 && (args.tune & 4096u) == 0;
     if (stats && (args.tune & 256u)) {
@@ -770,6 +832,16 @@
         if (trav_nodes != (const GPUBVHNode*)mir.nodes) f.face_leaf = nullptr;
         return f;
     };
+    {
+        rt_build_options bo;
+        rt_get_build_options(&bo);
+        const bool timing = stats ? (a.tune & 256u) != 0 : a.lane_cost != nullptr;
+        if (bo.entry_frontier && mir.owned && !gate && a.tris && !want_flat && !want_wf && !a.tree && !a.queue_head &&
+            !a.screens && scene_fast && (!stats || timing) && trav_nodes == (const GPUBVHNode*)mir.nodes &&
+            depth >= 0 && depth + 2 + (EF_K - 1) <= 64 &&
+            (a.tune & 4096u) == 0 && ((a.tune >> 4) & 3u) < 2u && (lean_mode(trav(a), timing ? 25 : 17) & rtfast::LEAN_BIT))
+            a.entry = entry_table(mir, a.cam, p->width, p->height, s);
+    }
     hipError_t e;
     if (gate) {
         a.gate = gate, a.gate_value = 1;
@@ -799,6 +871,17 @@
     return check(e, "render_kernel launch");
 }
 
+extern "C" uint64_t rt_entry_table_builds(void) { return g_entry_builds.load(); }
+
+void rt_internal_forget_entry_table(const void* mirror_nodes) {
+    std::lock_guard<std::mutex> lock(g_entry_mutex);
+    auto it = g_entry.find(mirror_nodes);
+    if (it == g_entry.end()) return;
+    if (it->second.dev) (void)hipFree(it->second.dev);
+    if (it->second.built) (void)hipEventDestroy(it->second.built);
+    g_entry.erase(it);
+}
+
 extern "C" int rt_trace_rays(const rt_trace_params* p, const GPUScene* scene, void* stream) {
     if (!p) return set_error("rt_trace_rays: null params");
     if (!scene) return set_error("rt_trace_rays: null scene");
diff --git a/include/rt_abi.h b/include/rt_abi.h
--- a/include/rt_abi.h
+++ b/include/rt_abi.h
@@ -338,9 +338,12 @@
     uint32_t bvh_small;
     int32_t host_bvh;
     int32_t leaf_screens;
+    int32_t entry_frontier;
 } rt_build_options;
 void rt_get_build_options(rt_build_options* out);
 int rt_set_build_options(const rt_build_options* options);
+
+uint64_t rt_entry_table_builds(void);
 
 int rt_bvh_build_device(const GPUVertex* vertices, uint32_t vertex_count, const GPUFace* faces, uint32_t face_count,
                         GPUBVHNode* nodes_out, uint32_t* face_indices_out, uint32_t* node_count_out,
```

After: 2372, median of 6. 1.01x the previous value.
